# markweberdev/maskbit

Hardware: AMD Instinct MI355X
Metric: images/sec (256x256, 64-step MaskBit-12bit, CFG) (higher is better)
Workload: dtype f16

## Files before the change

include/maskbit_hip_diag.h:

```cpp
#ifndef MASKBIT_HIP_DIAG_H
#define MASKBIT_HIP_DIAG_H

#include "maskbit_hip.h"

#ifdef __cplusplus
extern "C" {
#endif

int mb_gemm(int epi, const void* A, const void* W, const float* bias, const float* residual, float* out_f32,
            void* out_h16, int M, int N, int K, int period, int variant, mb_stream stream);
int mb_gemm_ex(int epi, const void* A, const void* W, const float* bias, const float* residual, float* out_f32, void* out_h16,
               int M, int N, int K, const float* ln_stats, const float* ln_g, const float* ln_b, int period, int variant, mb_stream stream);
int mb_layernorm(const float* y, const float* gamma, const float* beta, float eps, float* x_f32, void* x_h16, void* x_lo, float* stats,
                 int M, int d, mb_stream stream);
int mb_gemm_act_split(int epi, const void* A_hi, const void* A_lo, const void* W, const float* bias, const float* residual,
                      float* out_f32, void* out_h16, int M, int N, int kw, int variant, mb_stream stream);
int mb_gemm_mini(int epi, const void* A, const void* W, const float* bias, const float* residual, float* out_f32, void* out_h16, void* out4,
                 void* out4_scale, int rows, int pair, int N, int K, int nlo, const void* const* lo, mb_stream stream);
int mb_gemm_mini_seq(int epi, const void* A, const void* W, const float* bias, const float* residual, float* out_f32, void* out_h16, void* out4,
                     void* out4_scale, void* out4l, void* out4l_scale, int rows, int pair, int seq_rows, int N, int K, int nlo, const void* const* lo, mb_stream stream);
int mb_w4_from_f32(const float* W, int N, int K, void* dst4, void* scale_out, mb_stream stream);
int mb_w4lo_from_f32(const float* W, int N, int K, void* dst4, void* scale_out, mb_stream stream);
int mb_gemm_head(int epi, const void* A_hi, const void* A_lo, const void* W_hi, const void* W_lo, const float* scale, const float* bias, int bias_per_pos,
                 float* out_f32, int M, int N, int kw, int period, mb_stream stream);
int mb_cast_f32_to_h16(const float* src, void* dst, int64_t n, mb_stream stream);
int mb_split_f32_planes(const float* src, void* hi, void* lo, int N, int K, float* scale_out, unsigned* tmp, mb_stream stream);
int mb_gemm_mini_split(int epi, const void* A_hi, const void* A_lo, const void* W, const float* bias, void* out_h16, void* out4, void* out4_scale,
                       int rows, int N, int kw, const void* const* lo, mb_stream stream);
int mb_layernorm_f4(const float* y, const float* gamma, const float* beta, float eps, float* x_f32, void* x_h16, void* x4, void* x4_scale, void* xl4,
                    void* xl4_scale, int M, int d, mb_stream stream);
int mb_layernorm_f4_seq(const float* y, const float* gamma, const float* beta, float eps, float* x_f32, void* x_h16, void* x4, void* x4_scale, void* xl4,
                        void* xl4_scale, int M, int d, int seq_rows, mb_stream stream);

int mb_layernorm_pair(const float* y, const float* gamma, const float* beta, float eps, void* x_h16, float* stats, void* x4, void* x4_scale, void* xl4,
                      void* xl4_scale, int P, int d, int seq_rows, mb_stream stream);
int mb_pairify(const float* x_f32, void* x_h16, void* x4, void* x4_scale, void* xl4, void* xl4_scale, int P, int d, int seq_rows, mb_stream stream);
int mb_embed_ln(const int64_t* tokens, const int64_t* labels, const uint8_t* drop, const float* w_in, const float* b_in, const float* class_emb,
                const float* pos, const float* gamma, const float* beta, const float* tables, float* x_f32, void* x_h16, void* x_lo, void* x4,
                void* x4_scale, void* xl4, void* xl4_scale, int nb, int seq, int m, int gbits, int d, int nclass, mb_stream stream);
int mb_embed_pair(const int64_t* tokens, const int64_t* labels, const float* w_in, const float* b_in, const float* class_emb, const float* pos,
                  const float* gamma, const float* beta, const float* tables, float* x_f32, void* x_h16, void* x4, void* x4_scale, void* xl4,
                  void* xl4_scale, int nb, int seq, int m, int gbits, int d, int nclass, mb_stream stream);
int mb_attention_pair(const void* qkv, void* out_h16, int pairs, int N, int d, int heads, mb_stream stream);
int mb_attention_pair_f4(const void* qkv, void* out_h16, void* out4, void* out4_scale, void* out4l, void* out4l_scale, int pairs, int N, int d, int heads, mb_stream stream);
int mb_attention(const void* qkv, void* out_h16, void* out4, void* out4_scale, int nb, int N, int d, int heads, mb_stream stream);
int mb_attention_probs(const void* qkv, float* out_f32, int nb, int N, int d, int heads, mb_stream stream);
int mb_gen_set_alo(mb_gen* g, int gemm_mask);
int mb_set_cu_count(int n);
int mb_gemm_ht_supported(int epi, int M, int N, int K);

int mb_seeded_noise(const int64_t* seeds, int step, float randomize_temperature, float conf_weight, float* exp_u, float* exp_noise, float* conf_u,
                    float* conf_noise, int B, int P, int C, mb_stream stream);

int mb_vq_argmin(const float* z, const float* codebook, int N, int C, int K, int l2, int splits, int64_t* idx, float* dist, mb_stream stream);

int mb_conv_layer(const void* in_h16, const float* w_oihw, const float* bias, const float* gn_gamma, const float* gn_beta, const void* residual_h16,
                  void* out_h16, float* img_nchw, uint8_t* img_nhwc_u8, const float* out_gamma, const float* out_beta, float* out_scale_shift,
                  float* out_gn_part, int* part_tiles, unsigned* saturated, int B, int H, int W, int Cin, int Cout, int ks, int up, int final_layer,
                  mb_stream stream);
int mb_groupnorm_stats(const void* x_h16, const float* gamma, const float* beta, float* scale_shift, int B, int HW, int C, mb_stream stream);
int mb_avgpool2(const void* x_h16, void* y_h16, int B, int H, int W, int C, mb_stream stream);
int mb_s2d(const void* x_h16, void* y_h16, int B, int H, int W, int C, mb_stream stream);

int mb_conv_relu_layer(const void* in_h16, const float* w_oihw, const float* bias, void* out_h16, unsigned* saturated, int B, int H, int W, int Cin,
                       int Cout, int ks, mb_stream stream);
int mb_maxpool2(const void* x_h16, void* y_h16, int B, int H, int W, int C, mb_stream stream);
int mb_lpips_input(const float* real, const float* fake, const float* shift_scale, void* out_h16, int B, int H, int W, int clamp01, mb_stream stream);
int mb_lpips_distance(const void* feat_a, const void* feat_b, const float* w, int B, int HW, int C, double* per_image, mb_stream stream);
int mb_lpips_features(mb_lpips* h, const float* real, const float* fake, int B, int H, int W, int clamp01, void* tap0, void* tap1, void* tap2, void* tap3,
                      void* tap4, mb_stream stream);

int mb_convbn_layer(const void* in_h16, const float* w_oihw, const float* scale, const float* shift, void* out_h16, unsigned* saturated, int B, int H,
                    int W, int Cin, int Cout, int kh, int kw, int stride, int ph, int pw, int in_off, int in_cs, int out_off, int out_cs, int variant,
                    mb_stream stream);
int mb_pool3(const void* x_h16, void* y_h16, int B, int H, int W, int C, int mode, int in_off, int in_cs, int out_off, int out_cs, mb_stream stream);
int mb_inception_input(const uint8_t* u8, void* out_h16, int B, int H, int W, mb_stream stream);
int mb_inception_taps(mb_inception* h, const uint8_t* u8, int B, int H, int W, void* map0, void* map1, void* map2, void* map3, float* tap64,
                      float* tap192, float* tap768, float* pool, float* logits_unbiased, float* logits, mb_stream stream);

int mb_spatial_attention(const void* q, const void* k, const void* v, void* out_h16, unsigned* sat, int B, int N, int ld, int ldo, mb_stream stream);
int mb_taming_set_tap(mb_taming* h, int block, void* out_h16);

#ifdef __cplusplus
}
#endif
#endif
```

maskbit_amd/_lib.py:

```python
from __future__ import annotations

import ctypes as C
import os
from typing import Optional

_HERE = os.path.dirname(os.path.abspath(__file__))
LIB_PATH = os.path.join(_HERE, "libmaskbit_hip.so")
ABI_VERSION = 8


class GenCfg(C.Structure):
    _fields_ = [(n, C.c_int) for n in ("bits", "splits", "hidden", "heads", "depth", "mlp", "seq", "nclass", "prenorm", "embed_tables", "precision")]


class DecCfg(C.Structure):
    _fields_ = [("token_size", C.c_int), ("hidden_channels", C.c_int), ("num_resolutions", C.c_int),
                ("num_res_blocks", C.c_int), ("num_channels", C.c_int), ("channel_mult", C.c_int * 8),
                ("latent_size", C.c_int), ("build_encoder", C.c_int), ("sample_with_conv", C.c_int),
                ("enc_res_blocks", C.c_int)]


class SamplePlan(C.Structure):
    _fields_ = [("num_steps", C.c_int), ("use_guidance", C.c_int), ("scale", C.POINTER(C.c_float)),
                ("temperature", C.POINTER(C.c_float)), ("mask_len", C.POINTER(C.c_int)), ("step_begin", C.c_int), ("step_end", C.c_int)]


class EditPlan(C.Structure):
    _fields_ = [("num_steps", C.c_int), ("use_guidance", C.c_int), ("scale", C.POINTER(C.c_float)),
                ("temperature", C.POINTER(C.c_float)), ("mask_ratio", C.POINTER(C.c_float)), ("step_begin", C.c_int), ("step_end", C.c_int)]


SIGNATURES = {
    "mb_gen_saturation_count": (C.c_int, [C.c_void_p, C.POINTER(C.c_uint), C.c_int, C.c_void_p]),
    "mb_abi_version": (C.c_int, []),
    "mb_last_error": (C.c_char_p, []),
    "mb_gen_create": (C.c_int, [C.POINTER(GenCfg), C.c_int, C.POINTER(C.c_void_p)]),
    "mb_gen_destroy": (None, [C.c_void_p]),
    "mb_gen_load": (C.c_int, [C.c_void_p, C.c_char_p, C.c_void_p, C.POINTER(C.c_int64), C.c_int, C.c_void_p]),
    "mb_gen_set_alo": (C.c_int, [C.c_void_p, C.c_int]),
    "mb_gen_forward": (C.c_int, [C.c_void_p, C.c_void_p, C.c_void_p, C.c_void_p, C.c_void_p, C.c_int, C.c_void_p]),
    "mb_gen_forward_cfg": (C.c_int, [C.c_void_p, C.c_void_p, C.c_void_p, C.c_void_p, C.c_int, C.c_void_p]),
    "mb_gen_forward_attn": (C.c_int, [C.c_void_p, C.c_void_p, C.c_void_p, C.c_void_p, C.c_void_p, C.c_void_p, C.c_int, C.c_void_p]),
    "mb_sample_step": (C.c_int, [C.c_void_p, C.c_void_p, C.c_float, C.c_float, C.c_void_p, C.c_void_p, C.c_int,
                                 C.c_void_p, C.c_void_p, C.c_void_p, C.c_int, C.c_int, C.c_int, C.c_int, C.c_void_p]),
    "mb_dec_create": (C.c_int, [C.POINTER(DecCfg), C.c_int, C.POINTER(C.c_void_p)]),
    "mb_dec_destroy": (None, [C.c_void_p]),
    "mb_dec_load": (C.c_int, [C.c_void_p, C.c_char_p, C.c_void_p, C.POINTER(C.c_int64), C.c_int, C.c_void_p]),
    "mb_dec_decode": (C.c_int, [C.c_void_p, C.c_void_p, C.c_void_p, C.c_void_p, C.c_int, C.c_void_p]),
    "mb_dec_saturation_count": (C.c_int, [C.c_void_p, C.POINTER(C.c_uint), C.c_int, C.c_void_p]),
    "mb_enc_encode": (C.c_int, [C.c_void_p, C.c_void_p, C.c_void_p, C.c_void_p, C.c_void_p, C.c_int, C.c_void_p]),
    "mb_dec_create_vq": (C.c_int, [C.POINTER(DecCfg), C.c_int, C.c_int, C.c_int, C.POINTER(C.c_void_p)]),
    "mb_dec_decode_latent": (C.c_int, [C.c_void_p, C.c_void_p, C.c_void_p, C.c_void_p, C.c_int, C.c_void_p]),
    "mb_enc_encode_vq": (C.c_int, [C.c_void_p, C.c_void_p, C.c_void_p, C.c_void_p, C.c_void_p, C.c_void_p, C.c_int, C.c_void_p]),
    "mb_vq_argmin": (C.c_int, [C.c_void_p, C.c_void_p, C.c_int, C.c_int, C.c_int, C.c_int, C.c_int, C.c_void_p, C.c_void_p, C.c_void_p]),
    "mb_sample": (C.c_int, [C.c_void_p, C.c_void_p, C.POINTER(SamplePlan), C.c_void_p, C.c_int, C.c_void_p, C.c_void_p,
                            C.c_void_p, C.c_void_p, C.c_void_p, C.c_void_p, C.c_void_p]),
    "mb_sample_step_edit": (C.c_int, [C.c_void_p, C.c_void_p, C.c_float, C.c_float, C.c_void_p, C.c_void_p, C.c_float, C.c_void_p,
                                      C.c_void_p, C.c_void_p, C.c_void_p, C.c_int, C.c_int, C.c_int, C.c_int, C.c_void_p]),
    "mb_sample_edit": (C.c_int, [C.c_void_p, C.c_void_p, C.POINTER(EditPlan), C.c_void_p, C.c_int, C.c_void_p, C.c_void_p, C.c_void_p,
                                 C.c_void_p, C.c_void_p, C.c_void_p, C.c_void_p, C.c_void_p]),
    "mb_sample_step_seeded": (C.c_int, [C.c_void_p, C.c_void_p, C.c_float, C.c_float, C.c_void_p, C.c_int, C.c_float, C.c_float, C.c_float, C.c_void_p,
                                        C.c_void_p, C.c_void_p, C.c_void_p, C.c_int, C.c_int, C.c_int, C.c_int, C.c_void_p]),
    "mb_sample_seeded": (C.c_int, [C.c_void_p, C.c_void_p, C.POINTER(EditPlan), C.c_void_p, C.c_int, C.c_void_p, C.c_void_p, C.c_float,
                                   C.POINTER(C.c_float), C.c_void_p, C.c_void_p, C.c_void_p, C.c_void_p, C.c_void_p]),
    "mb_seeded_noise": (C.c_int, [C.c_void_p, C.c_int, C.c_float, C.c_float, C.c_void_p, C.c_void_p, C.c_void_p, C.c_void_p, C.c_int, C.c_int, C.c_int,
                                  C.c_void_p]),
    "mb_edit_init": (C.c_int, [C.c_void_p, C.c_void_p, C.c_void_p, C.c_void_p, C.c_int, C.c_int, C.c_int, C.c_int, C.c_void_p]),
    "mb_edit_token_mask": (C.c_int, [C.c_void_p, C.c_void_p, C.c_int, C.c_int, C.c_int, C.c_int, C.c_void_p]),
    "mb_edit_composite": (C.c_int, [C.c_void_p, C.c_void_p, C.c_void_p, C.c_void_p, C.c_void_p, C.c_int, C.c_int, C.c_int, C.c_int, C.c_void_p]),
    "mb_gemm_ex": (C.c_int, [C.c_int, C.c_void_p, C.c_void_p, C.c_void_p, C.c_void_p, C.c_void_p, C.c_void_p, C.c_int, C.c_int, C.c_int,
                             C.c_void_p, C.c_void_p, C.c_void_p, C.c_int, C.c_int, C.c_void_p]),
    "mb_layernorm": (C.c_int, [C.c_void_p, C.c_void_p, C.c_void_p, C.c_float, C.c_void_p, C.c_void_p, C.c_void_p, C.c_void_p, C.c_int, C.c_int, C.c_void_p]),
    "mb_w4_from_f32": (C.c_int, [C.c_void_p, C.c_int, C.c_int, C.c_void_p, C.c_void_p, C.c_void_p]),
    "mb_w4lo_from_f32": (C.c_int, [C.c_void_p, C.c_int, C.c_int, C.c_void_p, C.c_void_p, C.c_void_p]),
    "mb_gemm_head": (C.c_int, [C.c_int, C.c_void_p, C.c_void_p, C.c_void_p, C.c_void_p, C.c_void_p, C.c_void_p, C.c_int, C.c_void_p, C.c_int, C.c_int,
                               C.c_int, C.c_int, C.c_void_p]),
    "mb_cast_f32_to_h16": (C.c_int, [C.c_void_p, C.c_void_p, C.c_int64, C.c_void_p]),
    "mb_split_f32_planes": (C.c_int, [C.c_void_p, C.c_void_p, C.c_void_p, C.c_int, C.c_int, C.c_void_p, C.c_void_p, C.c_void_p]),
    "mb_layernorm_f4": (C.c_int, [C.c_void_p, C.c_void_p, C.c_void_p, C.c_float, C.c_void_p, C.c_void_p, C.c_void_p, C.c_void_p, C.c_void_p, C.c_void_p,
                                  C.c_int, C.c_int, C.c_void_p]),
    "mb_layernorm_f4_seq": (C.c_int, [C.c_void_p, C.c_void_p, C.c_void_p, C.c_float] + [C.c_void_p] * 6 + [C.c_int] * 3 + [C.c_void_p]),
    "mb_layernorm_pair": (C.c_int, [C.c_void_p, C.c_void_p, C.c_void_p, C.c_float] + [C.c_void_p] * 6 + [C.c_int] * 3 + [C.c_void_p]),
    "mb_pairify": (C.c_int, [C.c_void_p] * 6 + [C.c_int] * 3 + [C.c_void_p]),
    "mb_embed_ln": (C.c_int, [C.c_void_p] * 17 + [C.c_int] * 6 + [C.c_void_p]),
    "mb_embed_pair": (C.c_int, [C.c_void_p] * 15 + [C.c_int] * 6 + [C.c_void_p]),
    "mb_attention": (C.c_int, [C.c_void_p, C.c_void_p, C.c_void_p, C.c_void_p, C.c_int, C.c_int, C.c_int, C.c_int, C.c_void_p]),
    "mb_attention_probs": (C.c_int, [C.c_void_p, C.c_void_p, C.c_int, C.c_int, C.c_int, C.c_int, C.c_void_p]),
    "mb_attention_pair": (C.c_int, [C.c_void_p, C.c_void_p, C.c_int, C.c_int, C.c_int, C.c_int, C.c_void_p]),
    "mb_attention_pair_f4": (C.c_int, [C.c_void_p, C.c_void_p, C.c_void_p, C.c_void_p, C.c_void_p, C.c_void_p, C.c_int, C.c_int, C.c_int, C.c_int, C.c_void_p]),
    "mb_gemm_mini": (C.c_int, [C.c_int, C.c_void_p, C.c_void_p, C.c_void_p, C.c_void_p, C.c_void_p, C.c_void_p, C.c_void_p, C.c_void_p, C.c_int, C.c_int,
                               C.c_int, C.c_int, C.c_int, C.POINTER(C.c_void_p), C.c_void_p]),
    "mb_gemm_mini_seq": (C.c_int, [C.c_int, C.c_void_p, C.c_void_p, C.c_void_p, C.c_void_p, C.c_void_p, C.c_void_p, C.c_void_p, C.c_void_p, C.c_void_p, C.c_void_p, C.c_int, C.c_int,
                                   C.c_int, C.c_int, C.c_int, C.c_int, C.POINTER(C.c_void_p), C.c_void_p]),
    "mb_gemm_mini_split": (C.c_int, [C.c_int, C.c_void_p, C.c_void_p, C.c_void_p, C.c_void_p, C.c_void_p, C.c_void_p, C.c_void_p, C.c_int, C.c_int, C.c_int,
                                     C.POINTER(C.c_void_p), C.c_void_p]),
    "mb_gemm_act_split": (C.c_int, [C.c_int, C.c_void_p, C.c_void_p, C.c_void_p, C.c_void_p, C.c_void_p, C.c_void_p, C.c_void_p, C.c_int, C.c_int, C.c_int,
                                    C.c_int, C.c_void_p]),
    "mb_gemm": (C.c_int, [C.c_int, C.c_void_p, C.c_void_p, C.c_void_p, C.c_void_p, C.c_void_p, C.c_void_p, C.c_int, C.c_int, C.c_int,
                          C.c_int, C.c_int, C.c_void_p]),
    "mb_conv_layer": (C.c_int, [C.c_void_p] * 13 + [C.POINTER(C.c_int), C.POINTER(C.c_uint)] + [C.c_int] * 8 + [C.c_void_p]),
    "mb_groupnorm_stats": (C.c_int, [C.c_void_p, C.c_void_p, C.c_void_p, C.c_void_p, C.c_int, C.c_int, C.c_int, C.c_void_p]),
    "mb_avgpool2": (C.c_int, [C.c_void_p, C.c_void_p, C.c_int, C.c_int, C.c_int, C.c_int, C.c_void_p]),
    "mb_s2d": (C.c_int, [C.c_void_p, C.c_void_p, C.c_int, C.c_int, C.c_int, C.c_int, C.c_void_p]),
    "mb_eval_workspace_bytes": (C.c_size_t, [C.c_int, C.c_int, C.c_int, C.c_int]),
    "mb_eval_images": (C.c_int, [C.c_void_p, C.c_void_p, C.c_int, C.c_int, C.c_int, C.c_int, C.c_uint, C.c_int, C.c_void_p, C.c_void_p, C.c_void_p, C.c_void_p]),
    "mb_eval_codebook": (C.c_int, [C.c_void_p, C.c_int64, C.c_int, C.c_void_p, C.c_void_p, C.c_void_p]),
    "mb_mlm_workspace_bytes": (C.c_size_t, [C.c_int, C.c_int, C.c_int, C.c_int]),
    "mb_mlm_state_bytes": (C.c_size_t, []),
    "mb_mlm_mask": (C.c_int, [C.c_void_p, C.c_void_p, C.c_void_p, C.c_int64, C.c_void_p, C.c_void_p, C.c_int, C.c_int, C.c_int, C.c_void_p]),
    "mb_mlm_loss": (C.c_int, [C.c_void_p, C.c_void_p, C.c_void_p, C.c_float, C.c_int, C.c_int, C.c_int, C.c_int, C.c_void_p, C.c_void_p, C.c_void_p,
                              C.c_void_p, C.c_void_p]),
    "mb_lpips_create": (C.c_int, [C.c_int, C.c_int, C.c_int, C.POINTER(C.c_void_p)]),
    "mb_lpips_destroy": (None, [C.c_void_p]),
    "mb_lpips_load": (C.c_int, [C.c_void_p, C.c_char_p, C.c_void_p, C.POINTER(C.c_int64), C.c_int, C.c_void_p]),
    "mb_lpips_forward": (C.c_int, [C.c_void_p, C.c_void_p, C.c_void_p, C.c_int, C.c_int, C.c_int, C.c_int, C.c_void_p, C.c_void_p, C.c_void_p]),
    "mb_lpips_saturation_count": (C.c_int, [C.c_void_p, C.POINTER(C.c_uint), C.c_int, C.c_void_p]),
    "mb_conv_relu_layer": (C.c_int, [C.c_void_p] * 4 + [C.POINTER(C.c_uint)] + [C.c_int] * 6 + [C.c_void_p]),
    "mb_maxpool2": (C.c_int, [C.c_void_p, C.c_void_p, C.c_int, C.c_int, C.c_int, C.c_int, C.c_void_p]),
    "mb_lpips_input": (C.c_int, [C.c_void_p, C.c_void_p, C.c_void_p, C.c_void_p, C.c_int, C.c_int, C.c_int, C.c_int, C.c_void_p]),
    "mb_lpips_distance": (C.c_int, [C.c_void_p, C.c_void_p, C.c_void_p, C.c_int, C.c_int, C.c_int, C.c_void_p, C.c_void_p]),
    "mb_lpips_features": (C.c_int, [C.c_void_p, C.c_void_p, C.c_void_p, C.c_int, C.c_int, C.c_int, C.c_int] + [C.c_void_p] * 6),
    "mb_fid_accumulate": (C.c_int, [C.c_void_p, C.c_int, C.c_int, C.c_int, C.c_int64, C.c_void_p, C.c_void_p, C.c_void_p]),
    "mb_is_workspace_bytes": (C.c_size_t, [C.c_int, C.c_int]),
    "mb_is_accumulate": (C.c_int, [C.c_void_p, C.c_int, C.c_int, C.c_int, C.c_int64, C.c_void_p, C.c_void_p, C.c_void_p, C.c_void_p]),
    "mb_inception_create": (C.c_int, [C.c_int, C.POINTER(C.c_void_p)]),
    "mb_inception_destroy": (None, [C.c_void_p]),
    "mb_inception_load": (C.c_int, [C.c_void_p, C.c_char_p, C.c_void_p, C.POINTER(C.c_int64), C.c_int, C.c_void_p]),
    "mb_inception_forward": (C.c_int, [C.c_void_p, C.c_void_p, C.c_int, C.c_int, C.c_int, C.c_void_p, C.c_void_p, C.c_void_p, C.c_void_p]),
    "mb_inception_saturation_count": (C.c_int, [C.c_void_p, C.POINTER(C.c_uint), C.c_int, C.c_void_p]),
    "mb_convbn_layer": (C.c_int, [C.c_void_p] * 5 + [C.POINTER(C.c_uint)] + [C.c_int] * 15 + [C.c_void_p]),
    "mb_pool3": (C.c_int, [C.c_void_p, C.c_void_p] + [C.c_int] * 9 + [C.c_void_p]),
    "mb_inception_input": (C.c_int, [C.c_void_p, C.c_void_p, C.c_int, C.c_int, C.c_int, C.c_void_p]),
    "mb_inception_taps": (C.c_int, [C.c_void_p, C.c_void_p, C.c_int, C.c_int, C.c_int] + [C.c_void_p] * 11),
    "mb_taming_create": (C.c_int, [C.c_int, C.c_int, C.POINTER(C.c_void_p)]),
    "mb_taming_destroy": (None, [C.c_void_p]),
    "mb_taming_load": (C.c_int, [C.c_void_p, C.c_char_p, C.c_void_p, C.POINTER(C.c_int64), C.c_int, C.c_void_p]),
    "mb_taming_encode": (C.c_int, [C.c_void_p, C.c_void_p, C.c_void_p, C.c_void_p, C.c_void_p, C.c_void_p, C.c_int, C.c_void_p]),
    "mb_taming_decode": (C.c_int, [C.c_void_p, C.c_void_p, C.c_void_p, C.c_void_p, C.c_int, C.c_void_p]),
    "mb_taming_decode_latent": (C.c_int, [C.c_void_p, C.c_void_p, C.c_void_p, C.c_void_p, C.c_int, C.c_void_p]),
    "mb_taming_saturation_count": (C.c_int, [C.c_void_p, C.POINTER(C.c_uint), C.c_int, C.c_void_p]),
    "mb_taming_set_tap": (C.c_int, [C.c_void_p, C.c_int, C.c_void_p]),
    "mb_spatial_attention": (C.c_int, [C.c_void_p] * 5 + [C.c_int] * 4 + [C.c_void_p]),
    "mb_set_cu_count":(C.c_int, [C.c_int]),
    "mb_gemm_ht_supported": (C.c_int, [C.c_int, C.c_int, C.c_int, C.c_int]),
    "mb_prof_enable": (C.c_int, [C.c_int]),
    "mb_prof_read": (C.c_int, [C.c_char_p, C.c_int]),
}

_lib: Optional[C.CDLL] = None


def load() -> C.CDLL:
    global _lib
    if _lib is not None:
        return _lib
    import torch
    if not os.path.exists(LIB_PATH):
        raise RuntimeError(
            f"{LIB_PATH} is missing: the MaskBit HIP kernels are not built. Run `python -c 'import __graft_entry__ as g; "
            f"g.build()'` (needs hipcc, gfx950). There is no CPU fallback in maskbit_amd.")
    lib = C.CDLL(LIB_PATH)
    for name, (res, args) in SIGNATURES.items():
        fn = getattr(lib, name)
        fn.restype = res
        fn.argtypes = args
    v = lib.mb_abi_version()
    if v != ABI_VERSION:
        raise RuntimeError(f"libmaskbit_hip.so ABI {v} != binding ABI {ABI_VERSION}; rebuild")
    _lib = lib
    return lib


def check(rc: int, what: str = "") -> None:
    if rc != 0:
        msg = load().mb_last_error()
        raise RuntimeError(f"{what or 'libmaskbit_hip'} failed (code {rc}): {msg.decode() if msg else '?'}")


def prof_enable(on, every: int = 1) -> None:
    load().mb_prof_enable(max(1, int(every)) if on else 0)


def prof_read() -> dict:
    buf = C.create_string_buffer(1 << 16)
    n = load().mb_prof_read(buf, len(buf))
    if n < 0:
        check(n, "mb_prof_read")
    out = {}
    for line in buf.value.decode().splitlines():
        name, calls, ms = line.split()
        out[name] = (int(calls), float(ms))
    return out
```

maskbit_amd/csrc/attention.hip:

```cpp
#include <type_traits>

#include "mb_kernels.h"

namespace mb {

constexpr int ATT_SDEPTH = 3;
constexpr int ATT_NKT = 18;
constexpr int ATT_NP = ATT_NKT * 16;
constexpr int ATT_NW = 4;
constexpr int ATT_MAXQT = (ATT_NKT + ATT_NW - 1) / ATT_NW;

typedef __attribute__((ext_vector_type(4))) unsigned u32x4;

__device__ __forceinline__ uint2 fp4_row8(const f32x4 (&o)[4], float inv, float mul) {
  uint32_t p[4];
#pragma unroll
  for (int nt = 0; nt < 4; ++nt) p[nt] = fp4_pack4(o[nt][0] * inv, o[nt][1] * inv, o[nt][2] * inv, o[nt][3] * inv, mul);
  const auto sw = __builtin_amdgcn_permlane16_swap((p[0] & 0xffffu) | (p[2] << 16), (p[1] & 0xffffu) | (p[3] << 16), false, false);
  const uint32_t q0 = __builtin_amdgcn_perm(sw[1], sw[0], 0x05040100u);
  const uint32_t q1 = __builtin_amdgcn_perm(sw[1], sw[0], 0x07060302u);
  const auto sx = __builtin_amdgcn_permlane32_swap(q0, q1, false, false);
  return make_uint2(sx[0], sx[1]);
}

__device__ __forceinline__ uint2 fp4_row8_vals(const f32x4 (&lo)[4], float mul) {
  uint32_t p[4];
#pragma unroll
  for (int nt = 0; nt < 4; ++nt) p[nt] = fp4_pack4(lo[nt][0], lo[nt][1], lo[nt][2], lo[nt][3], mul);
  const auto sw = __builtin_amdgcn_permlane16_swap((p[0] & 0xffffu) | (p[2] << 16), (p[1] & 0xffffu) | (p[3] << 16), false, false);
  const uint32_t q0 = __builtin_amdgcn_perm(sw[1], sw[0], 0x05040100u);
  const uint32_t q1 = __builtin_amdgcn_perm(sw[1], sw[0], 0x07060302u);
  const auto sx = __builtin_amdgcn_permlane32_swap(q0, q1, false, false);
  return make_uint2(sx[0], sx[1]);
}
__device__ __forceinline__ uint2 fp4_lo_block(const f32x4 (&o)[4], float inv, uint32_t& sbyte) {
  f32x4 lo[4];
  float am = 0.f;
#pragma unroll
  for (int nt = 0; nt < 4; ++nt)
#pragma unroll
    for (int r = 0; r < 4; ++r) { const float v = o[nt][r] * inv; lo[nt][r] = v - (float)to_h(v); am = fmaxf(am, fabsf(lo[nt][r])); }
  am = rows_max(am);
  sbyte = fp4_scale_byte_nosat(am);
  return fp4_row8_vals(lo, fp4_scale_mul_nosat(am));
}

template <int DH, int AUX = 0>
__global__ __launch_bounds__(64 * ATT_NW, 2) void attention_kernel(const h16* __restrict__ qkv, h16* __restrict__ out,
                                                          int N, int d, int heads, float scale_log2e, int sq_off = 0,
                                                          uint8_t* __restrict__ out4 = nullptr, uint8_t* __restrict__ out4s = nullptr, int out4_nseq = 0,
                                                          uint8_t* __restrict__ out4l = nullptr, uint8_t* __restrict__ out4ls = nullptr) {
  constexpr int ROW = DH * 2;
  constexpr int SL = DH / 8;
  constexpr int KS = DH / 32;
  constexpr int NT = DH / 16;
  constexpr int RPI = 64 / SL;
  constexpr int NINST = ATT_NP / RPI;
  __shared__ __attribute__((aligned(16))) char smem[2 * ATT_NP * ROW];

  const int tid = threadIdx.x, lane = tid & 63;
  const int wave = __builtin_amdgcn_readfirstlane(tid >> 6);
  char* Ks = smem;
  char* Vs = Ks + ATT_NP * ROW;
  const int sq0 = blockIdx.x / heads, h = blockIdx.x - sq0 * heads;
  const size_t rs = (size_t)3 * d;
  constexpr int NPASS = AUX == 4 ? 2 : 1;
  f32x4 oc[AUX == 4 ? ATT_MAXQT - 1 : 1][DH / 16];
  constexpr int LAST_WAVES = ATT_NKT - ATT_NW * (ATT_MAXQT - 1);
  __shared__ __attribute__((aligned(16))) float oc_last[AUX == 4 ? LAST_WAVES * 64 * DH / 4 : 4];
#pragma unroll 1
  for (int pass = 0; pass < NPASS; ++pass) {
  const int sq = sq0 + (AUX == 4 ? pass * sq_off : sq_off);
  const h16* base = qkv + (size_t)sq * N * rs + h * DH;
  if (AUX == 4 && pass > 0) __syncthreads();

  auto kswz = [](int row) { return SL == 8 ? ((row >> 1) & 7) : ((0 - (row >> 2)) & 3); };
  auto vswz = [](int row) { return SL == 8 ? (((row >> 1) & 3) << 1) : (((row >> 1) & 1) << 1); };

  for (int j = wave; j < NINST; j += ATT_NW) {
    const int row = j * RPI + lane / SL, p = lane % SL;
    const h16* src = base + (size_t)min(row, N - 1) * rs;
    MB_GLDS16(src + d + (p ^ kswz(row)) * 8, Ks + j * 1024);
    MB_GLDS16(src + 2 * d + (p ^ vswz(row)) * 8, Vs + j * 1024);
  }
  const int wlast = wave;
  auto qt_of = [&](int i) { return i < ATT_MAXQT - 1 ? wave + ATT_NW * i : ATT_NW * (ATT_MAXQT - 1) + wlast; };
  const int l15 = lane & 15, g = lane >> 4;
  const int nqt = (N + 15) / 16;
  h16x8 qf[ATT_MAXQT][KS];
  auto q_fetch = [&](int i) {
    const int qrow = min(qt_of(i) * 16 + l15, N - 1);
#pragma unroll
    for (int ks = 0; ks < KS; ++ks) qf[i][ks] = *(const h16x8*)(base + (size_t)qrow * rs + (ks * 4 + g) * 8);
  };
#pragma unroll
  for (int i = 0; i < (AUX == 4 ? 1 : ATT_MAXQT); ++i) q_fetch(i);
  asm volatile("s_waitcnt vmcnt(0)" ::: "memory");
  __syncthreads();

  const int koff = l15 * ROW;
  const int vrow = g * 4 + (l15 >> 2), vchunk = (l15 & 3) * 8;
  unsigned vb_nt[NT];
#pragma unroll
  for (int nt = 0; nt < NT; ++nt)
    vb_nt[nt] = (unsigned)(uintptr_t)Vs + vrow * ROW + ((((nt * 32 + vchunk) >> 4) ^ vswz(vrow)) << 4) + (vchunk & 8);

#pragma unroll
  for (int i = 0; i < ATT_MAXQT; ++i) {
    const int qt = qt_of(i);
    if (qt >= nqt) break;
    f32x4 s[ATT_NKT];
    constexpr int GK = ATT_SDEPTH, NG = ATT_NKT / GK;
    static_assert(ATT_NKT % GK == 0, "whole groups");
    h16x8 kfr[2][GK][KS];
    auto k_fetch = [&](h16x8 (&dst)[GK][KS], int grp) {
#pragma unroll
      for (int j = 0; j < GK; ++j) {
        const int kt = grp * GK + j, row = kt * 16 + l15;
#pragma unroll
        for (int ks = 0; ks < KS; ++ks) dst[j][ks] = *(const h16x8*)(Ks + kt * 16 * ROW + koff + (((ks * 4 + g) ^ kswz(row)) * 16));
      }
    };
    k_fetch(kfr[0], 0);
#pragma unroll
    for (int grp = 0; grp < NG; ++grp) {
      if (grp + 1 < NG) k_fetch(kfr[(grp + 1) & 1], grp + 1);
#pragma unroll
      for (int ks = 0; ks < KS; ++ks)
#pragma unroll
        for (int j = 0; j < GK; ++j) {
          const int kt = grp * GK + j;
          if (ks == 0) s[kt] = f32x4{0.f, 0.f, 0.f, 0.f};
          if (kt == ATT_NKT - 1 && kt * 16 >= N) continue;
          s[kt] = MB_MFMA_16x16x32(kfr[grp & 1][j][ks], qf[i][ks], s[kt]);
        }
      __builtin_amdgcn_sched_barrier(0);
    }
    if (AUX == 4 && i + 1 < ATT_MAXQT) q_fetch(i + 1);
    float mx = -INFINITY;
#pragma unroll
    for (int kt = 0; kt < ATT_NKT; ++kt)
#pragma unroll
      for (int r = 0; r < 4; ++r) {
        if (kt >= ATT_NKT - 2) s[kt][r] = (kt * 16 + g * 4 + r < N) ? s[kt][r] : -INFINITY;
        mx = fmaxf(mx, s[kt][r]);
      }
    mx = rows_max(mx);
// ... 33 lines not shown
        else
          asm volatile("s_waitcnt lgkmcnt(0)" : "+v"(cur[0][0]), "+v"(cur[0][1]), "+v"(cur[1][0]), "+v"(cur[1][1]),
                       "+v"(cur[2][0]), "+v"(cur[2][1]), "+v"(cur[3][0]), "+v"(cur[3][1])::"memory");
      } else {
        if (more_in_flight)
          asm volatile("s_waitcnt lgkmcnt(4)" : "+v"(cur[0][0]), "+v"(cur[0][1]), "+v"(cur[1][0]), "+v"(cur[1][1])::"memory");
        else
          asm volatile("s_waitcnt lgkmcnt(0)" : "+v"(cur[0][0]), "+v"(cur[0][1]), "+v"(cur[1][0]), "+v"(cur[1][1])::"memory");
      }
      __builtin_amdgcn_sched_barrier(0);
      const f32x4 p0 = s[2 * kb], p1 = s[2 * kb + 1];
      const h16x8 pf = {(h16)p0[0], (h16)p0[1], (h16)p0[2], (h16)p0[3],
                         (h16)p1[0], (h16)p1[1], (h16)p1[2], (h16)p1[3]};
#pragma unroll
      for (int nt = 0; nt < NT; ++nt) {
        const u32x4 raw = {cur[nt][0].x, cur[nt][0].y, cur[nt][1].x, cur[nt][1].y};
        o[nt] = MB_MFMA_16x16x32(__builtin_bit_cast(h16x8, raw), pf, o[nt]);
      }
      __builtin_amdgcn_sched_barrier(0);
    };
    constexpr int NKB = ATT_NKT / 2;
    issue(va, std::integral_constant<int, 0>{});
    auto step = [&](auto kbc) {
      constexpr int kb = decltype(kbc)::value;
      if constexpr (kb < NKB) {
        if constexpr (kb + 1 < NKB) issue(vb, std::integral_constant<int, kb + 1>{});
        consume(va, kb, kb + 1 < NKB);
        if constexpr (kb + 1 < NKB) {
          if constexpr (kb + 2 < NKB) issue(va, std::integral_constant<int, kb + 2>{});
          consume(vb, kb + 1, kb + 2 < NKB);
        }
      }
    };
    step(std::integral_constant<int, 0>{}); step(std::integral_constant<int, 2>{}); step(std::integral_constant<int, 4>{});
    step(std::integral_constant<int, 6>{}); step(std::integral_constant<int, 8>{});
    static_assert(NKB <= 10, "add steps");
    const int q = qt * 16 + l15;
    if constexpr ((AUX == 4 || AUX == 5) && DH == 64) {
      if (out4 && (AUX != 4 || pass == 0)) {
        float am = 0.f;
#pragma unroll
        for (int nt = 0; nt < NT; ++nt)
#pragma unroll
          for (int r = 0; r < 4; ++r) am = fmaxf(am, fabsf(o[nt][r]));
        am = rows_max(am) * inv;
        const float mul = fp4_scale_mul_nosat(am);
        const uint2 pk8 = fp4_row8(o, inv, mul);
        uint32_t lob = 0;
        uint2 lo8 = make_uint2(0u, 0u);
        if (out4l) lo8 = fp4_lo_block(o, inv, lob);
        if (q < 256) {
          const size_t row = (size_t)sq * N + q;
          if (g == 0) out4s[fp4_scale_index(h, out4_nseq, sq, q)] = (uint8_t)fp4_scale_byte_nosat(am);
          *(uint2*)(out4 + row * 2 * d + (h * DH) / 2 + (g >> 1) * 16 + (g & 1) * 8) = pk8;
          if (out4l) {
            if (g == 0) out4ls[fp4_scale_index(h, out4_nseq, sq, q)] = (uint8_t)lob;
            *(uint2*)(out4l + row * 2 * d + (h * DH) / 2 + (g >> 1) * 16 + (g & 1) * 8) = lo8;
          }
        }
      }
    }
    if (q < N) {
      const size_t ooff = ((size_t)sq * N + q) * d + h * DH;
#pragma unroll
      for (int nt = 0; nt < NT; ++nt) {
        f32x4 v = {o[nt][0] * inv, o[nt][1] * inv, o[nt][2] * inv, o[nt][3] * inv};
        if constexpr (AUX == 4) {
          if (i < ATT_MAXQT - 1) { f32x4& r = oc[i < ATT_MAXQT - 1 ? i : 0][nt]; if (pass == 0) r = v; else v = v - r; }
          else { f32x4* slot = (f32x4*)oc_last + ((qt - ATT_NW * (ATT_MAXQT - 1)) * NT + nt) * 64 + lane; if (pass == 0) *slot = v; else v = v - *slot; }
        }
        const h16x4 hi = {to_h(v[0]), to_h(v[1]), to_h(v[2]), to_h(v[3])};
        *(h16x4*)(out + ooff + nt * 16 + g * 4) = hi;
      }
    }
  }
  }
}

constexpr int ATTL_KB = 128;
template <int DH, bool PAIRM = false>
__global__ __launch_bounds__(256, 2) void attention_long_kernel(const h16* __restrict__ qkv, h16* __restrict__ out,
                                                               int N, int d, int heads, int nchunk, float scale_log2e, int sq_off = 0,
                                                               uint8_t* __restrict__ out4 = nullptr, uint8_t* __restrict__ out4s = nullptr, int out4_nseq = 0,
                                                               uint8_t* __restrict__ out4l = nullptr, uint8_t* __restrict__ out4ls = nullptr) {
  constexpr int ROW = DH * 2, SL = DH / 8, KS = DH / 32, NT = DH / 16, RPI = 64 / SL;
  constexpr int BLK_BYTES = ATTL_KB * ROW;
  constexpr int NINST = ATTL_KB / RPI;
  constexpr int NKT = ATTL_KB / 16;
  __shared__ __attribute__((aligned(16))) char smem[2 * 2 * BLK_BYTES];
  const int tid = threadIdx.x, lane = tid & 63;
  const int wave = __builtin_amdgcn_readfirstlane(tid >> 6);
  int bid = blockIdx.x;
  const int chunk = bid % nchunk; bid /= nchunk;
  const int sq0 = bid / heads, h = bid - sq0 * heads;
  const size_t rs = (size_t)3 * d;
  auto kswz = [](int row) { return SL == 8 ? ((row >> 1) & 7) : ((0 - (row >> 2)) & 3); };
  auto vswz = [](int row) { return SL == 8 ? (((row >> 1) & 3) << 1) : (((row >> 1) & 1) << 1); };
  const int nblk = (N + ATTL_KB - 1) / ATTL_KB;
  f32x4 oc[NT];
#pragma unroll 1
  for (int pass = 0; pass < (PAIRM ? 2 : 1); ++pass) {
  const int sq = sq0 + pass * sq_off;
  const h16* base = qkv + (size_t)sq * N * rs + h * DH;
  if (PAIRM && pass > 0) __syncthreads();
  auto stage = [&](int b, int buf) {
    char* Kb = smem + buf * 2 * BLK_BYTES;
    char* Vb = Kb + BLK_BYTES;
    for (int j = wave; j < NINST; j += 4) {
      const int r = j * RPI + lane / SL, p = lane % SL;
      const h16* src = base + (size_t)min(b * ATTL_KB + r, N - 1) * rs;
      MB_GLDS16(src + d + (p ^ kswz(r)) * 8, Kb + j * 1024);
      MB_GLDS16(src + 2 * d + (p ^ vswz(r)) * 8, Vb + j * 1024);
    }
  };
  const int l15 = lane & 15, g = lane >> 4;
  const int qt = chunk * 4 + wave;
  h16x8 qf[KS];
  {
    const int qrow = min(qt * 16 + l15, N - 1);
#pragma unroll
    for (int ks = 0; ks < KS; ++ks) qf[ks] = *(const h16x8*)(base + (size_t)qrow * rs + (ks * 4 + g) * 8);
  }
  const int koff = l15 * ROW;
  const int vrow = g * 4 + (l15 >> 2), vchunk = (l15 & 3) * 8;
  unsigned vb_nt[NT];
#pragma unroll
  for (int nt = 0; nt < NT; ++nt) vb_nt[nt] = vrow * ROW + ((((nt * 32 + vchunk) >> 4) ^ vswz(vrow)) << 4) + (vchunk & 8);

  float m_run = -INFINITY, l_run = 0.f;
  f32x4 o[NT];
#pragma unroll
  for (int nt = 0; nt < NT; ++nt) o[nt] = f32x4{0.f, 0.f, 0.f, 0.f};

  stage(0, 0);
  for (int b = 0; b < nblk; ++b) {
    if (b + 1 < nblk) stage(b + 1, (b + 1) & 1);
    if (b + 1 < nblk) {
      if constexpr (NINST == 16) asm volatile("s_waitcnt vmcnt(8)" ::: "memory");
      else asm volatile("s_waitcnt vmcnt(4)" ::: "memory");
    } else asm volatile("s_waitcnt vmcnt(0)" ::: "memory");
    __syncthreads();
    const char* Kb = smem + (b & 1) * 2 * BLK_BYTES;
    const unsigned Vb = (unsigned)(uintptr_t)(Kb + BLK_BYTES);
    f32x4 sblk[NKT];
#pragma unroll
    for (int kt = 0; kt < NKT; ++kt) {
      sblk[kt] = f32x4{0.f, 0.f, 0.f, 0.f};
      const int row = kt * 16 + l15;
#pragma unroll
      for (int ks = 0; ks < KS; ++ks) {
        const h16x8 kf = *(const h16x8*)(Kb + kt * 16 * ROW + koff + (((ks * 4 + g) ^ kswz(row)) * 16));
        sblk[kt] = MB_MFMA_16x16x32(kf, qf[ks], sblk[kt]);
      }
    }
    const int key0 = b * ATTL_KB;
    float mx = -INFINITY;
#pragma unroll
    for (int kt = 0; kt < NKT; ++kt)
#pragma unroll
      for (int r = 0; r < 4; ++r) {
        if (key0 + kt * 16 + g * 4 + r >= N) sblk[kt][r] = -INFINITY;
        mx = fmaxf(mx, sblk[kt][r]);
      }
    mx = rows_max(mx);
    const float m_new = fmaxf(m_run, mx);
    const float alpha = __builtin_amdgcn_exp2f((m_run - m_new) * scale_log2e);
    const float mxs = m_new * scale_log2e;
    float sum = 0.f;
    h16x4 pk[NKT];
#pragma unroll
    for (int kt = 0; kt < NKT; ++kt) {
      float p[4];
#pragma unroll
      for (int r = 0; r < 4; ++r) { p[r] = __builtin_amdgcn_exp2f(fmaf(sblk[kt][r], scale_log2e, -mxs)); sum += p[r]; }
      pk[kt] = h16x4{(h16)p[0], (h16)p[1], (h16)p[2], (h16)p[3]};
    }
    sum = rows_sum(sum);
// ... 47 lines not shown
        if (out4l) {
          if (g == 0) out4ls[fp4_scale_index(h, out4_nseq, sq, q, (N - 1) >> 6)] = (uint8_t)lob;
          *(uint2*)(out4l + row * 2 * d + (h * DH) / 2 + (g >> 1) * 16 + (g & 1) * 8) = lo8;
        }
      }
    }
  }
  if (q < N || PAIRM) {
    const size_t ooff = ((size_t)sq * N + min(q, N - 1)) * d + h * DH;
#pragma unroll
    for (int nt = 0; nt < NT; ++nt) {
      f32x4 v = {o[nt][0] * inv, o[nt][1] * inv, o[nt][2] * inv, o[nt][3] * inv};
      if constexpr (PAIRM) { if (pass == 0) oc[nt] = v; else v = v - oc[nt]; }
      if (q >= N) continue;
      const h16x4 hi = {to_h(v[0]), to_h(v[1]), to_h(v[2]), to_h(v[3])};
      *(h16x4*)(out + ooff + nt * 16 + g * 4) = hi;
    }
  }
  }
}

template <int DH>
__global__ __launch_bounds__(256) void attention_probs_kernel(const h16* __restrict__ qkv, float* __restrict__ out, int N, int d, int heads) {
  extern __shared__ __attribute__((aligned(16))) char smem[];
  const int wave = threadIdx.x >> 6, lane = threadIdx.x & 63;
  const int rows_per_seq = (N + 3) / 4;
  const int seq = blockIdx.x / rows_per_seq, r = (blockIdx.x % rows_per_seq) * 4 + wave;
  if (r >= N) return;
  float* sc = (float*)smem + (size_t)wave * 2 * N;
  float* av = sc + N;
  for (int j = lane; j < N; j += 64) av[j] = 0.f;
  const float scale = 1.0f / sqrtf((float)DH), invh = 1.0f / (float)heads;
  const h16* base = qkv + (size_t)seq * N * 3 * d;
  for (int h = 0; h < heads; ++h) {
    float q[DH];
    const h16* qp = base + (size_t)r * 3 * d + h * DH;
#pragma unroll
    for (int i = 0; i < DH / 8; ++i) {
      const h16x8 v = *(const h16x8*)(qp + i * 8);
#pragma unroll
      for (int e = 0; e < 8; ++e) q[i * 8 + e] = (float)v[e] * scale;
    }
    float mx = -3.0e38f;
    for (int j = lane; j < N; j += 64) {
      const h16* kp = base + (size_t)j * 3 * d + d + h * DH;
      float a = 0.f;
#pragma unroll
      for (int i = 0; i < DH / 8; ++i) {
        const h16x8 v = *(const h16x8*)(kp + i * 8);
#pragma unroll
        for (int e = 0; e < 8; ++e) a = fmaf(q[i * 8 + e], (float)v[e], a);
      }
      sc[j] = a;
      mx = fmaxf(mx, a);
    }
    mx = wave_max(mx);
    float sum = 0.f;
    for (int j = lane; j < N; j += 64) { const float e = expf(sc[j] - mx); sc[j] = e; sum += e; }
    sum = wave_sum(sum);
    const float w = invh / sum;
    for (int j = lane; j < N; j += 64) av[j] = fmaf(sc[j], w, av[j]);
  }
  float* orow = out + ((size_t)seq * N + r) * N;
  for (int j = lane; j < N; j += 64) orow[j] = av[j];
}

int attention_probs(hipStream_t s, const h16* qkv, float* out, int nb, int N, int d, int heads) {
  const int dh = d / heads;
  const size_t lds = (size_t)4 * 2 * N * sizeof(float);
  if ((dh != 32 && dh != 64) || lds > 160 * 1024) return -1;
  dim3 grid(nb * ((N + 3) / 4)), block(256);
  if (dh == 64) {
    (void)hipFuncSetAttribute((const void*)attention_probs_kernel<64>, hipFuncAttributeMaxDynamicSharedMemorySize, (int)lds);
    hipLaunchKernelGGL(attention_probs_kernel<64>, grid, block, lds, s, qkv, out, N, d, heads);
  } else {
    (void)hipFuncSetAttribute((const void*)attention_probs_kernel<32>, hipFuncAttributeMaxDynamicSharedMemorySize, (int)lds);
    hipLaunchKernelGGL(attention_probs_kernel<32>, grid, block, lds, s, qkv, out, N, d, heads);
  }
  return 0;
}

static bool att_streams(int N) { return N > ATT_NP || N < ATT_NP - 32; }

void attention(hipStream_t s, const h16* qkv, h16* out, int nb, int N, int d, int heads, uint8_t* out4, uint8_t* out4s) {
  const int dh = d / heads;
  const float scale_log2e = 1.4426950408889634f / sqrtf((float)dh);
  if (att_streams(N)) {
    const int nchunk = (N + 63) / 64;
    const bool f4 = N > ATT_NP && (N - 1) % 64 == 0;
    dim3 grid(nb * heads * nchunk), block(256);
    if (dh == 64) hipLaunchKernelGGL(attention_long_kernel<64>, grid, block, 0, s, qkv, out, N, d, heads, nchunk, scale_log2e, 0, f4 ? out4 : nullptr, f4 ? out4s : nullptr, nb);
    else hipLaunchKernelGGL(attention_long_kernel<32>, grid, block, 0, s, qkv, out, N, d, heads, nchunk, scale_log2e);
    return;
  }
  dim3 grid(nb * heads), block(64 * ATT_NW);
  if (out4 && dh == 64 && N == 257)
    hipLaunchKernelGGL((attention_kernel<64, 5>), grid, block, 0, s, qkv, out, N, d, heads, scale_log2e, 0, out4, out4s, nb);
  else if (dh == 64) hipLaunchKernelGGL(attention_kernel<64>, grid, block, 0, s, qkv, out, N, d, heads, scale_log2e);
  else hipLaunchKernelGGL(attention_kernel<32>, grid, block, 0, s, qkv, out, N, d, heads, scale_log2e);
}

int attention_pair(hipStream_t s, const h16* qkv, h16* out, int P, int N, int d, int heads, uint8_t* out4, uint8_t* out4s, uint8_t* out4l, uint8_t* out4ls) {
  const int dh = d / heads;
  if (dh != 64 && dh != 32) return -1;
  if ((out4l || out4ls) && (!out4 || !out4s || !out4l || !out4ls)) return -1;
  const float scale_log2e = 1.4426950408889634f / sqrtf((float)dh);
  if (att_streams(N)) {
    if ((out4 || out4s) && (dh != 64 || (N - 1) % 64 || N < ATT_NP)) return -1;
    const int nchunk = ((N + 15) / 16 + 3) / 4;
    dim3 grid(P * heads * nchunk), block(256);
    if (dh == 64) hipLaunchKernelGGL((attention_long_kernel<64, true>), grid, block, 0, s, qkv, out, N, d, heads, nchunk, scale_log2e, P, out4, out4s, P, out4l, out4ls);
    else hipLaunchKernelGGL((attention_long_kernel<32, true>), grid, block, 0, s, qkv, out, N, d, heads, nchunk, scale_log2e, P);
    return 0;
  }
  dim3 grid(P * heads), block(64 * ATT_NW);
  if ((out4 || out4s) && (dh != 64 || N != 257)) return -1;
  if (dh == 64) hipLaunchKernelGGL((attention_kernel<64, 4>), grid, block, 0, s, qkv, out, N, d, heads, scale_log2e, P, out4, out4s, P, out4l, out4ls);
  else hipLaunchKernelGGL((attention_kernel<32, 4>), grid, block, 0, s, qkv, out, N, d, heads, scale_log2e, P);
  return 0;
}

}
```

maskbit_amd/csrc/diag.hip:

```cpp
#include <hip/hip_runtime.h>

#include "../../include/maskbit_hip_diag.h"
#include "mb_abi.h"
#include "mb_conv.h"
#include "mb_kernels.h"
#include "mb_spattn.h"
#include "mb_vq.h"

using mb::fail;
using mb::launched;
using mb::ProfScope;

namespace {

int run_gemm(mb_stream stream, int epi, const mb::GemmArgs& a, int variant, const char* mini = nullptr) {
  ProfScope p("gemm_diag", (hipStream_t)stream);
  if (mb::gemm_tn((hipStream_t)stream, (mb::GemmEpi)epi, a, variant))
    return mini ? fail(-3, "%s: shape refused", mini) : fail(-3, "GEMM shape M=%d N=%d K=%d is outside the kernels' shapes", a.M, a.N, a.K);
  return launched();
}

int w4_entry(const char* what, decltype(mb::w4_from_f32)* pack, const float* W, int N, int K, void* dst4, void* scale_out, mb_stream stream) {
  if (!W || !dst4 || !scale_out || N <= 0 || K <= 0 || N % 64 || K % 128) return fail(-1, "%s: bad arguments", what);
  pack((hipStream_t)stream, W, (uint8_t*)dst4, N, K, (uint8_t*)scale_out);
  return launched();
}

int pool_entry(const char* what, decltype(mb::launch_s2d)* launch, const void* x, void* y, int B, int H, int W, int C, mb_stream stream) {
  if (!x || !y) return fail(-1, "%s: null argument", what);
  if (B <= 0 || H <= 0 || W <= 0 || H % 2 || W % 2 || C <= 0 || C % 8) return fail(-1, "%s: H and W must be even, C a multiple of 8", what);
  launch((hipStream_t)stream, (const h16*)x, (h16*)y, B, H, W, C);
  return launched();
}

int f4_rows(const char* who, mb::Fp4Rows& f4, void* x4, void* x4_scale, void* xl4, void* xl4_scale, int rows, int d, int seq_rows) {
  f4 = mb::Fp4Rows{};
  if ((x4 != nullptr) != (x4_scale != nullptr) || (xl4 != nullptr) != (xl4_scale != nullptr)) return fail(-1, "%s: an e2m1 copy and its scale array go together", who);
  if (!x4 && !xl4) return 0;
  if (d != 768 && d != 1024) return fail(-1, "%s: e2m1 copies are written at d = 768 / 1024 only, not %d", who, d);
  if (seq_rows < 65 || (seq_rows - 1) % 64 || rows % seq_rows)
    return fail(-1, "%s: e2m1 copies: sequences of 64 k tokens + the class token, whole sequences (%d rows of %d)", who, rows, seq_rows);
  f4 = mb::Fp4Rows{(uint8_t*)x4, (uint8_t*)x4_scale, (uint8_t*)xl4, (uint8_t*)xl4_scale, rows / seq_rows, seq_rows};
  return 0;
}

int embed_args(const char* who, mb::EmbedArgs& e, const int64_t* tokens, const int64_t* labels, const float* w_in, const float* b_in, const float* class_emb,
               const float* pos, const float* gamma, const float* beta, const float* tables, float* x_f32, void* x_h16, void* x4, void* x4_scale, void* xl4,
               void* xl4_scale, int nb, int seq, int m, int gbits, int d, int nclass) {
  if (!tokens || !labels || !class_emb || !pos || !gamma || !beta || !x_f32 || !x_h16 || (!tables && (!w_in || !b_in))) return fail(-1, "%s: null argument", who);
  if (nb <= 0 || seq <= 0 || m <= 0 || gbits <= 0 || d <= 0 || nclass < 0) return fail(-1, "%s: bad sizes", who);
  if (d > 2048) return fail(-1, "%s: d = %d is beyond the row kernels (2048)", who, d);
  if ((int64_t)m * gbits > 24) return fail(-1, "%s: %d groups of %d bits are beyond the embed kernels (24 bits)", who, m, gbits);
  if (tables && m > 8) return fail(-1, "%s: %d embedding tables are beyond the embed kernel (8)", who, m);
  mb::Fp4Rows f4;
  if (int rc = f4_rows(who, f4, x4, x4_scale, xl4, xl4_scale, nb * (seq + 1), d, seq + 1)) return rc;
  e = mb::EmbedArgs{tokens, labels, nullptr, nullptr, b_in, class_emb, pos, gamma, beta, x_f32, (h16*)x_h16, nb, seq, m, gbits, d, nclass, tables};
  e.f4 = f4;
  return 0;
}
int embed_weight(const char* who, mb::DevArena& arena, mb::EmbedArgs& e, const float* w_in, hipStream_t s) {
  if (e.tables) return 0;
  const int K = e.m * e.gbits;
  float* wt = nullptr;
  arena.get(&wt, (size_t)K * e.d);
  if (int rc = arena.failed(who)) return rc;
  mb::transpose_f32(s, w_in, wt, e.d, K);
  e.w_in = wt;
  return 0;
}

}

extern "C" {

int mb_set_cu_count(int n) { mb::set_cu_count(n); return 0; }
int mb_gemm_ht_supported(int epi, int M, int N, int K) {
  mb::GemmArgs a{nullptr, nullptr, nullptr, nullptr, nullptr, nullptr, M, N, K, 0};
  return mb::gemm_ht_supported((mb::GemmEpi)epi, a) ? 1 : 0;
}

int mb_gemm(int epi, const void* A, const void* W, const float* bias, const float* residual, float* out_f32, void* out_h16,
            int M, int N, int K, int period, int variant, mb_stream stream) {
  if (!A || !W || !bias || epi < 0 || epi > 4) return fail(-1, "mb_gemm: bad arguments");
  if (K % 64) return fail(-1, "mb_gemm: K must be a multiple of 64");
  mb::GemmArgs a{(const h16*)A, (const h16*)W, bias, residual, out_f32, (h16*)out_h16, M, N, K, period};
  return run_gemm(stream, epi, a, variant);
}
int mb_gemm_ex(int epi, const void* A, const void* W, const float* bias, const float* residual, float* out_f32, void* out_h16,
               int M, int N, int K, const float* ln_stats, const float* ln_g, const float* ln_b, int period, int variant, mb_stream stream) {
  if (!A || !W || !bias || epi < 0 || epi > 4) return fail(-1, "mb_gemm_ex: bad arguments");
  if (K % 64) return fail(-1, "mb_gemm_ex: K must be a multiple of 64");
  if (ln_stats && (!ln_g || !ln_b || epi != mb::EPI_RES_F32)) return fail(-1, "mb_gemm_ex: LayerNorm residual needs gamma, beta and the fp32+residual epilogue");
  mb::GemmArgs a{(const h16*)A, (const h16*)W, bias, residual, out_f32, (h16*)out_h16, M, N, K, period, nullptr, ln_stats, ln_g, ln_b};
  return run_gemm(stream, epi, a, variant);
}
int mb_gemm_act_split(int epi, const void* A_hi, const void* A_lo, const void* W, const float* bias, const float* residual, float* out_f32,
                      void* out_h16, int M, int N, int kw, int variant, mb_stream stream) {
  if (!A_hi || !A_lo || !W || !bias || epi < 0 || epi > 3 || kw <= 0 || kw % 64) return fail(-1, "mb_gemm_act_split: bad arguments");
  mb::GemmArgs a{(const h16*)A_hi, (const h16*)W, bias, residual, out_f32, (h16*)out_h16, M, N, 2 * kw, 0};
  a.A2 = (const h16*)A_lo; a.kw = kw;
  return run_gemm(stream, epi, a, variant);
}
int mb_gemm_mini(int epi, const void* A, const void* W, const float* bias, const float* residual, float* out_f32, void* out_h16, void* out4,
                 void* out4_scale, int rows, int pair, int N, int K, int nlo, const void* const* lo , mb_stream stream) {
  return mb_gemm_mini_seq(epi, A, W, bias, residual, out_f32, out_h16, out4, out4_scale, nullptr, nullptr, rows, pair, 0, N, K, nlo, lo, stream);
}
int mb_gemm_mini_seq(int epi, const void* A, const void* W, const float* bias, const float* residual, float* out_f32, void* out_h16, void* out4,
                     void* out4_scale, void* out4l, void* out4l_scale, int rows, int pair, int seq_rows, int N, int K, int nlo, const void* const* lo, mb_stream stream) {
  if ((out4l || out4l_scale) && (!out4l || !out4l_scale || !out4 || !out4_scale)) return fail(-1, "mb_gemm_mini_seq: the lo copy (out4l / out4l_scale) rides with the value copy (out4 / out4_scale)");
  if (!A || !W || !bias || epi < 0 || epi > 2 || rows <= 0 || K <= 0 || K % 64 || nlo < 0 || nlo > 2 || (nlo && !lo)) return fail(-1, "mb_gemm_mini: bad arguments");
  mb::GemmArgs a{(const h16*)A, (const h16*)W, bias, residual, out_f32, (h16*)out_h16, pair ? 2 * rows : rows, N, K, 0};
  if (pair) a.pair_rows = rows;
  a.seq_rows = seq_rows;
  a.nlo = nlo;
  for (int i = 0; i < nlo; ++i) a.lo[i] = {(const uint8_t*)lo[4 * i], (const uint8_t*)lo[4 * i + 1], (const uint8_t*)lo[4 * i + 2], (const uint8_t*)lo[4 * i + 3]};
  a.out4 = (uint8_t*)out4; a.out4_scale = (uint8_t*)out4_scale;
  a.out4l = (uint8_t*)out4l; a.out4l_scale = (uint8_t*)out4l_scale;
  if ((!seq_rows && a.M % 257) || !mb::gemm_ht_supported((mb::GemmEpi)epi, a)) return fail(-3, "mb_gemm_mini: shape not supported by the sequence-aligned tiles");
  return run_gemm(stream, epi, a, 257, "mb_gemm_mini");
}
int mb_gemm_mini_split(int epi, const void* A_hi, const void* A_lo, const void* W, const float* bias, void* out_h16, void* out4, void* out4_scale,
                       int rows, int N, int kw, const void* const* lo , mb_stream stream) {
  if (!A_hi || !A_lo || !W || !bias || !out_h16 || !lo || epi < 0 || epi > 1 || rows <= 0 || rows % 257 || kw <= 0 || kw % 128)
    return fail(-1, "mb_gemm_mini_split: bad arguments");
  mb::GemmArgs a{(const h16*)A_hi, (const h16*)W, bias, nullptr, nullptr, (h16*)out_h16, rows, N, 2 * kw, 0};
  a.A2 = (const h16*)A_lo; a.kw = kw;
  a.nlo = 1;
  a.lo[0] = {(const uint8_t*)lo[0], (const uint8_t*)lo[1], (const uint8_t*)lo[2], (const uint8_t*)lo[3]};
  a.out4 = (uint8_t*)out4; a.out4_scale = (uint8_t*)out4_scale;
  if (!mb::gemm_ht_supported((mb::GemmEpi)epi, a)) return fail(-3, "mb_gemm_mini_split: shape not supported by the sequence-aligned tiles");
  return run_gemm(stream, epi, a, 257, "mb_gemm_mini_split");
}

int mb_gemm_head(int epi, const void* A_hi, const void* A_lo, const void* W_hi, const void* W_lo, const float* scale, const float* bias, int bias_per_pos,
                 float* out_f32, int M, int N, int kw, int period, mb_stream stream) {
  if (!A_hi || !A_lo || !W_hi || !bias || !out_f32) return fail(-1, "mb_gemm_head: null argument");
  if ((W_lo != nullptr) != (scale != nullptr)) return fail(-1, "mb_gemm_head: the weights' lo plane and the scale go together");
  if (epi != mb::EPI_GELU_F32 && epi != mb::EPI_LOGITS_F32) return fail(-1, "mb_gemm_head: epilogue 3 or 4");
  if (M <= 0 || N <= 0 || N % 4 || kw <= 0 || kw % 64) return fail(-1, "mb_gemm_head: M > 0, N a multiple of 4, kw a multiple of 64");
  if (epi == mb::EPI_LOGITS_F32 && (period < 2 || M % period)) return fail(-1, "mb_gemm_head: epilogue 4: whole sequences of period >= 2 rows");
  if (bias_per_pos && epi != mb::EPI_LOGITS_F32) return fail(-1, "mb_gemm_head: a per-position bias goes with epilogue 4");
  mb::GemmArgs a{(const h16*)A_hi, (const h16*)W_hi, bias, nullptr, out_f32, nullptr, M, N, (W_lo ? 3 : 2) * kw, period, scale};
  a.A2 = (const h16*)A_lo; a.kw = kw; a.W2 = (const h16*)W_lo;
  a.bias_per_pos = bias_per_pos;
  return run_gemm(stream, epi, a, 0, "mb_gemm_head");
}
int mb_cast_f32_to_h16(const float* src, void* dst, int64_t n, mb_stream stream) {
  if (!src || !dst || n < 0) return fail(-1, "mb_cast_f32_to_h16: bad arguments");
  mb::cast_f32_to_h16((hipStream_t)stream, src, (h16*)dst, (size_t)n);
  return launched();
}
int mb_split_f32_planes(const float* src, void* hi, void* lo, int N, int K, float* scale_out, unsigned* tmp, mb_stream stream) {
  if (!src || !hi || !lo || !scale_out || !tmp || N <= 0 || K <= 0) return fail(-1, "mb_split_f32_planes: bad arguments");
  mb::split_f32_to_h16_planes((hipStream_t)stream, src, (h16*)hi, (h16*)lo, N, K, scale_out, tmp);
  return launched();
}

int mb_w4_from_f32(const float* W, int N, int K, void* dst4, void* scale_out, mb_stream stream) {
  return w4_entry("mb_w4_from_f32", mb::w4_from_f32, W, N, K, dst4, scale_out, stream);
}
int mb_w4lo_from_f32(const float* W, int N, int K, void* dst4, void* scale_out, mb_stream stream) {
  return w4_entry("mb_w4lo_from_f32", mb::w4lo_from_f32, W, N, K, dst4, scale_out, stream);
}

int mb_layernorm(const float* y, const float* gamma, const float* beta, float eps, float* x_f32, void* x_h16, void* x_lo, float* stats, int M,
                 int d, mb_stream stream) {
  if (!y || !gamma || !beta || M <= 0 || d <= 0 || d > 2048) return fail(-1, "mb_layernorm: bad arguments");
  mb::layernorm_rows((hipStream_t)stream, y, gamma, beta, eps, x_f32, (h16*)x_h16, stats, M, d, (h16*)x_lo);
  return launched();
}
int mb_layernorm_f4_seq(const float* y, const float* gamma, const float* beta, float eps, float* x_f32, void* x_h16, void* x4, void* x4_scale, void* xl4,
                        void* xl4_scale, int M, int d, int seq_rows, mb_stream stream) {
  if (!y || !gamma || !beta || (!x4 && !xl4) || M <= 0) return fail(-1, "mb_layernorm_f4: bad arguments (an e2m1 output is required)");
  mb::Fp4Rows f4;
  if (int rc = f4_rows("mb_layernorm_f4", f4, x4, x4_scale, xl4, xl4_scale, M, d, seq_rows)) return rc;
  mb::layernorm_rows((hipStream_t)stream, y, gamma, beta, eps, x_f32, (h16*)x_h16, nullptr, M, d, nullptr, f4);
  return launched();
}
int mb_layernorm_f4(const float* y, const float* gamma, const float* beta, float eps, float* x_f32, void* x_h16, void* x4, void* x4_scale, void* xl4,
                    void* xl4_scale, int M, int d, mb_stream stream) {
  return mb_layernorm_f4_seq(y, gamma, beta, eps, x_f32, x_h16, x4, x4_scale, xl4, xl4_scale, M, d, 257, stream);
}

int mb_layernorm_pair(const float* y, const float* gamma, const float* beta, float eps, void* x_h16, float* stats, void* x4, void* x4_scale, void* xl4,
                      void* xl4_scale, int P, int d, int seq_rows, mb_stream stream) {
  if (!y || !gamma || !beta || !x_h16 || P <= 0 || d <= 0 || d > 2048) return fail(-1, "mb_layernorm_pair: bad arguments");
  mb::Fp4Rows f4;
  if (int rc = f4_rows("mb_layernorm_pair", f4, x4, x4_scale, xl4, xl4_scale, P, d, seq_rows)) return rc;
  if (mb::layernorm_pair((hipStream_t)stream, y, gamma, beta, eps, (h16*)x_h16, stats, P, d, f4))
    return fail(-3, "mb_layernorm_pair: width %d is outside the pair kernels (768 or 1024)", d);
  return launched();
}
int mb_pairify(const float* x_f32, void* x_h16, void* x4, void* x4_scale, void* xl4, void* xl4_scale, int P, int d, int seq_rows, mb_stream stream) {
  if (!x_f32 || !x_h16 || P <= 0 || d <= 0 || d > 2048) return fail(-1, "mb_pairify: bad arguments");
  mb::Fp4Rows f4;
  if (int rc = f4_rows("mb_pairify", f4, x4, x4_scale, xl4, xl4_scale, P, d, seq_rows)) return rc;
  if (mb::pairify_rows((hipStream_t)stream, x_f32, (h16*)x_h16, P, d, f4))
    return fail(-3, "mb_pairify: width %d is outside the pair kernels (768 or 1024)", d);
  return launched();
}
int mb_embed_ln(const int64_t* tokens, const int64_t* labels, const uint8_t* drop, const float* w_in, const float* b_in, const float* class_emb,
                const float* pos, const float* gamma, const float* beta, const float* tables, float* x_f32, void* x_h16, void* x_lo, void* x4,
                void* x4_scale, void* xl4, void* xl4_scale, int nb, int seq, int m, int gbits, int d, int nclass, mb_stream stream) {
  mb::EmbedArgs e;
  if (int rc = embed_args("mb_embed_ln", e, tokens, labels, w_in, b_in, class_emb, pos, gamma, beta, tables, x_f32, x_h16, x4, x4_scale, xl4, xl4_scale,
                          nb, seq, m, gbits, d, nclass)) return rc;
  e.drop = drop; e.x_lo = (h16*)x_lo;
  mb::DevArena arena;
  if (int rc = embed_weight("mb_embed_ln", arena, e, w_in, (hipStream_t)stream)) return rc;
  mb::embed_ln((hipStream_t)stream, e);
  if (hipStreamSynchronize((hipStream_t)stream) != hipSuccess) return fail(-10, "mb_embed_ln: the launch failed");
  return launched();
}
int mb_embed_pair(const int64_t* tokens, const int64_t* labels, const float* w_in, const float* b_in, const float* class_emb, const float* pos,
                  const float* gamma, const float* beta, const float* tables, float* x_f32, void* x_h16, void* x4, void* x4_scale, void* xl4,
                  void* xl4_scale, int nb, int seq, int m, int gbits, int d, int nclass, mb_stream stream) {
  const bool f4 = x4 || x4_scale || xl4 || xl4_scale;
  if (tables || (m > 0 && gbits > 0 && (int64_t)m * gbits > 24) || (!f4 && d > 0 && d <= 2048 && d != 768 && d != 1024))
    return fail(-3, "mb_embed_pair: not served by the fused kernel (embedding tables, more than 24 bits, widths other than 768 / 1024): embed_ln + pairify");
  mb::EmbedArgs e;
  if (int rc = embed_args("mb_embed_pair", e, tokens, labels, w_in, b_in, class_emb, pos, gamma, beta, tables, x_f32, x_h16, x4, x4_scale, xl4, xl4_scale,
                          nb, seq, m, gbits, d, nclass)) return rc;
  mb::DevArena arena;
  if (int rc = embed_weight("mb_embed_pair", arena, e, w_in, (hipStream_t)stream)) return rc;
  const int refused = mb::embed_pair((hipStream_t)stream, e);
  if (hipStreamSynchronize((hipStream_t)stream) != hipSuccess) return fail(-10, "mb_embed_pair: the launch failed");
  if (refused) return fail(-3, "mb_embed_pair: not served by the fused kernel");
  return launched();
}

int mb_attention(const void* qkv, void* out_h16, void* out4, void* out4_scale, int nb, int N, int d, int heads, mb_stream stream) {
  if (!qkv || !out_h16 || (!out4) != (!out4_scale) || nb <= 0 || N <= 0 || d <= 0 || heads <= 0 || d % heads) return fail(-1, "mb_attention: bad arguments");
  if (d / heads != 32 && d / heads != 64) return fail(-3, "mb_attention: head width %d is outside the attention kernels (32 or 64)", d / heads);
  ProfScope p("attention", (hipStream_t)stream);
  mb::attention((hipStream_t)stream, (const h16*)qkv, (h16*)out_h16, nb, N, d, heads, (uint8_t*)out4, (uint8_t*)out4_scale);
  return launched();
}
int mb_attention_probs(const void* qkv, float* out_f32, int nb, int N, int d, int heads, mb_stream stream) {
  if (!qkv || !out_f32 || nb <= 0 || N <= 0 || d <= 0 || heads <= 0 || d % heads) return fail(-1, "mb_attention_probs: bad arguments");
  if (mb::attention_probs((hipStream_t)stream, (const h16*)qkv, out_f32, nb, N, d, heads))
    return fail(-3, "mb_attention_probs: head width %d / N = %d tokens is outside the probabilities kernel (32 or 64; N <= 5120)", d / heads, N);
  return launched();
}
int mb_attention_pair(const void* qkv, void* out_h16, int pairs, int N, int d, int heads, mb_stream stream) {
  if (!qkv || !out_h16 || pairs <= 0 || N <= 0 || heads <= 0 || d % heads) return fail(-1, "mb_attention_pair: bad arguments");
  ProfScope p("attention", (hipStream_t)stream);
  if (mb::attention_pair((hipStream_t)stream, (const h16*)qkv, (h16*)out_h16, pairs, N, d, heads, nullptr, nullptr))
    return fail(-3, "mb_attention_pair: head width %d (N = %d tokens) is outside the attention kernels", d / heads, N);
  return launched();
}
int mb_attention_pair_f4(const void* qkv, void* out_h16, void* out4, void* out4_scale, void* out4l, void* out4l_scale, int pairs, int N, int d, int heads, mb_stream stream) {
  if (!qkv || !out_h16 || !out4 || !out4_scale || (!out4l) != (!out4l_scale) || pairs <= 0 || N <= 0 || heads <= 0 || d % heads) return fail(-1, "mb_attention_pair_f4: bad arguments");
  ProfScope p("attention", (hipStream_t)stream);
  if (mb::attention_pair((hipStream_t)stream, (const h16*)qkv, (h16*)out_h16, pairs, N, d, heads, (uint8_t*)out4, (uint8_t*)out4_scale, (uint8_t*)out4l, (uint8_t*)out4l_scale))
    return fail(-3, "mb_attention_pair_f4: head width %d / N = %d tokens: no e2m1 copy for this shape", d / heads, N);
  return launched();
}

int mb_seeded_noise(const int64_t* seeds, int step, float randomize_temperature, float conf_weight, float* exp_u, float* exp_noise, float* conf_u,
                    float* conf_noise, int B, int P, int C, mb_stream stream) {
  if (!seeds || !exp_noise || !conf_noise) return fail(-1, "mb_seeded_noise: null argument");
  if (B <= 0 || P <= 0 || C <= 0 || step < 0) return fail(-1, "mb_seeded_noise: bad sizes");
  if (exp_u == exp_noise || conf_u == conf_noise) return fail(-1, "mb_seeded_noise: the uniforms and the noise must not alias");
  if (mb::seeded_noise_dump((hipStream_t)stream, seeds, step, randomize_temperature, conf_weight, exp_u, exp_noise, conf_u, conf_noise, B, P, C))
    return fail(-1, "mb_seeded_noise: C=%d or P=%d too large", C, P);
  return launched();
}

int mb_vq_argmin(const float* z, const float* codebook, int N, int C, int K, int l2, int splits, int64_t* idx, float* dist, mb_stream stream) {
  if (!z || !codebook || !idx) return fail(-1, "mb_vq_argmin: null argument");
  if (int rc = mb::vq_argmin(z, codebook, N, C, K, l2, splits, idx, dist, (hipStream_t)stream)) return rc;
  return launched();
}

int mb_conv_layer(const void* in_h16, const float* w_oihw, const float* bias, const float* gn_gamma, const float* gn_beta, const void* residual_h16,
                  void* out_h16, float* img_nchw, uint8_t* img_nhwc_u8, const float* out_gamma, const float* out_beta, float* out_scale_shift,
                  float* out_gn_part, int* part_tiles, unsigned* saturated, int B, int H, int W, int Cin, int Cout, int ks, int up_, int final_layer,
                  mb_stream stream) {
  using namespace mb;
  hipStream_t s = (hipStream_t)stream;
  const bool fin = final_layer != 0, up = up_ != 0;
  if (!in_h16 || !w_oihw || B <= 0 || Cin <= 0 || Cout <= 0) return fail(-1, "mb_conv_layer: null or empty argument");
  if (ks < 1 || ks > 3) return fail(-1, "mb_conv_layer: ks must be 1, 2 or 3");
  if (H <= 0 || W <= 0 || H % TH8 || W % TW) return fail(-1, "mb_conv_layer: the output must be whole 8 x 16 pixel tiles");
  if (fin && (ks != 3 || up || Cout > 4 || residual_h16 || !(img_nchw || img_nhwc_u8))) return fail(-1, "mb_conv_layer: final layer: ks 3, at most 4 channels, no residual, an image output");
  if (!fin && (!out_h16 || Cout % 4)) return fail(-1, "mb_conv_layer: fp16 output: Cout must be a multiple of 4");
  if (up && ks != 3) return fail(-1, "mb_conv_layer: upsampling goes with ks 3");
  if (ks == 2 && (Cin % 16 || gn_gamma)) return fail(-1, "mb_conv_layer: ks 2 (stride-2 conv): Cin must be a multiple of 16, no prologue");
  if ((gn_gamma != nullptr) != (gn_beta != nullptr) || (gn_gamma && (Cin % CK || Cin > 2048))) return fail(-1, "mb_conv_layer: prologue: gamma and beta, Cin a multiple of 64 up to 2048");
  if (out_scale_shift && (fin || !out_gamma || !out_beta || Cout % 32 || Cout > 2048)) return fail(-1, "mb_conv_layer: output statistics: gamma and beta, Cout a multiple of 32 up to 2048");
  Conv c;
  if (ks == 2) shape_down_conv(c, Cin); else shape_conv(c, Cin, Cout, ks, bias != nullptr, up, fin);
  if (ks == 2) { c.cout = Cout; c.cout_w = Cout; c.cout_pad = (Cout + 127) / 128 * 128; c.has_bias = bias != nullptr; }
  DevArena m;
  GnCtx gc;
  const int Hin = ks == 2 ? 2 * H : (up ? H / 2 : H), Win = ks == 2 ? 2 * W : (up ? W / 2 : W);
  if (up && (H % 2 || W % 2)) return fail(-1, "mb_conv_layer: upsampling needs even H and W");
  const size_t npix_in = (size_t)B * Hin * Win;
  h16* staged = nullptr;
  m.get(&c.w, conv_weight_elems(c)); m.get(&c.b, (size_t)c.cout_pad); m.get(&c.sat, 1);
  m.get(&gc.part, gn_part_elems(B, std::max(H, Hin), std::max(W, Win))); m.get(&gc.ss, (size_t)B * std::max(c.cin_pad, std::max(Cout, 1)));
  if (int rc = m.failed("mb_conv_layer")) return rc;
  bool ok = hipMemsetAsync(c.b, 0, c.cout_pad * sizeof(float), s) == hipSuccess && hipMemsetAsync(c.sat, 0, sizeof(unsigned), s) == hipSuccess;
  if (ok && bias) ok = hipMemcpyAsync(c.b, bias, (size_t)Cout * sizeof(float), hipMemcpyDeviceToDevice, s) == hipSuccess;
  launch_repack_conv(s, c, w_oihw);
  const h16* in = (const h16*)in_h16;
  if (ks == 2) {
    if (!m.get(&staged, npix_in * Cin)) return m.failed("mb_conv_layer");
    launch_s2d(s, in, staged, B, Hin, Win, Cin);
    in = staged;
  } else if (c.cin_pad != Cin) {
    if (!m.get(&staged, npix_in * c.cin_pad)) return m.failed("mb_conv_layer");
    ok = ok && hipMemsetAsync(staged, 0, npix_in * c.cin_pad * sizeof(h16), s) == hipSuccess &&
         hipMemcpy2DAsync(staged, c.cin_pad * sizeof(h16), in, Cin * sizeof(h16), Cin * sizeof(h16), npix_in, hipMemcpyDeviceToDevice, s) == hipSuccess;
    in = staged;
  }
  if (!ok) return fail(-10, "mb_conv_layer: copy failed");
  const float2* gn = nullptr;
  if (gn_gamma) {
    Norm n; n.c = Cin; n.g = const_cast<float*>(gn_gamma); n.b = const_cast<float*>(gn_beta);
    launch_gn(s, &gc, n, in, B, Hin * Win);
    gn = gc.ss;
  }
  launch_conv(s, &gc, c, in, gn, (const h16*)residual_h16, (h16*)out_h16, img_nchw, img_nhwc_u8, B, H, W, fin);
  const int tiles = gc.of == (const void*)out_h16 && !fin ? gc.ntile : 0;
  if (part_tiles) *part_tiles = tiles;
  if (out_gn_part && tiles) ok = hipMemcpyAsync(out_gn_part, gc.part, (size_t)B * tiles * 64 * sizeof(float), hipMemcpyDeviceToDevice, s) == hipSuccess;
  if (ok && out_scale_shift) {
    Norm n; n.c = Cout; n.g = const_cast<float*>(out_gamma); n.b = const_cast<float*>(out_beta);
    launch_gn(s, &gc, n, (const h16*)out_h16, B, H * W);
    ok = hipMemcpyAsync(out_scale_shift, gc.ss, (size_t)B * Cout * sizeof(float2), hipMemcpyDeviceToDevice, s) == hipSuccess;
  }
  unsigned nsat = 0;
  ok = ok && hipMemcpyAsync(&nsat, c.sat, sizeof(unsigned), hipMemcpyDeviceToHost, s) == hipSuccess;
  if (hipStreamSynchronize(s) != hipSuccess || !ok) return fail(-10, "mb_conv_layer: copy failed");
  if (saturated) *saturated = nsat;
  return launched();
// ... 63 lines not shown
```

maskbit_amd/csrc/engine.hip:

```cpp
#include <hip/hip_runtime.h>

#include <algorithm>
#include <cstdio>
#include <cstring>
#include <string>
#include <vector>

#include "../../include/maskbit_hip_diag.h"
#include "mb_abi.h"
#include "mb_kernels.h"

using mb::fail;
using mb::g_prof;
using mb::launched;
using mb::ProfScope;

struct F4Buf { uint8_t *v = nullptr, *s = nullptr; };

struct mb_gen {
  mb_gen_cfg c{};
  int max_seqs = 0, chunk_seqs = 0, N = 0, C = 0, gbits = 0, device = 0;
  struct Layer {
    h16 *wqkv = nullptr, *wo = nullptr, *w1 = nullptr, *w2 = nullptr;
    float *bqkv = nullptr, *bo = nullptr, *b1 = nullptr, *b2 = nullptr;
    float *ln1g = nullptr, *ln1b = nullptr, *ln2g = nullptr, *ln2b = nullptr;
  };
  std::vector<Layer> layers;
  float *w_in = nullptr, *b_in = nullptr, *class_emb = nullptr, *pos = nullptr, *ln0g = nullptr, *ln0b = nullptr;
  h16 *wl = nullptr, *wp = nullptr;
  float *bl = nullptr, *lnhg = nullptr, *lnhb = nullptr, *bp = nullptr;
  float *lnag = nullptr, *lnab = nullptr;
  float *tables = nullptr, *bias_pos = nullptr;
  unsigned* split_tmp = nullptr;
  float *y_f32 = nullptr, *ln_stats = nullptr;
  h16 *x_h16 = nullptr, *x_lo = nullptr, *qkv = nullptr, *att = nullptr, *h = nullptr;
  bool pair_ok = false, mini_ok = false;
  F4Buf x4, xl4;
  std::vector<uint8_t*> w4, w4s;
  float* logits_tmp = nullptr;
  h16 *wl_lo = nullptr, *wp_lo = nullptr;
  float* head_scale = nullptr;
  unsigned* sat = nullptr;
  std::vector<uint8_t*> w4lo, w4los;
  F4Buf att4, h4;
  F4Buf attl4, hl4;
  struct Run {
    struct Id {
      int B = 0, steps = 0, guided = 0, kind = 0;
      bool operator==(const Id& o) const { return B == o.B && steps == o.steps && guided == o.guided && kind == o.kind; }
    } id;
    int next = -1;
    const int64_t* cfg_labels = nullptr;
    int cfg_B = 0;
  } run;
  int* num_regen = nullptr;
  int alo_mask = 0, alo_mask_built = 0;
  int64_t *tok_a = nullptr, *tok_b = nullptr, *tok_cfg = nullptr, *lab_cfg = nullptr, *pred = nullptr, *codes = nullptr;
  uint8_t* drop_cfg = nullptr;
  float* logits = nullptr;
  mb::DevArena mem;
  int loaded = 0;
};

namespace {

void alloc_f4(mb::DevArena& m, F4Buf* b, size_t rows, size_t width, size_t ntok) {
  m.zeroed(&b->v, rows * 2 * width);
  m.zeroed(&b->s, (width / 64) * ntok + 256);
}

int head_gemms(mb_gen* g, float* logits, int M, hipStream_t s) {
  using namespace mb;
  const mb_gen_cfg& c = g->c;
  const int d = c.hidden;
  int rc = 0;
  { ProfScope p("gemm_head", s, true);
    GemmArgs ga{g->x_h16, g->wl, g->bl, nullptr, g->y_f32, nullptr, M, d, 3 * d, 0, g->head_scale};
    ga.A2 = g->x_lo; ga.kw = d; ga.W2 = g->wl_lo;
    rc |= gemm_tn(s, EPI_GELU_F32, ga); }
  { ProfScope p("layernorm", s, true);
    layernorm_rows(s, g->y_f32, g->lnhg, g->lnhb, 1e-12f, nullptr, g->x_h16, nullptr, M, d, g->x_lo); }
  { ProfScope p("gemm_head", s, true);
    GemmArgs ga{g->x_h16, g->wp, c.embed_tables ? g->bias_pos : g->bp, nullptr, logits, nullptr, M, c.splits * g->C, (g->wp_lo ? 3 : 2) * d, g->N,
                g->wp_lo ? g->head_scale + 1 : nullptr};
    ga.A2 = g->x_lo; ga.kw = d; ga.W2 = g->wp_lo;
    ga.bias_per_pos = c.embed_tables;
    rc |= gemm_tn(s, EPI_LOGITS_F32, ga); }
  return rc;
}

int gen_forward_impl(mb_gen* g, const int64_t* tokens, const int64_t* labels, const uint8_t* drop, float* logits,
                     int nb, hipStream_t s, float* attn = nullptr) {
  using namespace mb;
  const mb_gen_cfg& c = g->c;
  const int d = c.hidden, f = c.mlp, N = g->N, M = nb * N;
  auto attn_maps = [&](int l) {
    return attn ? attention_probs(s, g->qkv, attn + (size_t)l * nb * N * N, nb, N, d, c.heads) : 0;
  };
  int attn_rc = 0, gemm_rc = 0;
  const bool xlo = c.precision >= 1;
  const bool wm = g->mini_ok && c.precision >= 2;
  const bool xlo_all = xlo && !wm;
  auto xlo_layer = [&](int l) { return xlo && (xlo_all || 2 * l + 1 >= c.depth); };
  h16* const xlo_ffn = xlo ? g->x_lo : nullptr;
  h16* const xlo_qkv = xlo_all ? g->x_lo : nullptr;
  Fp4Rows f4x;
  if (wm) { f4x.x4 = g->x4.v; f4x.x4s = g->x4.s; f4x.nseq = nb; f4x.seq_rows = N; }
  auto lo_set = [&](GemmArgs& ga, const uint8_t* a4, const uint8_t* a4s, int widx) {
    if (!wm) return;
    ga.nlo = 1; ga.lo[0] = {a4, a4s, g->w4lo[widx], g->w4los[widx]};
  };
  auto xgemm = [&](GemmEpi epi, const h16* W, const float* bias, h16* out, int Nout, int widx) {
    GemmArgs ga{g->x_h16, W, bias, nullptr, nullptr, out, M, Nout, d, 0};
    if (wm) ga.seq_rows = N;
    lo_set(ga, g->x4.v, g->x4.s, widx);
    if (wm && epi == EPI_GELU_H16) { ga.out4 = g->h4.v; ga.out4_scale = g->h4.s; }
    if (((widx & 3) == 2 || xlo_all) && xlo_layer(widx >> 2)) { ga.K = 2 * d; ga.A2 = g->x_lo; ga.kw = d; }
    ga.sat = g->sat;
    gemm_rc |= gemm_tn(s, epi, ga, wm ? 257 : 0);
  };
  auto rgemm = [&](const h16* A, const h16* W, const float* bias, int K, int widx, const uint8_t* a4, const uint8_t* a4s, const float* ln_g, const float* ln_b) {
    GemmArgs ga{A, W, bias, g->y_f32, g->y_f32, nullptr, M, d, K, 0};
    if (ln_g) { ga.ln_stats = g->ln_stats; ga.ln_g = ln_g; ga.ln_b = ln_b; }
    if (wm) ga.seq_rows = N;
    lo_set(ga, a4, a4s, widx);
    gemm_rc |= gemm_tn(s, EPI_RES_F32, ga, wm ? 257 : 0);
  };
  {
    ProfScope p("embed_ln", s, true);
    EmbedArgs e{tokens, labels, drop, g->w_in, g->b_in, g->class_emb, g->pos, g->ln0g, g->ln0b,
                g->y_f32, g->x_h16, nb, c.seq, c.splits, g->gbits, d, c.nclass, g->tables};
    e.x_lo = c.depth ? (c.prenorm ? nullptr : xlo_qkv) : g->x_lo;
    e.f4 = f4x;
    embed_ln(s, e);
  }
  for (int l = 0; l < c.depth; ++l) {
    const mb_gen::Layer& L = g->layers[l];
    if (c.prenorm) { ProfScope p("layernorm", s, true); layernorm_rows(s, g->y_f32, L.ln1g, L.ln1b, 1e-12f, nullptr, g->x_h16, nullptr, M, d, xlo_qkv, f4x); }
    { ProfScope p("gemm_qkv", s, true); xgemm(EPI_H16, L.wqkv, L.bqkv, g->qkv, 3 * d, 4 * l); }
    { ProfScope p("attention", s, true); attention(s, g->qkv, g->att, nb, N, d, c.heads, wm ? g->att4.v : nullptr, wm ? g->att4.s : nullptr); }
    attn_rc |= attn_maps(l);
    { ProfScope p("gemm_attn_out", s, true);
      const bool re = !c.prenorm && l > 0;
      rgemm(g->att, L.wo, L.bo, d, 4 * l + 1, g->att4.v, g->att4.s, re ? g->layers[l - 1].ln2g : nullptr, re ? g->layers[l - 1].ln2b : nullptr); }
    { ProfScope p("layernorm", s, true);
      layernorm_rows(s, g->y_f32, c.prenorm ? L.ln2g : L.ln1g, c.prenorm ? L.ln2b : L.ln1b, 1e-12f, nullptr, g->x_h16, c.prenorm ? nullptr : g->ln_stats, M, d, xlo_layer(l) ? xlo_ffn : nullptr, f4x); }
    { ProfScope p("gemm_ffn_up", s, true); xgemm(EPI_GELU_H16, L.w1, L.b1, g->h, f, 4 * l + 2); }
    { ProfScope p("gemm_ffn_down", s, true);
      rgemm(g->h, L.w2, L.b2, f, 4 * l + 3, g->h4.v, g->h4.s, c.prenorm ? nullptr : L.ln1g, c.prenorm ? nullptr : L.ln1b); }
    if (!c.prenorm) { ProfScope p("layernorm", s, true);
      const bool last = l + 1 == c.depth;
      layernorm_rows(s, g->y_f32, L.ln2g, L.ln2b, 1e-12f, nullptr, g->x_h16, g->ln_stats, M, d, last ? g->x_lo : xlo_qkv, last ? Fp4Rows{} : f4x); }
  }
  if (c.prenorm) { ProfScope p("layernorm", s, true); layernorm_rows(s, g->y_f32, g->lnag, g->lnab, 1e-12f, nullptr, g->x_h16, nullptr, M, d, g->x_lo); }
  gemm_rc |= head_gemms(g, logits, M, s);
  if (int rc = launched()) return rc;
  if (attn_rc) return fail(-3, "attention maps: head dim %d / %d tokens not supported", d / c.heads, N);
  if (gemm_rc) return fail(-3, "a trunk GEMM of this forward (%d sequences x %d tokens, hidden %d, mlp %d; precision %d%s) is outside the half-tile "
                               "kernel's shapes: its correction mini-tiles cannot run", nb, N, d, f, c.precision, wm ? ", weight-correction mini-tiles" : "");
  return 0;
}

int gen_forward_pair_impl(mb_gen* g, const int64_t* tokens, const int64_t* labels, const uint8_t* drop, float* logits, int B, bool wmode, hipStream_t s) {
  using namespace mb;
  const mb_gen_cfg& c = g->c;
  const int d = c.hidden, f = c.mlp, N = g->N, nb = 2 * B, M = nb * N, P = B * N;
  int rc = 0;
  auto alo_on = [&](int gemm) { return wmode && c.precision >= 3 && ((g->alo_mask >> gemm) & 1); };
  auto f4_for = [&](bool feeds_ffn = false) {
    Fp4Rows f;
    if (wmode) {
      f.x4 = g->x4.v; f.x4s = g->x4.s; f.nseq = B; f.seq_rows = N;
      if (alo_on(feeds_ffn ? 2 : 0)) { f.xl4 = g->xl4.v; f.xl4s = g->xl4.s; }
    }
    return f;
  };
  auto pgemm = [&](GemmEpi epi, const h16* A, const h16* W, const float* bias, h16* out16, float* res, int Nout, int K, int widx, int lo,
                   const uint8_t* a4 = nullptr, const uint8_t* a4s = nullptr, const uint8_t* al4 = nullptr, const uint8_t* al4s = nullptr) {
    GemmArgs ga{A, W, bias, res, res, out16, M, Nout, K, 0};
    ga.pair_rows = P;
    ga.seq_rows = N;
    if (epi != EPI_RES_F32) ga.sat = g->sat;
    if (lo) {
      ga.nlo = lo; ga.lo[0] = {a4, a4s, g->w4lo[widx], g->w4los[widx]};
      if (lo == 2) ga.lo[1] = {al4, al4s, g->w4[widx], g->w4s[widx]};
    }
    return ga;
  };
  {
    ProfScope p("embed_ln", s, true);
    EmbedArgs e{tokens, labels, nullptr, g->w_in, g->b_in, g->class_emb, g->pos, g->ln0g, g->ln0b,
                g->y_f32, g->x_h16, B, c.seq, c.splits, g->gbits, d, c.nclass, g->tables};
    e.f4 = f4_for();
    if (embed_pair(s, e)) {
      e.drop = drop; e.nb = nb; e.f4 = Fp4Rows{};
      embed_ln(s, e);
      rc |= pairify_rows(s, g->y_f32, g->x_h16, P, d, f4_for());
    }
  }
  if (c.prenorm && c.depth > 0) {
    ProfScope p("layernorm", s, true);
    rc |= layernorm_pair(s, g->y_f32, g->layers[0].ln1g, g->layers[0].ln1b, 1e-12f, g->x_h16, nullptr, P, d, f4_for());
  }
  for (int l = 0; l < c.depth; ++l) {
    const mb_gen::Layer& L = g->layers[l];
    const int xlo_mode = wmode ? (alo_on(2) ? 2 : 1) : 0;
    { ProfScope p("gemm_qkv", s, true);
      GemmArgs ga = pgemm(EPI_H16, g->x_h16, L.wqkv, L.bqkv, g->qkv, nullptr, 3 * d, d, 4 * l, wmode ? (alo_on(0) ? 2 : 1) : 0, g->x4.v, g->x4.s, g->xl4.v, g->xl4.s);
      rc |= gemm_tn(s, EPI_H16, ga, 257); }
    const bool lo_o = alo_on(1), lo_h = alo_on(3);
    { ProfScope p("attention", s, true); rc |= attention_pair(s, g->qkv, g->att, B, N, d, c.heads, wmode ? g->att4.v : nullptr, wmode ? g->att4.s : nullptr,
                                                              lo_o ? g->attl4.v : nullptr, lo_o ? g->attl4.s : nullptr); }
    { ProfScope p("gemm_attn_out", s, true);
      GemmArgs ga = pgemm(EPI_RES_F32, g->att, L.wo, L.bo, nullptr, g->y_f32, d, d, 4 * l + 1, wmode ? (alo_on(1) ? 2 : 1) : 0, g->att4.v, g->att4.s, g->attl4.v, g->attl4.s);
      if (l > 0 && !c.prenorm) { ga.ln_stats = g->ln_stats; ga.ln_g = g->layers[l - 1].ln2g; ga.ln_b = g->layers[l - 1].ln2b; }
      rc |= gemm_tn(s, EPI_RES_F32, ga, 257); }
    { ProfScope p("layernorm", s, true);
      rc |= layernorm_pair(s, g->y_f32, c.prenorm ? L.ln2g : L.ln1g, c.prenorm ? L.ln2b : L.ln1b, 1e-12f, g->x_h16, c.prenorm ? nullptr : g->ln_stats, P, d, f4_for(true)); }
    { ProfScope p("gemm_ffn_up", s, true);
      GemmArgs ga = pgemm(EPI_GELU_H16, g->x_h16, L.w1, L.b1, g->h, nullptr, f, d, 4 * l + 2, xlo_mode, g->x4.v, g->x4.s, g->xl4.v, g->xl4.s);
      if (wmode) { ga.out4 = g->h4.v; ga.out4_scale = g->h4.s; }
      if (lo_h) { ga.out4l = g->hl4.v; ga.out4l_scale = g->hl4.s; }
      rc |= gemm_tn(s, EPI_GELU_H16, ga, 257); }
    { ProfScope p("gemm_ffn_down", s, true);
      GemmArgs ga = pgemm(EPI_RES_F32, g->h, L.w2, L.b2, nullptr, g->y_f32, d, f, 4 * l + 3, wmode ? (alo_on(3) ? 2 : 1) : 0, g->h4.v, g->h4.s, g->hl4.v, g->hl4.s);
      if (!c.prenorm) { ga.ln_stats = g->ln_stats; ga.ln_g = L.ln1g; ga.ln_b = L.ln1b; }
      rc |= gemm_tn(s, EPI_RES_F32, ga, 257); }
    { ProfScope p("layernorm", s, true);
      if (c.prenorm) {
        if (l + 1 == c.depth) layernorm_rows(s, g->y_f32, g->lnag, g->lnab, 1e-12f, nullptr, g->x_h16, nullptr, M, d, g->x_lo);
        else rc |= layernorm_pair(s, g->y_f32, g->layers[l + 1].ln1g, g->layers[l + 1].ln1b, 1e-12f, g->x_h16, nullptr, P, d, f4_for());
      }
      else if (l + 1 == c.depth) layernorm_rows(s, g->y_f32, L.ln2g, L.ln2b, 1e-12f, nullptr, g->x_h16, g->ln_stats, M, d, g->x_lo);
      else rc |= layernorm_pair(s, g->y_f32, L.ln2g, L.ln2b, 1e-12f, g->x_h16, g->ln_stats, P, d, f4_for()); }
  }
  rc |= head_gemms(g, logits, M, s);
  if (int lrc = launched()) return lrc;
  if (rc) return fail(-3, "differential CFG forward: a kernel refused the shape (%d pairs x %d tokens, hidden %d, mlp %d)", B, N, d, f);
  return 0;
}

int gen_forward(mb_gen* g, const int64_t* tokens, const int64_t* labels, const uint8_t* drop, float* logits, int nb, hipStream_t s,
                float* attn = nullptr) {
  const int chunk = g->chunk_seqs;
  g_prof.begin_forward(true);
  if (nb <= chunk) return gen_forward_impl(g, tokens, labels, drop, logits, nb, s, attn);
  if (attn) return fail(-3, "attention maps are limited to %d sequences per call", chunk);
  const size_t P = (size_t)g->c.seq * g->c.splits;
  for (int b0 = 0; b0 < nb; b0 += chunk) {
    const int nc = nb - b0 < chunk ? nb - b0 : chunk;
    int rc = gen_forward_impl(g, tokens + (size_t)b0 * P, labels + b0, drop ? drop + b0 : nullptr, logits + (size_t)b0 * P * g->C, nc, s);
    if (rc) return rc;
  }
  return 0;
}

int gen_forward_cfg(mb_gen* g, const int64_t* tokens, const int64_t* labels, float* logits, int B, hipStream_t s) {
  const size_t P = (size_t)g->c.seq * g->c.splits;
  const bool pair = g->pair_ok && g->c.precision >= 1;
  const bool wmode = pair && g->c.precision >= 2;
  const int chunk = g->chunk_seqs / 2;
  if (chunk < 1) return fail(-1, "engine holds %d sequences: too few for a guided forward", g->chunk_seqs);
  for (int b0 = 0; b0 < B; b0 += chunk) {
    const int nc = B - b0 < chunk ? B - b0 : chunk;
    HIP_TRY(hipMemcpyAsync(g->tok_cfg, tokens + (size_t)b0 * P, nc * P * sizeof(int64_t), hipMemcpyDeviceToDevice, s));
    if (!(pair && !g->c.embed_tables && g->c.bits <= 24))
      HIP_TRY(hipMemcpyAsync(g->tok_cfg + nc * P, tokens + (size_t)b0 * P, nc * P * sizeof(int64_t), hipMemcpyDeviceToDevice, s));
    if (!(nc == B && g->run.cfg_labels == labels && g->run.cfg_B == B)) {
      HIP_TRY(hipMemcpyAsync(g->lab_cfg, labels + b0, nc * sizeof(int64_t), hipMemcpyDeviceToDevice, s));
      HIP_TRY(hipMemcpyAsync(g->lab_cfg + nc, labels + b0, nc * sizeof(int64_t), hipMemcpyDeviceToDevice, s));
      HIP_TRY(hipMemsetAsync(g->drop_cfg, 0, nc, s));
      HIP_TRY(hipMemsetAsync(g->drop_cfg + nc, 1, nc, s));
    }
    float* out = (nc == B) ? logits : g->logits_tmp;
    if (b0 == 0) g_prof.begin_forward(false);
    int rc = pair ? gen_forward_pair_impl(g, g->tok_cfg, g->lab_cfg, g->drop_cfg, out, nc, wmode, s)
                  : gen_forward_impl(g, g->tok_cfg, g->lab_cfg, g->drop_cfg, out, 2 * nc, s);
    if (rc) return rc;
    if (nc != B) {
      HIP_TRY(hipMemcpyAsync(logits + (size_t)b0 * P * g->C, out, nc * P * g->C * sizeof(float), hipMemcpyDeviceToDevice, s));
      HIP_TRY(hipMemcpyAsync(logits + (size_t)(B + b0) * P * g->C, out + (size_t)nc * P * g->C, nc * P * g->C * sizeof(float), hipMemcpyDeviceToDevice, s));
    }
  }
  return 0;
}

}

extern "C" {

int mb_abi_version(void) { return MB_ABI_VERSION; }
const char* mb_last_error(void) { return mb::g_err.c_str(); }

int mb_prof_enable(int on) {
  if (!on) g_prof.drain();
  g_prof.on = on != 0;
  if (on) { g_prof.acc.clear(); g_prof.stride = on; g_prof.tick[0] = g_prof.tick[1] = 0; }
  return 0;
}
int mb_prof_read(char* buf, int buflen) {
  g_prof.drain();
  std::string out;
  char line[256];
  for (auto& kv : g_prof.acc) {
    snprintf(line, sizeof line, "%s %ld %.6f\n", g_prof.names[kv.first].c_str(), kv.second.first, kv.second.second);
    out += line;
  }
  if ((int)out.size() + 1 > buflen) return fail(-3, "mb_prof_read: buffer too small (%zu needed)", out.size() + 1);
  memcpy(buf, out.c_str(), out.size() + 1);
  return (int)out.size();
}

int mb_gen_create(const mb_gen_cfg* cfg, int max_seqs, mb_gen** out) {
  if (!cfg || !out || max_seqs <= 0) return fail(-1, "mb_gen_create: bad arguments");
  const mb_gen_cfg& c = *cfg;
  if (c.splits <= 0 || c.bits % c.splits) return fail(-1, "bits (%d) must be divisible by splits (%d)", c.bits, c.splits);
  if (c.bits > 24) return fail(-1, "bits > 24 is not supported");
// ... 84 lines not shown
  int l = -1, sub = -1; char rest[96] = {0};
  std::string n(name);
  if (c.embed_tables && (n.rfind("prediction_layer.", 0) == 0 || n.rfind("input_proj.", 0) == 0))
    return fail(-2, "mb_gen_load: unknown checkpoint entry '%s' (embed_tables engine: tok_emb_list.* / bias.* instead)", name);
  if (sscanf(name, "transformer.layers.%d.%d.%95s", &l, &sub, rest) == 3) {
    if (l < 0 || l >= c.depth) return fail(-2, "layer index out of range in '%s'", name);
    mb_gen::Layer& L = g->layers[l];
    std::string r(rest);
    if (sub == 0) {
      if (r == "mha.in_proj_weight") { dst_h = L.wqkv; want = 3 * d * d; wrows = 3 * d; wcols = d; sidx = 4 * l; }
      else if (r == "mha.in_proj_bias") { dst_f = L.bqkv; want = 3 * d; }
      else if (r == "mha.out_proj.weight") { dst_h = L.wo; want = d * d; wrows = d; wcols = d; sidx = 4 * l + 1; }
      else if (r == "mha.out_proj.bias") { dst_f = L.bo; want = d; }
      else if (r == "norm.weight") { dst_f = L.ln1g; want = d; }
      else if (r == "norm.bias") { dst_f = L.ln1b; want = d; }
    } else if (sub == 1) {
      if (r == "net.0.weight") { dst_h = L.w1; want = f * d; wrows = f; wcols = d; sidx = 4 * l + 2; }
      else if (r == "net.0.bias") { dst_f = L.b1; want = f; }
      else if (r == "net.2.weight") { dst_h = L.w2; want = d * f; wrows = d; wcols = f; sidx = 4 * l + 3; }
      else if (r == "net.2.bias") { dst_f = L.b2; want = d; }
      else if (r == "norm.weight") { dst_f = L.ln2g; want = d; }
      else if (r == "norm.bias") { dst_f = L.ln2b; want = d; }
    }
  } else if (n == "pos_emb") { dst_f = g->pos; want = (size_t)g->N * d; }
  else if (n == "class_emb.weight") { dst_f = g->class_emb; want = (size_t)(c.nclass + 1) * d; }
  else if (n == "input_proj.weight") { dst_f = g->w_in; want = d * c.bits; }
  else if (n == "input_proj.bias") { dst_f = g->b_in; want = d; }
  else if (n == "first_layer.0.weight") { dst_f = g->ln0g; want = d; }
  else if (n == "first_layer.0.bias") { dst_f = g->ln0b; want = d; }
  else if (n == "last_layer.0.weight") { dst_h = g->wl; want = d * d; wrows = d; wcols = d; sidx = 4 * c.depth; }
  else if (n == "last_layer.0.bias") { dst_f = g->bl; want = d; }
  else if (n == "last_layer.2.weight") { dst_f = g->lnhg; want = d; }
  else if (n == "last_layer.2.bias") { dst_f = g->lnhb; want = d; }
  else if (n == "prediction_layer.weight") { dst_h = g->wp; want = (size_t)c.splits * g->C * d; wrows = c.splits * g->C; wcols = d; sidx = 4 * c.depth + 1; }
  else if (n == "prediction_layer.bias") { dst_f = g->bp; want = (size_t)c.splits * g->C; }
  else if (n == "bits_to_indices") return 0;
  else if (c.prenorm && n == "norm_after_transformer.weight") { dst_f = g->lnag; want = d; }
  else if (c.prenorm && n == "norm_after_transformer.bias") { dst_f = g->lnab; want = d; }
  else if (c.embed_tables) {
    int q = -1;
    if (sscanf(name, "tok_emb_list.%d.weight", &q) == 1 && n == "tok_emb_list." + std::to_string(q) + ".weight") {
      if (q < 0 || q >= c.splits) return fail(-2, "group index out of range in '%s'", name);
      const size_t rows = (size_t)g->C + 1;
      if (numel != rows * d) return fail(-4, "mb_gen_load: '%s' has %zu elements, expected %zu", name, numel, rows * d);
      HIP_TRY(hipMemcpyAsync(g->tables + (size_t)q * rows * d, data, numel * sizeof(float), hipMemcpyDeviceToDevice, s));
      mb::cast_f32_to_h16(s, data, g->wp + (size_t)q * g->C * d, (size_t)g->C * d);
      g->loaded++;
      return 0;
    }
    if (sscanf(name, "bias.%d", &q) == 1 && n == "bias." + std::to_string(q)) {
      if (q < 0 || q >= c.splits) return fail(-2, "group index out of range in '%s'", name);
      if (numel != (size_t)c.seq * g->C) return fail(-4, "mb_gen_load: '%s' has %zu elements, expected %zu", name, numel, (size_t)c.seq * g->C);
      HIP_TRY(hipMemcpy2DAsync(g->bias_pos + (size_t)q * g->C, (size_t)c.splits * g->C * sizeof(float), data, (size_t)g->C * sizeof(float),
                               (size_t)g->C * sizeof(float), (size_t)c.seq, hipMemcpyDeviceToDevice, s));
      g->loaded++;
      return 0;
    }
  }
  if (!dst_f && !dst_h) return fail(-2, "mb_gen_load: unknown checkpoint entry '%s'", name);
  if (numel != want) return fail(-4, "mb_gen_load: '%s' has %zu elements, expected %zu", name, numel, want);
  if (dst_f == g->w_in) mb::transpose_f32(s, data, g->w_in, (int)d, c.bits);
  else if (dst_h == g->wl) mb::split_f32_to_h16_planes(s, data, g->wl, g->wl_lo, wrows, wcols, g->head_scale, g->split_tmp);
  else if (dst_h == g->wp) mb::split_f32_to_h16_planes(s, data, g->wp, g->wp_lo, wrows, wcols, g->head_scale + 1, g->split_tmp);
  else if (dst_h) {
    mb::cast_f32_to_h16(s, data, dst_h, numel);
    if (g->mini_ok && sidx >= 0 && sidx < 4 * c.depth) {
      mb::w4lo_from_f32(s, data, g->w4lo[sidx], wrows, wcols, g->w4los[sidx]);
      if (g->w4[sidx]) mb::w4_from_f32(s, data, g->w4[sidx], wrows, wcols, g->w4s[sidx]);
    }
  }
  else HIP_TRY(hipMemcpyAsync(dst_f, data, numel * sizeof(float), hipMemcpyDeviceToDevice, s));
  g->loaded++;
  return 0;
}

int mb_gen_set_alo(mb_gen* g, int gemm_mask) {
  if (!g || gemm_mask < 0 || gemm_mask > 15) return fail(-1, "mb_gen_set_alo: mask outside [0, 15]");
  if (gemm_mask & ~g->alo_mask_built)
    return fail(-1, "mb_gen_set_alo: the handle was created (precision %d) with the activation-lo operands of GEMM mask %d only", g->c.precision, g->alo_mask_built);
  g->alo_mask = gemm_mask;
  return 0;
}

int mb_gen_saturation_count(mb_gen* g, unsigned* count, int reset, mb_stream stream) {
  if (!g || !count) return fail(-1, "mb_gen_saturation_count: null argument");
  HIP_TRY(hipMemcpyAsync(count, g->sat, sizeof(unsigned), hipMemcpyDeviceToHost, (hipStream_t)stream));
  if (reset) HIP_TRY(hipMemsetAsync(g->sat, 0, sizeof(unsigned), (hipStream_t)stream));
  HIP_TRY(hipStreamSynchronize((hipStream_t)stream));
  return 0;
}

int mb_gen_forward(mb_gen* g, const int64_t* tokens, const int64_t* labels, const uint8_t* drop, float* logits,
                   int nb, mb_stream stream) {
  if (!g || !tokens || !labels || !logits) return fail(-1, "mb_gen_forward: null argument");
  if (nb <= 0 || nb > g->max_seqs) return fail(-1, "mb_gen_forward: nb=%d outside [1, %d]", nb, g->max_seqs);
  return gen_forward(g, tokens, labels, drop, logits, nb, (hipStream_t)stream);
}

int mb_gen_forward_cfg(mb_gen* g, const int64_t* tokens, const int64_t* labels, float* logits, int B, mb_stream stream) {
  if (!g || !tokens || !labels || !logits) return fail(-1, "mb_gen_forward_cfg: null argument");
  if (B <= 0 || 2 * B > g->max_seqs) return fail(-1, "mb_gen_forward_cfg: B=%d needs %d sequences, engine holds %d", B, 2 * B, g->max_seqs);
  return gen_forward_cfg(g, tokens, labels, logits, B, (hipStream_t)stream);
}

int mb_gen_forward_attn(mb_gen* g, const int64_t* tokens, const int64_t* labels, const uint8_t* drop, float* logits, float* attn,
                        int nb, mb_stream stream) {
  if (!g || !tokens || !labels || !logits || !attn) return fail(-1, "mb_gen_forward_attn: null argument");
  if (nb <= 0 || nb > g->max_seqs) return fail(-1, "mb_gen_forward_attn: nb=%d outside [1, %d]", nb, g->max_seqs);
  return gen_forward(g, tokens, labels, drop, logits, nb, (hipStream_t)stream, attn);
}

static int sample_step_checked(const char* who, const mb::StepArgs& a, const int64_t* tokens_in, const int32_t* num_regen, float mask_ratio, hipStream_t s) {
  if (!a.logits_c || (!a.seeds && (!a.exp_noise || !a.conf_noise)) || !tokens_in || !a.tokens) return fail(-1, "%s: null argument", who);
  if (tokens_in == a.tokens) return fail(-1, "%s: tokens_in and tokens_out must not alias", who);
  if (a.B <= 0 || a.P <= 0 || a.C <= 0) return fail(-1, "%s: bad sizes", who);
  ProfScope p(a.seeds ? "sample_step_seeded" : num_regen ? "sample_step_edit" : "sample_step", s);
  if (mb::sample_step(s, a, tokens_in, num_regen, mask_ratio)) return fail(-1, "%s: C=%d or n*m=%d too large", who, a.C, a.P);
  return launched();
}

static int step_slots(int n, int m) { return n > 0 && m > 0 ? n * m : 0; }

int mb_sample_step(const float* logits_c, const float* logits_u, float scale, float temperature,
                   const float* exp_noise, const float* conf_noise, int k_mask_len, const int64_t* tokens_in,
                   int64_t* tokens_out, int64_t* pred_out, int B, int n, int m, int C, mb_stream stream) {
  mb::StepArgs a{};
  a.logits_c = logits_c; a.logits_u = logits_u; a.scale = scale; a.temperature = temperature;
  a.exp_noise = exp_noise; a.conf_noise = conf_noise; a.k_mask_len = k_mask_len;
  a.tokens = tokens_out; a.pred = pred_out; a.B = B; a.P = step_slots(n, m); a.C = C;
  return sample_step_checked("mb_sample_step", a, tokens_in, nullptr, 0.f, (hipStream_t)stream);
}

int mb_sample_step_edit(const float* logits_c, const float* logits_u, float scale, float temperature, const float* exp_noise, const float* conf_noise,
                        float mask_ratio, const int32_t* num_regen, const int64_t* tokens_in, int64_t* tokens_out, int64_t* pred_out, int B, int n, int m,
                        int C, mb_stream stream) {
  if (!num_regen) return fail(-1, "mb_sample_step_edit: null argument");
  mb::StepArgs a{};
  a.logits_c = logits_c; a.logits_u = logits_u; a.scale = scale; a.temperature = temperature;
  a.exp_noise = exp_noise; a.conf_noise = conf_noise;
  a.tokens = tokens_out; a.pred = pred_out; a.B = B; a.P = step_slots(n, m); a.C = C;
  return sample_step_checked("mb_sample_step_edit", a, tokens_in, num_regen, mask_ratio, (hipStream_t)stream);
}

int mb_sample_step_seeded(const float* logits_c, const float* logits_u, float scale, float temperature, const int64_t* seeds, int step,
                          float randomize_temperature, float conf_weight, float mask_ratio, const int32_t* num_regen, const int64_t* tokens_in,
                          int64_t* tokens_out, int64_t* pred_out, int B, int n, int m, int C, mb_stream stream) {
  if (!seeds || !num_regen) return fail(-1, "mb_sample_step_seeded: null argument");
  if (step < 0) return fail(-1, "mb_sample_step_seeded: step = %d is negative", step);
  if (pred_out && (pred_out == tokens_out || pred_out == tokens_in)) return fail(-1, "mb_sample_step_seeded: pred_out must not alias tokens_in or tokens_out");
  mb::StepArgs a{};
  a.logits_c = logits_c; a.logits_u = logits_u; a.scale = scale; a.temperature = temperature;
  a.seeds = seeds; a.step = step; a.rand_temp = randomize_temperature; a.conf_w = conf_weight;
  a.tokens = tokens_out; a.pred = pred_out; a.B = B; a.P = step_slots(n, m); a.C = C;
  return sample_step_checked("mb_sample_step_seeded", a, tokens_in, num_regen, mask_ratio, (hipStream_t)stream);
}

}

namespace {

struct RunNoise {
  const float* exp_noise = nullptr; const float* conf_noise = nullptr;
  const int64_t* seeds = nullptr; float rand_temp = 0.f; const float* conf_weight = nullptr;
};
struct RunSpec {
  const char* who = nullptr;
// ... 130 lines not shown
```

maskbit_amd/csrc/gemm.hip:

```cpp
#include <cstdio>
#include <cstdlib>

#include "mb_kernels.h"

namespace mb {

constexpr int BM = 128, BN = 128, BK = 64;
constexpr int TILE_BYTES = BM * BK * 2;

template <int EPI>
__global__ __launch_bounds__(256, 2) void gemm_tn_kernel(GemmArgs a) {
  __shared__ __attribute__((aligned(16))) char smem[4 * TILE_BYTES];
  const int tid = threadIdx.x, lane = tid & 63, wave = tid >> 6;
  const int wm = wave >> 1, wn = wave & 1;
  const int tiles_n = (a.N + BN - 1) / BN;
  const int tiles_m = (a.M + BM - 1) / BM;
  const int L = xcd_remap(blockIdx.x, tiles_m * tiles_n);
  const int m0 = (L / tiles_n) * BM, n0 = (L % tiles_n) * BN;
  const int K = a.K, KA = a.kw ? a.kw : a.K, nka = KA / BK;
  const int KW = a.kw ? a.kw : a.K, nkw = KW / BK;

  const h16* xsrc[4];
  const h16* wsrc[4];
  const ptrdiff_t a2 = a.A2 ? a.A2 - a.A : 0;
  const ptrdiff_t w2 = a.W2 ? a.W2 - a.W : 0;
#pragma unroll
  for (int j = 0; j < 4; ++j) {
    const int row = wave * 32 + j * 8 + (lane >> 3);
    const int slot = (lane & 7) ^ ((row >> 1) & 7);
    const int mr = min(m0 + row, a.M - 1), nr = min(n0 + row, a.N - 1);
    xsrc[j] = a.A + (size_t)mr * KA + slot * 8;
    wsrc[j] = a.W + (size_t)nr * KW + slot * 8;
  }
  auto stage = [&](int t, int buf) {
    const int ta = t < nka ? t : t - nka;
    char* xb = smem + buf * 2 * TILE_BYTES + wave * 32 * 128;
    char* wb = xb + TILE_BYTES;
    if (a.W2) {
      const int seg = t / nkw, tt = t - seg * nkw;
#pragma unroll
      for (int j = 0; j < 4; ++j) {
        MB_GLDS16(xsrc[j] + (seg == 1 ? a2 : 0) + tt * BK, xb + j * 8 * 128);
        MB_GLDS16(wsrc[j] + (seg == 2 ? w2 : 0) + tt * BK, wb + j * 8 * 128);
      }
      return;
    }
#pragma unroll
    for (int j = 0; j < 4; ++j) {
      MB_GLDS16(xsrc[j] + (t < nka ? 0 : a2) + ta * BK, xb + j * 8 * 128);
      MB_GLDS16(wsrc[j] + (t < nkw ? t : t - nkw) * BK, wb + j * 8 * 128);
    }
  };

  int foff[2];
#pragma unroll
  for (int kk = 0; kk < 2; ++kk)
    foff[kk] = (lane & 15) * 128 + (((kk * 4 + (lane >> 4)) ^ ((lane & 15) >> 1)) * 16);

  f32x4 acc[4][4];
#pragma unroll
  for (int i = 0; i < 4; ++i)
#pragma unroll
    for (int j = 0; j < 4; ++j) acc[i][j] = f32x4{0.f, 0.f, 0.f, 0.f};

  const int nk = K / BK;
  stage(0, 0);
  for (int t = 0; t < nk; ++t) {
    asm volatile("s_waitcnt vmcnt(0)" ::: "memory");
    __syncthreads();
    if (t + 1 < nk) stage(t + 1, (t + 1) & 1);
    const char* xb = smem + (t & 1) * 2 * TILE_BYTES + wm * 64 * 128;
    const char* wb = smem + (t & 1) * 2 * TILE_BYTES + TILE_BYTES + wn * 64 * 128;
#pragma unroll
    for (int kk = 0; kk < 2; ++kk) {
      h16x8 wf[4], xf[4];
#pragma unroll
      for (int i = 0; i < 4; ++i) wf[i] = *(const h16x8*)(wb + i * 16 * 128 + foff[kk]);
#pragma unroll
      for (int j = 0; j < 4; ++j) xf[j] = *(const h16x8*)(xb + j * 16 * 128 + foff[kk]);
#pragma unroll
      for (int i = 0; i < 4; ++i)
#pragma unroll
        for (int j = 0; j < 4; ++j)
          acc[i][j] = MB_MFMA_16x16x32(wf[i], xf[j], acc[i][j]);
    }
  }

  const float sc = a.scale ? *a.scale : 1.0f;
  bool satb = false;
#pragma unroll
  for (int j = 0; j < 4; ++j) {
    const int m = m0 + wm * 64 + j * 16 + (lane & 15);
    if (m >= a.M) continue;
    size_t orow = (size_t)m;
    const float* brow = a.bias;
    if (EPI == EPI_LOGITS_F32) {
      const int sq = m / a.period, pos = m - sq * a.period;
      if (pos == a.period - 1) continue;
      orow = (size_t)sq * (a.period - 1) + pos;
      if (a.bias_per_pos) brow = a.bias + (size_t)pos * a.N;
// ... 158 lines not shown
```

maskbit_amd/csrc/gemm_ht.hip:

```cpp
#include <algorithm>

#include "mb_kernels.h"

namespace mb {

#define MB_SWZ(r) (((r) >> 1) & 7)

typedef int i32x4 __attribute__((ext_vector_type(4)));
typedef int i32x8 __attribute__((ext_vector_type(8)));
typedef h16 h16x16 __attribute__((ext_vector_type(16)));


template <int MT, int EPI, int XP = 0, bool SEQ = false, bool PAIR = false, int NS = 1>
__global__ __launch_bounds__(512, 2) void gemm_ht_kernel(GemmArgs a, int tiles_m, int tiles_n) {
  constexpr bool HN = NS > 1, QN = NS == 4;
  constexpr int NTW = 4 / NS;
  static_assert(NS == 1 || NS == 2 || NS == 4, "column split");
  static_assert(!HN || (SEQ && !PAIR && XP == 6 && EPI == EPI_RES_F32), "half-column tiles: plain sequence tiles with mini-tiles, residual epilogue");
  static_assert(!SEQ || MT == 8, "sequence-aligned tiles use the 256-row machinery");
  static_assert(XP == 0 || XP == 6, "fp16 K-tiles, optionally with mini-tiles");
  static_assert(!PAIR || SEQ, "pair tiles are sequence-aligned");
  constexpr bool MINI = XP == 6;
  static_assert(!MINI || SEQ, "mini-tile passes are written for sequence-aligned tiles");
  constexpr int MINI_A = 128 * 64, MINI_B = 256 * 64;
  constexpr bool PERSIST = true;
  constexpr int BM = 32 * MT, MH = MT / 2;
  constexpr int AH_ROWS = BM / 2;
  constexpr int AH_BYTES = AH_ROWS * 128, BH_BYTES = 128 * 128;
  constexpr int X_BYTES = SEQ ? 1024 : 0;
  constexpr int PAR_BYTES = 2 * AH_BYTES + 2 * BH_BYTES + X_BYTES;
  constexpr int MINI_OFF = 2 * PAR_BYTES;
  constexpr int A_INSTR = AH_ROWS / 8;
  extern __shared__ __attribute__((aligned(16))) char smem[];

  const int tid = threadIdx.x, lane = tid & 63;
  const int wave = __builtin_amdgcn_readfirstlane(tid >> 6);
  const int grp = wave >> 2;
  const int wm = wave >> 2, wn = wave & 3;
  const int l15 = lane & 15, g = lane >> 4;
  const int K = a.K, nk = K / 64;
  constexpr bool SPLIT = !PAIR;
  const int KA = SPLIT && a.kw ? a.kw : K, nka = KA / 64;
  const int KW = SPLIT && a.kw ? a.kw : K, nkw = KW / 64;
  const h16* const Alo = SPLIT && a.A2 ? a.A2 : a.A;
  const h16* const Wlo = a.W;
  const int SQ = a.seq_rows ? a.seq_rows : 257;
  const int tps_sh = 31 - __builtin_clz((unsigned)((SQ - 1) >> (PAIR ? 7 : 8)));
  const int TPS = 1 << tps_sh;
  const int ntiles = tiles_m * tiles_n;

  struct Plan {
    uint32_t offA[2][2], offB[2][2], offX;
    int m0, n0;
    int cls;
    int q;
    int seq;
    int hb;
  };
  int dstA[2], dstB[2];
#pragma unroll
  for (int j = 0; j < 2; ++j) { dstA[j] = min(wave + 8 * j, A_INSTR - 1) * 1024; dstB[j] = (QN ? (wave >> 1) * 4 + (wave & 1) : wave + 8 * j) * 1024; }
  auto make_plan = [&](int vb, Plan& p) {
    int lane_o = lane;
    asm volatile("" : "+v"(lane_o));
    const int L = xcd_remap(vb, ntiles);
    const int sr = L / (8 * tiles_n);
    const int rows_sr = min(8, tiles_m - sr * 8);
    const int rem = L - sr * 8 * tiles_n;
    const int tn = rem / rows_sr, tm = sr * 8 + (rem - tn * rows_sr);
    p.m0 = SEQ ? (tm >> tps_sh) * SQ + (tm & (TPS - 1)) * (PAIR ? 128 : 256) : tm * BM; p.n0 = (tn / NS) * 256;
    p.hb = tn % NS;
    p.cls = SEQ ? (tm >> tps_sh) * SQ + SQ - 1 : 0; p.q = SEQ ? tm & (TPS - 1) : 0;
    p.seq = SEQ ? tm >> tps_sh : tm;
#pragma unroll
    for (int j = 0; j < 2; ++j) {
      const int ja = min(wave + 8 * j, A_INSTR - 1);
      const int hra = ja * 8 + (lane_o >> 3);
      const int wms = hra / (8 * MT), r = hra - wms * (8 * MT);
      const int slot_a = (lane_o & 7) ^ MB_SWZ(hra);
      const int hrb = (QN ? (wave >> 1) * 4 + (wave & 1) : wave + 8 * j) * 8 + (lane_o >> 3);
      const int wns = hrb >> 5, c = hrb & 31;
      const int slot_b = (lane_o & 7) ^ MB_SWZ(hrb);
#pragma unroll
      for (int h = 0; h < 2; ++h) {
        const int gm = PAIR ? p.m0 + h * a.pair_rows + hra : min(p.m0 + wms * (16 * MT) + h * (8 * MT) + r, a.M - 1);
        p.offA[h][j] = (uint32_t)gm * (uint32_t)(2 * KA) + slot_a * 16;
        const int gn = min(p.n0 + wns * 64 + (HN ? p.hb * (64 / NS) : h * 32) + c, a.N - 1);
        p.offB[h][j] = (uint32_t)gn * (uint32_t)(2 * KW) + slot_b * 16;
      }
    }
    p.offX = (uint32_t)(PAIR ? p.cls + ((lane_o >> 3) == 1 ? a.pair_rows : 0) : min(p.cls, a.M - 1)) * (uint32_t)(2 * KA) + ((lane_o & 7) ^ MB_SWZ(lane_o >> 3)) * 16;
  };
  auto ktile_a = [&](int u) -> const char* { if constexpr (!SPLIT) return (const char*)a.A + u * 128; return (const char*)(u < nka ? a.A : Alo) + (u < nka ? u : u - nka) * 128; };
  auto ktile_w = [&](int u) -> const char* { if constexpr (!SPLIT) return (const char*)a.W + u * 128; return (const char*)(u < nkw ? a.W : Wlo) + (u < nkw ? u : u - nkw) * 128; };
  auto dma_x = [&](const Plan& p, const char* kp, int parb) {
    if (SEQ && wave == 7) MB_GLDS16_SB(kp, p.offX, smem + parb + 2 * AH_BYTES + 2 * BH_BYTES);
  };
  auto dma_a = [&](const Plan& p, const char* kp, int parb, int h) {
    char* buf = smem + parb + h * AH_BYTES;
#pragma unroll
    for (int j = 0; j < 2; ++j) {
      MB_GLDS16_SB2(kp, p.offA[h][j], buf, dstA[j]);
    }
  };
  auto dma_b = [&](const Plan& p, const char* kp, int parb, int h) {
    if (HN && h == 1) return;
    char* buf = smem + parb + 2 * AH_BYTES + h * BH_BYTES;
#pragma unroll
    for (int j = 0; j < (QN ? 1 : 2); ++j) {
      MB_GLDS16_SB2(kp, p.offB[h][j], buf, dstB[j]);
    }
  };
  const int KM = SPLIT && a.kw ? a.kw : K;
  const int nmk = KM / 128;
  const int nseq = PAIR ? a.pair_rows / SQ : a.M / SQ;
  const int grp_bytes = PAIR ? TPS * 128 : TPS * 256;
  const bool mini_every = MINI && (PAIR ? a.nlo == 2 : !a.kw);
  struct MiniPos { const uint8_t *a4, *w4, *xs, *ws; };
  const uint32_t ml_a = (uint32_t)((lane >> 2) * 2 * KM + (((lane & 3) ^ ((lane >> 3) & 3)) * 16));
  auto ml_w = [&]() -> uint32_t { int lo_ = lane; asm volatile("" : "+v"(lo_)); return (uint32_t)lo_ * 16; };
  const uint32_t ml_xs = (uint32_t)(lane >> 5) * (uint32_t)nseq * (uint32_t)grp_bytes + (lane & 15) * 4;
  auto ml_ws = [&]() -> uint32_t { int lo_ = lane; asm volatile("" : "+v"(lo_)); return (uint32_t)(lo_ & 15) * 4; };
  auto mini_pos = [&](const Plan& p) -> MiniPos {
    constexpr int si = 0, ps = 0;
    const int m0 = p.m0, n0 = p.n0, hb = p.hb, tq = p.q, sq = p.seq;
    const uint32_t row0 = PAIR ? m0 + wave * 16 : m0 + (wave >> 2) * 128 + ps * 64 + (wave & 3) * 16;
    const uint32_t wrow = QN ? wave * 4 + hb : HN ? (wave >> 1) * 4 + hb * 2 + (wave & 1) : wave;
    const uint32_t gq = PAIR ? tq * 2 + wm : tq * 4 + wm * 2 + ps;
    MiniPos m;
    m.a4 = a.lo[si].A4 + (size_t)row0 * 2 * KM;
    m.w4 = a.lo[si].W4 + (size_t)((n0 >> 4) + wrow) * nmk * 1024;
    m.xs = a.lo[si].a_scale + ((uint32_t)sq * (uint32_t)grp_bytes + gq * 64);
    m.ws = a.lo[si].w_scale + (uint32_t)(((n0 >> 6) + wn) * nmk) * 64;
    auto uni = [](const uint8_t* q) -> const uint8_t* {
      const uint64_t v = (uint64_t)q;
      return (const uint8_t*)(((uint64_t)(uint32_t)__builtin_amdgcn_readfirstlane((int)(v >> 32)) << 32) | (uint32_t)__builtin_amdgcn_readfirstlane((int)v));
    };
    m.a4 = uni(m.a4); m.w4 = uni(m.w4); m.xs = uni(m.xs); m.ws = uni(m.ws);
    return m;
  };
  const uint32_t xs_step = 2u * (uint32_t)nseq * (uint32_t)grp_bytes;
  auto mini_step = [&](MiniPos& m) { m.a4 += 64; m.w4 += 1024; m.xs += xs_step; m.ws += 64; };
  auto mini_switch = [&](MiniPos& m) {
    const size_t back = (size_t)nmk;
    if constexpr (PAIR) {
      auto ka = (const char __attribute__((address_space(4)))*)__builtin_amdgcn_kernarg_segment_ptr();
      asm volatile("" : "+s"(ka));
      auto l = (const GemmArgs::LoSet __attribute__((address_space(4)))*)(ka + offsetof(GemmArgs, lo));
// ... 604 lines not shown
```

maskbit_amd/csrc/mb_common.h:

```cpp
#pragma once
#include <hip/hip_runtime.h>
#include <stdint.h>

typedef _Float16 h16;
#define MB_MFMA_16x16x32(a, b, c) __builtin_amdgcn_mfma_f32_16x16x32_f16(a, b, c, 0, 0, 0)
#define MB_H16_MAX 65504.0f
typedef __attribute__((ext_vector_type(2))) h16 h16x2;
typedef __attribute__((ext_vector_type(4))) h16 h16x4;
typedef __attribute__((ext_vector_type(8))) h16 h16x8;

__device__ __forceinline__ h16 to_h(float x) { return (h16)__builtin_amdgcn_fmed3f(x, -MB_H16_MAX, MB_H16_MAX); }
typedef __attribute__((ext_vector_type(4))) float f32x4;
typedef __attribute__((ext_vector_type(16))) float f32x16;

#define MB_WAVE 64

#define MB_GLDS16_AUX(gptr, ldsptr, aux)                                                        \
  __builtin_amdgcn_global_load_lds((const void __attribute__((address_space(1)))*)(gptr),       \
                                   (void __attribute__((address_space(3)))*)(ldsptr), 16, 0, aux)
#define MB_GLDS16(gptr, ldsptr) MB_GLDS16_AUX(gptr, ldsptr, 0)
#define MB_GLDS16_SB(sbase, voff, ldsptr)                                                                      \
  _Pragma("clang diagnostic push") _Pragma("clang diagnostic ignored \"-Winline-asm\"")                        \
  asm volatile("s_mov_b32 m0, %2\n\ts_nop 0\n\tglobal_load_lds_dwordx4 %0, %1"                                 \
               :: "v"((uint32_t)(voff)), "s"((const void*)(sbase)),                                             \
// ... 7 lines not shown
  _Pragma("clang diagnostic pop")

__device__ __forceinline__ float wave_sum(float v) {
#pragma unroll
  for (int o = 32; o > 0; o >>= 1) v += __shfl_xor(v, o);
  return v;
}
__device__ __forceinline__ float wave_max(float v) {
#pragma unroll
  for (int o = 32; o > 0; o >>= 1) v = fmaxf(v, __shfl_xor(v, o));
  return v;
}

typedef float f32x2 __attribute__((ext_vector_type(2)));
__device__ __forceinline__ float rows_max(float v) {
  auto a = __builtin_amdgcn_permlane16_swap(__float_as_uint(v), __float_as_uint(v), false, false);
  v = fmaxf(__uint_as_float(a[0]), __uint_as_float(a[1]));
  auto b = __builtin_amdgcn_permlane32_swap(__float_as_uint(v), __float_as_uint(v), false, false);
  return fmaxf(__uint_as_float(b[0]), __uint_as_float(b[1]));
}
__device__ __forceinline__ float row16_max(float v) {
  v = fmaxf(v, __uint_as_float(__builtin_amdgcn_update_dpp(0u, __float_as_uint(v), 0xB1, 0xF, 0xF, false)));
  v = fmaxf(v, __uint_as_float(__builtin_amdgcn_update_dpp(0u, __float_as_uint(v), 0x4E, 0xF, 0xF, false)));
  v = fmaxf(v, __uint_as_float(__builtin_amdgcn_update_dpp(0u, __float_as_uint(v), 0x141, 0xF, 0xF, false)));
  return fmaxf(v, __uint_as_float(__builtin_amdgcn_update_dpp(0u, __float_as_uint(v), 0x140, 0xF, 0xF, false)));
}
__device__ __forceinline__ float rows_sum(float v) {
  auto a = __builtin_amdgcn_permlane16_swap(__float_as_uint(v), __float_as_uint(v), false, false);
  v = __uint_as_float(a[0]) + __uint_as_float(a[1]);
  auto b = __builtin_amdgcn_permlane32_swap(__float_as_uint(v), __float_as_uint(v), false, false);
  return __uint_as_float(b[0]) + __uint_as_float(b[1]);
}
__device__ __forceinline__ f32x2 gelu_erf2(f32x2 x) {
  const float a0 = fabsf(x.x), a1 = fabsf(x.y);
  const f32x2 t = {__builtin_amdgcn_rcpf(fmaf(0.3275911f * 0.70710678118654752f, a0, 1.0f)),
                   __builtin_amdgcn_rcpf(fmaf(0.3275911f * 0.70710678118654752f, a1, 1.0f))};
  f32x2 p = __builtin_elementwise_fma(t, (f32x2)(0.5f * 1.061405429f), (f32x2)(-0.5f * 1.453152027f));
  p = __builtin_elementwise_fma(p, t, (f32x2)(0.5f * 1.421413741f));
  p = __builtin_elementwise_fma(p, t, (f32x2)(-0.5f * 0.284496736f));
  p = __builtin_elementwise_fma(p, t, (f32x2)(0.5f * 0.254829592f));
  p = p * t;
  const f32x2 w = (x * x) * (f32x2)(-0.5f * 1.4426950408889634f);
  const f32x2 e = {__builtin_amdgcn_exp2f(w.x), __builtin_amdgcn_exp2f(w.y)};
  const f32x2 h = p * e;
  return (f32x2){fmaf(-a0, h.x, fmaxf(x.x, 0.0f)), fmaf(-a1, h.y, fmaxf(x.y, 0.0f))};
}
__device__ __forceinline__ float gelu_erf(float x) { return gelu_erf2((f32x2){x, x}).x; }

__device__ __forceinline__ uint32_t fp4_scale_byte(float maxlo) {
  const int e = (__float_as_int(maxlo) >> 23) & 0xff;
  return (uint32_t)(e >= 2 ? e - 2 : 0);
}
__device__ __forceinline__ float fp4_scale_mul(float maxlo) {
  const int e = (__float_as_int(maxlo) >> 23) & 0xff;
  return e >= 2 ? __int_as_float((256 - e) << 23) : 0.0f;
}
__device__ __forceinline__ int fp4_nosat_exp(float amax) {
  const int b = __float_as_int(amax);
  return ((b >> 23) & 0xff) + (((b & 0x7fffff) > 0x400000) ? 1 : 0);
}
__device__ __forceinline__ uint32_t fp4_scale_byte_nosat(float amax) { const int e = fp4_nosat_exp(amax); return (uint32_t)(e >= 2 ? e - 2 : 0); }
__device__ __forceinline__ float fp4_scale_mul_nosat(float amax) {
  const int e = fp4_nosat_exp(amax);
  return (e >= 2 && e <= 254) ? __int_as_float((256 - e) << 23) : 0.0f;
}
__device__ __forceinline__ uint32_t fp4_code(float v) {
  const float a = fminf(fabsf(v), 6.0f);
  int k = ((__float_as_int(a) >> 23) & 0xff) - 127;
  k = max(0, min(k, 2));
  const float r = rintf(a * __int_as_float((128 - k) << 23));
  return (uint32_t)((int)r + 2 * k) | (v < 0.0f ? 8u : 0u);
}
__device__ __forceinline__ uint32_t fp4_pack4(float v0, float v1, float v2, float v3, float mul) {
  const float inv = mul > 0.f ? __builtin_amdgcn_rcpf(mul) : 1.0f;
  const float z = mul > 0.f ? 1.0f : 0.0f;
  uint32_t w = __builtin_amdgcn_cvt_scalef32_pk_fp4_f32(0u, v0 * z, v1 * z, inv, 0);
  return __builtin_amdgcn_cvt_scalef32_pk_fp4_f32(w, v2 * z, v3 * z, inv, 1) & 0xffffu;
}

__device__ __forceinline__ float ln_affine(float v, float mean, float rstd, float g, float b) {
  return __fmaf_rn(__fmul_rn(__fsub_rn(v, mean), rstd), g, b);
}

__device__ __forceinline__ int xcd_remap(int b, int nblk) {
  const int q = nblk >> 3, r = nblk & 7, x = b & 7, i = b >> 3;
  return (x < r ? x * (q + 1) : r * (q + 1) + (x - r) * q) + i;
}
```

maskbit_amd/csrc/mb_kernels.h:

```cpp
#pragma once
#include "mb_common.h"

namespace mb {

enum GemmEpi {
  EPI_H16 = 0,
  EPI_GELU_H16 = 1,
  EPI_RES_F32 = 2,
  EPI_GELU_F32 = 3,
  EPI_LOGITS_F32 = 4,
};
struct GemmArgs {
  const h16* A;
  const h16* W;
  const float* bias;
  const float* residual;
  float* out_f32;
  h16* out_h16;
  int M, N, K;
  int period;
  const float* scale = nullptr;
  const float* ln_stats = nullptr;
  const float* ln_g = nullptr;
  const float* ln_b = nullptr;
  int bias_per_pos = 0;
  const h16* A2 = nullptr;
  int kw = 0;
  const h16* W2 = nullptr;
  int pair_rows = 0;
  int seq_rows = 0;
  uint8_t* out4 = nullptr;
  uint8_t* out4_scale = nullptr;
  uint8_t* out4l = nullptr;
  uint8_t* out4l_scale = nullptr;
  struct LoSet { const uint8_t* A4; const uint8_t* a_scale; const uint8_t* W4; const uint8_t* w_scale; };
  LoSet lo[2] = {};
  int nlo = 0;
  unsigned* sat = nullptr;
};
__host__ __device__ inline size_t w4_packed_offset(int n, int k, int K) {
  const int r = n & 15, c = (k & 127) >> 5;
  return ((size_t)(n >> 4) * (K >> 7) + (k >> 7)) * 1024 + r * 64 + ((c ^ ((r >> 1) & 3)) << 4) + ((k & 31) >> 1);
}
__host__ __device__ inline size_t w4_scale_index(int n, int j, int K) {
  return (((size_t)(n >> 6) * (K >> 7) + j) * 16 + (n & 15)) * 4 + ((n >> 4) & 3);
}
__host__ __device__ inline size_t fp4_scale_index(int blk, int nseq, int seq, int r, int groups = 4) {
  return (((size_t)blk * nseq + seq) * groups + (r >> 6)) * 64 + (r & 15) * 4 + ((r >> 4) & 3);
}
int gemm_tn(hipStream_t s, GemmEpi epi, const GemmArgs& a, int variant = 0);
bool gemm_ht_supported(GemmEpi epi, const GemmArgs& a);
void gemm_ht(hipStream_t s, GemmEpi epi, const GemmArgs& a, int mt);
void set_cu_count(int n);

void w4_from_f32(hipStream_t s, const float* src, uint8_t* dst4, int N, int K, uint8_t* scale_out);
void w4lo_from_f32(hipStream_t s, const float* src, uint8_t* dst4, int N, int K, uint8_t* scale_out);

struct Fp4Rows { uint8_t* x4 = nullptr; uint8_t* x4s = nullptr; uint8_t* xl4 = nullptr; uint8_t* xl4s = nullptr; int nseq = 0; int seq_rows = 257; };

void layernorm_rows(hipStream_t s, const float* y, const float* gamma, const float* beta, float eps,
                    float* x_f32, h16* x_h16, float* stats, int M, int d, h16* x_lo = nullptr,
                    const Fp4Rows& f4 = Fp4Rows{});

int layernorm_pair(hipStream_t s, const float* y, const float* gamma, const float* beta, float eps, h16* x_h16, float* stats, int P, int d,
                   const Fp4Rows& f4 = Fp4Rows{});
int pairify_rows(hipStream_t s, const float* x32, h16* x_h16, int P, int d, const Fp4Rows& f4 = Fp4Rows{});

struct EmbedArgs {
  const int64_t* tokens;
  const int64_t* labels;
  const uint8_t* drop;
  const float* w_in;
  const float* b_in;
  const float* class_emb;
  const float* pos;
  const float* gamma; const float* beta;
  float* x_f32; h16* x_h16;
  int nb, seq, m, gbits, d, nclass;
  const float* tables = nullptr;
  h16* x_lo = nullptr;
  Fp4Rows f4;
};
void embed_ln(hipStream_t s, const EmbedArgs& a);
int embed_pair(hipStream_t s, const EmbedArgs& a);
void transpose_f32(hipStream_t s, const float* src , float* dst , int rows, int cols);

void attention(hipStream_t s, const h16* qkv, h16* out, int nb, int N, int d, int heads,
               uint8_t* out4 = nullptr, uint8_t* out4s = nullptr);
int attention_pair(hipStream_t s, const h16* qkv, h16* out, int P, int N, int d, int heads, uint8_t* out4 = nullptr, uint8_t* out4s = nullptr,
                   uint8_t* out4l = nullptr, uint8_t* out4ls = nullptr);
int attention_probs(hipStream_t s, const h16* qkv, float* out, int nb, int N, int d, int heads);

struct StepArgs {
  const float* logits_c; const float* logits_u;
  float scale, temperature;
  const float* exp_noise;
  const float* conf_noise;
  int k_mask_len;
  int64_t* tokens;
  int64_t* pred;
  int B, P , C;
  const int64_t* seeds = nullptr;
  int step = 0;
  float rand_temp = 0.f, conf_w = 0.f;
};
int sample_step(hipStream_t s, const StepArgs& a, const int64_t* tokens_in, const int* num_regen = nullptr, float mask_ratio = 0.f);
int seeded_noise_dump(hipStream_t s, const int64_t* seeds, int step, float rand_temp, float conf_w, float* exp_u, float* exp_noise, float* conf_u,
                      float* conf_noise, int B, int P, int C);

void fill_i64(hipStream_t s, int64_t* dst, int64_t value, size_t n);

void edit_load_tokens(hipStream_t s, const int64_t* src, int64_t* dst, int* num_regen, int B, int P, int C);
void edit_init(hipStream_t s, const int64_t* codes, const uint8_t* regen, int64_t* tokens, int* num_regen, int B, int n, int m, int gbits);
void edit_token_mask(hipStream_t s, const uint8_t* pixel_mask, uint8_t* token_mask, int B, int H, int W, int st);
int edit_composite(hipStream_t s, const float* gen, const float* orig, const uint8_t* pixel_mask, float* out_nchw, uint8_t* out_u8, int B, int C, int H, int W);
void combine_groups(hipStream_t s, const int64_t* tokens , int64_t* codes , size_t rows, int m, int gbits);

void cast_f32_to_h16(hipStream_t s, const float* src, h16* dst, size_t n);
void split_f32_to_h16_planes(hipStream_t s, const float* src, h16* hi, h16* lo, int N, int K, float* scale_out, unsigned* tmp);

}
```

maskbit_amd/csrc/norm_embed.hip:

```cpp
#include "mb_kernels.h"

namespace mb {

constexpr int MAXS = 32;

template <int NV>
__device__ __forceinline__ void fp4_row_store(const float4* v, int lane, uint8_t* x4row, uint8_t* scales, int nseq, int seq, int tok, int groups) {
#pragma unroll
  for (int q = 0; q < NV; ++q) {
    float am = fmaxf(fmaxf(fabsf(v[q].x), fabsf(v[q].y)), fmaxf(fabsf(v[q].z), fabsf(v[q].w)));
    am = row16_max(am);
    if ((lane & 15) == 0) scales[fp4_scale_index(q * 4 + (lane >> 4), nseq, seq, tok, groups)] = (uint8_t)fp4_scale_byte_nosat(am);
    *(uint16_t*)(x4row + q * 128 + lane * 2) = (uint16_t)fp4_pack4(v[q].x, v[q].y, v[q].z, v[q].w, fp4_scale_mul_nosat(am));
  }
}
template <int NV>
__device__ __forceinline__ void fp4_rows_out(const Fp4Rows& f4, float4* v, int lane, int row, int d) {
  const int seq = row / f4.seq_rows, tok = row - seq * f4.seq_rows, groups = (f4.seq_rows - 1) >> 6;
  if (tok == f4.seq_rows - 1) return;
  if (f4.x4) fp4_row_store<NV>(v, lane, f4.x4 + (size_t)row * 2 * d, f4.x4s, f4.nseq, seq, tok, groups);
  if (f4.xl4) {
#pragma unroll
    for (int q = 0; q < NV; ++q)
      v[q] = make_float4(v[q].x - (float)to_h(v[q].x), v[q].y - (float)to_h(v[q].y), v[q].z - (float)to_h(v[q].z), v[q].w - (float)to_h(v[q].w));
    fp4_row_store<NV>(v, lane, f4.xl4 + (size_t)row * 2 * d, f4.xl4s, f4.nseq, seq, tok, groups);
  }
}

template <int NV>
__device__ __forceinline__ void ln_finish(float4* v, const float* sc, int ns, int d, int lane,
                                          const float* __restrict__ gamma, const float* __restrict__ beta,
                                          float eps, float* xo, h16* xb, float* st = nullptr, h16* xl = nullptr,
                                          const Fp4Rows* f4 = nullptr, int row = 0) {
  constexpr bool VEC = NV > 0;
  constexpr int nv = NV;
  float s = 0.f;
  if (VEC) {
#pragma unroll
    for (int q = 0; q < nv; ++q) s += (v[q].x + v[q].y) + (v[q].z + v[q].w);
  }
  else     { for (int q = 0; q < ns; ++q) s += sc[q]; }
  const float mean = wave_sum(s) / (float)d;
  float ss = 0.f;
  if (VEC) {
#pragma unroll
    for (int q = 0; q < nv; ++q) {
      const float a = v[q].x - mean, b = v[q].y - mean, c = v[q].z - mean, e = v[q].w - mean;
      ss += (a * a + b * b) + (c * c + e * e);
    }
  } else {
    for (int q = 0; q < ns; ++q) { const int c = lane + q * 64; if (c < d) { const float a = sc[q] - mean; ss += a * a; } }
  }
  const float rstd = rsqrtf(wave_sum(ss) / (float)d + eps);
  if (st && lane == 0) *(float2*)st = make_float2(mean, rstd);
  if (VEC) {
#pragma unroll
    for (int q = 0; q < nv; ++q) {
      const int c = q * 256 + lane * 4;
      const float4 g = *(const float4*)(gamma + c), b = *(const float4*)(beta + c);
      float4 o;
      o.x = ln_affine(v[q].x, mean, rstd, g.x, b.x); o.y = ln_affine(v[q].y, mean, rstd, g.y, b.y);
      o.z = ln_affine(v[q].z, mean, rstd, g.z, b.z); o.w = ln_affine(v[q].w, mean, rstd, g.w, b.w);
      if (xo) *(float4*)(xo + c) = o;
      const h16x4 hi = {to_h(o.x), to_h(o.y), to_h(o.z), to_h(o.w)};
      if (xb) *(h16x4*)(xb + c) = hi;
      if (xl) *(h16x4*)(xl + c) = h16x4{to_h(o.x - (float)hi[0]), to_h(o.y - (float)hi[1]), to_h(o.z - (float)hi[2]), to_h(o.w - (float)hi[3])};
      if (f4) v[q] = o;
    }
    if constexpr (VEC) { if (f4) fp4_rows_out<NV>(*f4, v, lane, row, d); }
  } else {
    for (int q = 0; q < ns; ++q) {
      const int c = lane + q * 64;
      if (c < d) {
        const float o = ln_affine(sc[q], mean, rstd, gamma[c], beta[c]);
        if (xo) xo[c] = o;
        if (xb) xb[c] = to_h(o);
        if (xl) xl[c] = to_h(o - (float)to_h(o));
      }
    }
  }
}

template <int NV>
__global__ __launch_bounds__(256) void ln_rows_kernel(const float* __restrict__ y, const float* __restrict__ gamma,
                                                      const float* __restrict__ beta, float eps, float* x_f32,
                                                      h16* x_h16, float* stats, int M, int d, h16* x_lo, Fp4Rows f4) {
  const int lane = threadIdx.x & 63;
  const int row = blockIdx.x * 4 + (threadIdx.x >> 6);
  if (row >= M) return;
  const float* yr = y + (size_t)row * d;
  constexpr bool VEC = NV > 0;
  float4 v[VEC ? NV : 1]; float sc[VEC ? 1 : MAXS];
  const int ns = (d + 63) / 64;
  if (VEC) {
#pragma unroll
    for (int q = 0; q < NV; ++q) v[q] = *(const float4*)(yr + q * 256 + lane * 4);
  }
  else     { for (int q = 0; q < ns; ++q) { const int c = lane + q * 64; sc[q] = c < d ? yr[c] : 0.f; } }
  ln_finish<NV>(v, sc, ns, d, lane, gamma, beta, eps, x_f32 ? x_f32 + (size_t)row * d : nullptr,
                 x_h16 ? x_h16 + (size_t)row * d : nullptr, stats ? stats + (size_t)row * 2 : nullptr,
                 x_lo ? x_lo + (size_t)row * d : nullptr,
                 (f4.x4 || f4.xl4) ? &f4 : nullptr, row);
}

template <int NV>
__device__ __forceinline__ float2 ln_normalize(float4* v, int d, const float* __restrict__ gamma, const float* __restrict__ beta, float eps, int lane) {
  float s = 0.f;
#pragma unroll
  for (int q = 0; q < NV; ++q) s += (v[q].x + v[q].y) + (v[q].z + v[q].w);
  const float mean = wave_sum(s) / (float)d;
  float ss = 0.f;
#pragma unroll
  for (int q = 0; q < NV; ++q) {
    const float a = v[q].x - mean, b = v[q].y - mean, c = v[q].z - mean, e = v[q].w - mean;
    ss += (a * a + b * b) + (c * c + e * e);
  }
  const float rstd = rsqrtf(wave_sum(ss) / (float)d + eps);
#pragma unroll
  for (int q = 0; q < NV; ++q) {
    const int c = q * 256 + lane * 4;
    const float4 g = *(const float4*)(gamma + c), b = *(const float4*)(beta + c);
    v[q] = make_float4(ln_affine(v[q].x, mean, rstd, g.x, b.x), ln_affine(v[q].y, mean, rstd, g.y, b.y),
                       ln_affine(v[q].z, mean, rstd, g.z, b.z), ln_affine(v[q].w, mean, rstd, g.w, b.w));
  }
  return make_float2(mean, rstd);
}

template <int NV>
__device__ __forceinline__ void pair_store(float4* xc, const float4* xu, int lane, h16* oc, h16* ou, const Fp4Rows& f4, int row, int d) {
#pragma unroll
  for (int q = 0; q < NV; ++q) {
    const int c = q * 256 + lane * 4;
    *(h16x4*)(oc + c) = h16x4{to_h(xc[q].x), to_h(xc[q].y), to_h(xc[q].z), to_h(xc[q].w)};
    *(h16x4*)(ou + c) = h16x4{to_h(xu[q].x - xc[q].x), to_h(xu[q].y - xc[q].y), to_h(xu[q].z - xc[q].z), to_h(xu[q].w - xc[q].w)};
  }
  if (f4.x4 || f4.xl4) fp4_rows_out<NV>(f4, xc, lane, row, d);
}

template <int NV>
__global__ __launch_bounds__(256) void ln_pair_kernel(const float* __restrict__ y, const float* __restrict__ gamma, const float* __restrict__ beta, float eps,
                                                      h16* __restrict__ x_h16, float* __restrict__ stats, int P, int d, Fp4Rows f4) {
  const int lane = threadIdx.x & 63;
  const int row = blockIdx.x * 4 + (threadIdx.x >> 6);
  if (row >= P) return;
  float4 vc[NV], vu[NV];
#pragma unroll
  for (int q = 0; q < NV; ++q) { vc[q] = *(const float4*)(y + (size_t)row * d + q * 256 + lane * 4); vu[q] = *(const float4*)(y + (size_t)(row + P) * d + q * 256 + lane * 4); }
  const float2 sc = ln_normalize<NV>(vc, d, gamma, beta, eps, lane), su = ln_normalize<NV>(vu, d, gamma, beta, eps, lane);
  if (stats && lane == 0) { *(float2*)(stats + 2 * (size_t)row) = sc; *(float2*)(stats + 2 * (size_t)(row + P)) = su; }
  pair_store<NV>(vc, vu, lane, x_h16 + (size_t)row * d, x_h16 + (size_t)(row + P) * d, f4, row, d);
}

template <int NV>
__global__ __launch_bounds__(256) void pairify_kernel(const float* __restrict__ x32, h16* __restrict__ x_h16, int P, int d, Fp4Rows f4) {
  const int lane = threadIdx.x & 63;
  const int row = blockIdx.x * 4 + (threadIdx.x >> 6);
  if (row >= P) return;
  float4 vc[NV], vu[NV];
#pragma unroll
  for (int q = 0; q < NV; ++q) { vc[q] = *(const float4*)(x32 + (size_t)row * d + q * 256 + lane * 4); vu[q] = *(const float4*)(x32 + (size_t)(row + P) * d + q * 256 + lane * 4); }
  pair_store<NV>(vc, vu, lane, x_h16 + (size_t)row * d, x_h16 + (size_t)(row + P) * d, f4, row, d);
}

int layernorm_pair(hipStream_t s, const float* y, const float* gamma, const float* beta, float eps, h16* x_h16, float* stats, int P, int d,
                   const Fp4Rows& f4) {
  dim3 grid((P + 3) / 4), block(256);
  if (d == 1024) hipLaunchKernelGGL(ln_pair_kernel<4>, grid, block, 0, s, y, gamma, beta, eps, x_h16, stats, P, d, f4);
  else if (d == 768) hipLaunchKernelGGL(ln_pair_kernel<3>, grid, block, 0, s, y, gamma, beta, eps, x_h16, stats, P, d, f4);
  else return -1;
  return 0;
}
int pairify_rows(hipStream_t s, const float* x32, h16* x_h16, int P, int d, const Fp4Rows& f4) {
  dim3 grid((P + 3) / 4), block(256);
  if (d == 1024) hipLaunchKernelGGL(pairify_kernel<4>, grid, block, 0, s, x32, x_h16, P, d, f4);
  else if (d == 768) hipLaunchKernelGGL(pairify_kernel<3>, grid, block, 0, s, x32, x_h16, P, d, f4);
  else return -1;
  return 0;
}

void layernorm_rows(hipStream_t s, const float* y, const float* gamma, const float* beta, float eps,
                    float* x_f32, h16* x_h16, float* stats, int M, int d, h16* x_lo, const Fp4Rows& f4) {
  dim3 grid((M + 3) / 4), block(256);
  if (d == 1024) hipLaunchKernelGGL(ln_rows_kernel<4>, grid, block, 0, s, y, gamma, beta, eps, x_f32, x_h16, stats, M, d, x_lo, f4);
  else if (d == 768) hipLaunchKernelGGL(ln_rows_kernel<3>, grid, block, 0, s, y, gamma, beta, eps, x_f32, x_h16, stats, M, d, x_lo, f4);
  else hipLaunchKernelGGL(ln_rows_kernel<0>, grid, block, 0, s, y, gamma, beta, eps, x_f32, x_h16, stats, M, d, x_lo, Fp4Rows{});
}

constexpr int MAXBITS = 24;

template <int NV>
__global__ __launch_bounds__(256) void embed_ln_kernel(EmbedArgs a) {
  const int lane = threadIdx.x & 63;
  const int row = blockIdx.x * 4 + (threadIdx.x >> 6);
  const int N = a.seq + 1;
  if (row >= a.nb * N) return;
  const int sq = row / N, t = row - sq * N;
  const int d = a.d, K = a.m * a.gbits;
  uint32_t plus = 0, live = 0;
  const float* cls = nullptr;
  const float* trow[8] = {};
  if (t < a.seq) {
    for (int g = 0; g < a.m; ++g) {
      const int64_t idx = a.tokens[((size_t)sq * a.seq + t) * a.m + g];
      if (a.tables && g < 8) {
        const int64_t nrow = ((int64_t)1 << a.gbits) + 1;
        const int64_t ix = idx < 0 ? 0 : (idx >= nrow ? nrow - 1 : idx);
        trow[g] = a.tables + ((size_t)g * nrow + (size_t)ix) * d;
      }
      const uint32_t gm = (1u << a.gbits) - 1u;
      if (idx != ((int64_t)1 << a.gbits)) { live |= gm << (g * a.gbits); plus |= ((uint32_t)idx & gm) << (g * a.gbits); }
    }
  } else {
    int64_t lab = a.labels[sq];
    if (a.drop && a.drop[sq]) lab = a.nclass;
    lab = lab < 0 ? 0 : (lab > a.nclass ? a.nclass : lab);
    cls = a.class_emb + (size_t)lab * d;
  }
  const float* pos = a.pos + (size_t)t * d;
  constexpr bool VEC = NV > 0;
  float4 v[VEC ? NV : 1]; float sc[VEC ? 1 : MAXS];
  const int ns = (d + 63) / 64;
  if (VEC) {
#pragma unroll
    for (int q = 0; q < NV; ++q) {
      const int c = q * 256 + lane * 4;
      float4 e = cls ? *(const float4*)(cls + c) : (a.tables ? make_float4(0.f, 0.f, 0.f, 0.f) : *(const float4*)(a.b_in + c));
      if (!cls && a.tables) {
#pragma unroll
        for (int g = 0; g < 8; ++g)
          if (g < a.m) { const float4 w = *(const float4*)(trow[g] + c); e.x += w.x; e.y += w.y; e.z += w.z; e.w += w.w; }
      } else if (!cls) {
#pragma unroll
        for (int j = 0; j < MAXBITS; ++j) {
          if (j < K) {
            const float4 w = *(const float4*)(a.w_in + (size_t)j * d + c);
            const float sj = ((live >> j) & 1u) ? (((plus >> j) & 1u) ? 1.f : -1.f) : 0.f;
            e.x = fmaf(sj, w.x, e.x); e.y = fmaf(sj, w.y, e.y); e.z = fmaf(sj, w.z, e.z); e.w = fmaf(sj, w.w, e.w);
          }
        }
      }
      const float4 p = *(const float4*)(pos + c);
      v[q] = make_float4(e.x + p.x, e.y + p.y, e.z + p.z, e.w + p.w);
    }
  } else {
    for (int q = 0; q < ns; ++q) {
      const int c = lane + q * 64;
      float e = 0.f;
      if (c < d) {
        if (cls) e = cls[c];
        else if (a.tables) {
          for (int g = 0; g < a.m && g < 8; ++g) e += trow[g][c];
        } else {
          e = a.b_in[c];
          for (int j = 0; j < K; ++j) {
            const float sj = ((live >> j) & 1u) ? (((plus >> j) & 1u) ? 1.f : -1.f) : 0.f;
            e = fmaf(sj, a.w_in[(size_t)j * d + c], e);
          }
        }
        e += pos[c];
      }
      sc[q] = e;
    }
  }
  ln_finish<NV>(v, sc, ns, d, lane, a.gamma, a.beta, 1e-12f, a.x_f32 + (size_t)row * d, a.x_h16 + (size_t)row * d, nullptr,
                 a.x_lo ? a.x_lo + (size_t)row * d : nullptr,
                 (a.f4.x4 || a.f4.xl4) ? &a.f4 : nullptr, row);
}

// ... 87 lines not shown
```

Before: 34.39.

## Add alternating block-walk order across transformer kernels for cache reuse

Introduces walk_tile/walk_seq/walk_row helpers that remap block indices into grouped and optionally reversed orders. They are threaded through attention, layernorm, pairify and GEMM launches so consecutive kernels can visit sequences in an order that reuses data the previous kernel left in the last-level cache. A fused GEMM+layernorm diagnostic entry point is also added. The remapping adds some index arithmetic per block, and changing the traversal order could hurt locality if the grouping does not fit the cache.

Result: faster. 34.75, median of 6 (+1.0%).

```diff
diff --git a/include/maskbit_hip_diag.h b/include/maskbit_hip_diag.h
--- a/include/maskbit_hip_diag.h
+++ b/include/maskbit_hip_diag.h
@@ -27,6 +27,8 @@
 int mb_split_f32_planes(const float* src, void* hi, void* lo, int N, int K, float* scale_out, unsigned* tmp, mb_stream stream);
 int mb_gemm_mini_split(int epi, const void* A_hi, const void* A_lo, const void* W, const float* bias, void* out_h16, void* out4, void* out4_scale,
                        int rows, int N, int kw, const void* const* lo, mb_stream stream);
+int mb_gemm_mini_ln(const void* A, const void* W, const float* bias, float* y, const float* ln_stats, const float* ln_g, const float* ln_b, int rows, int pair,
+                    int seq_rows, int N, int K, int nlo, const void* const* lo, mb_stream stream);
 int mb_layernorm_f4(const float* y, const float* gamma, const float* beta, float eps, float* x_f32, void* x_h16, void* x4, void* x4_scale, void* xl4,
                     void* xl4_scale, int M, int d, mb_stream stream);
 int mb_layernorm_f4_seq(const float* y, const float* gamma, const float* beta, float eps, float* x_f32, void* x_h16, void* x4, void* x4_scale, void* xl4,
@@ -47,6 +49,12 @@
 int mb_attention_probs(const void* qkv, float* out_f32, int nb, int N, int d, int heads, mb_stream stream);
 int mb_gen_set_alo(mb_gen* g, int gemm_mask);
 int mb_set_cu_count(int n);
+int mb_gen_set_walk(mb_gen* g, int mode);
+int mb_diag_set_walk(int reverse);
+int mb_walk_tile(int vb, int ntiles, int reverse);
+int mb_walk_seq(int slot, int n, int grp, int reverse);
+int mb_walk_row(int slot, int rows, int seq_rows, int pair, int reverse);
+int mb_walk_group(int seq_rows, int pair);
 int mb_gemm_ht_supported(int epi, int M, int N, int K);
 
 int mb_seeded_noise(const int64_t* seeds, int step, float randomize_temperature, float conf_weight, float* exp_u, float* exp_noise, float* conf_u,
diff --git a/maskbit_amd/_lib.py b/maskbit_amd/_lib.py
--- a/maskbit_amd/_lib.py
+++ b/maskbit_amd/_lib.py
@@ -94,6 +94,7 @@
                                    C.c_int, C.c_int, C.c_int, C.c_int, C.POINTER(C.c_void_p), C.c_void_p]),
     "mb_gemm_mini_split": (C.c_int, [C.c_int, C.c_void_p, C.c_void_p, C.c_void_p, C.c_void_p, C.c_void_p, C.c_void_p, C.c_void_p, C.c_int, C.c_int, C.c_int,
                                      C.POINTER(C.c_void_p), C.c_void_p]),
+    "mb_gemm_mini_ln": (C.c_int, [C.c_void_p] * 7 + [C.c_int] * 6 + [C.POINTER(C.c_void_p), C.c_void_p]),
     "mb_gemm_act_split": (C.c_int, [C.c_int, C.c_void_p, C.c_void_p, C.c_void_p, C.c_void_p, C.c_void_p, C.c_void_p, C.c_void_p, C.c_int, C.c_int, C.c_int,
                                     C.c_int, C.c_void_p]),
     "mb_gemm": (C.c_int, [C.c_int, C.c_void_p, C.c_void_p, C.c_void_p, C.c_void_p, C.c_void_p, C.c_void_p, C.c_int, C.c_int, C.c_int,
@@ -142,6 +143,12 @@
     "mb_taming_set_tap": (C.c_int, [C.c_void_p, C.c_int, C.c_void_p]),
     "mb_spatial_attention": (C.c_int, [C.c_void_p] * 5 + [C.c_int] * 4 + [C.c_void_p]),
     "mb_set_cu_count":(C.c_int, [C.c_int]),
+    "mb_gen_set_walk": (C.c_int, [C.c_void_p, C.c_int]),
+    "mb_diag_set_walk": (C.c_int, [C.c_int]),
+    "mb_walk_tile": (C.c_int, [C.c_int] * 3),
+    "mb_walk_seq": (C.c_int, [C.c_int] * 4),
+    "mb_walk_row": (C.c_int, [C.c_int] * 5),
+    "mb_walk_group": (C.c_int, [C.c_int] * 2),
     "mb_gemm_ht_supported": (C.c_int, [C.c_int, C.c_int, C.c_int, C.c_int]),
     "mb_prof_enable": (C.c_int, [C.c_int]),
     "mb_prof_read": (C.c_int, [C.c_char_p, C.c_int]),
diff --git a/maskbit_amd/csrc/attention.hip b/maskbit_amd/csrc/attention.hip
--- a/maskbit_amd/csrc/attention.hip
+++ b/maskbit_amd/csrc/attention.hip
@@ -49,7 +49,8 @@
 __global__ __launch_bounds__(64 * ATT_NW, 2) void attention_kernel(const h16* __restrict__ qkv, h16* __restrict__ out,
                                                           int N, int d, int heads, float scale_log2e, int sq_off = 0,
                                                           uint8_t* __restrict__ out4 = nullptr, uint8_t* __restrict__ out4s = nullptr, int out4_nseq = 0,
-                                                          uint8_t* __restrict__ out4l = nullptr, uint8_t* __restrict__ out4ls = nullptr) {
+                                                          uint8_t* __restrict__ out4l = nullptr, uint8_t* __restrict__ out4ls = nullptr,
+                                                          int reverse = 0, int wgrp = 8) {
   constexpr int ROW = DH * 2;
   constexpr int SL = DH / 8;
   constexpr int KS = DH / 32;
@@ -62,7 +63,9 @@
   const int wave = __builtin_amdgcn_readfirstlane(tid >> 6);
   char* Ks = smem;
   char* Vs = Ks + ATT_NP * ROW;
-  const int sq0 = blockIdx.x / heads, h = blockIdx.x - sq0 * heads;
+  const int wslot = reverse ? (int)(gridDim.x - 1 - blockIdx.x) : (int)blockIdx.x;
+  const int sslot = wslot / heads, h = wslot - sslot * heads;
+  const int sq0 = walk_seq(sslot, (int)gridDim.x / heads, wgrp, 0);
   const size_t rs = (size_t)3 * d;
   constexpr int NPASS = AUX == 4 ? 2 : 1;
   f32x4 oc[AUX == 4 ? ATT_MAXQT - 1 : 1][DH / 16];
@@ -262,7 +265,8 @@
 __global__ __launch_bounds__(256, 2) void attention_long_kernel(const h16* __restrict__ qkv, h16* __restrict__ out,
                                                                int N, int d, int heads, int nchunk, float scale_log2e, int sq_off = 0,
                                                                uint8_t* __restrict__ out4 = nullptr, uint8_t* __restrict__ out4s = nullptr, int out4_nseq = 0,
-                                                               uint8_t* __restrict__ out4l = nullptr, uint8_t* __restrict__ out4ls = nullptr) {
+                                                               uint8_t* __restrict__ out4l = nullptr, uint8_t* __restrict__ out4ls = nullptr,
+                                                               int reverse = 0, int wgrp = 8) {
   constexpr int ROW = DH * 2, SL = DH / 8, KS = DH / 32, NT = DH / 16, RPI = 64 / SL;
   constexpr int BLK_BYTES = ATTL_KB * ROW;
   constexpr int NINST = ATTL_KB / RPI;
@@ -270,9 +274,10 @@
   __shared__ __attribute__((aligned(16))) char smem[2 * 2 * BLK_BYTES];
   const int tid = threadIdx.x, lane = tid & 63;
   const int wave = __builtin_amdgcn_readfirstlane(tid >> 6);
-  int bid = blockIdx.x;
+  int bid = reverse ? (int)(gridDim.x - 1 - blockIdx.x) : (int)blockIdx.x;
   const int chunk = bid % nchunk; bid /= nchunk;
-  const int sq0 = bid / heads, h = bid - sq0 * heads;
+  const int sslot = bid / heads, h = bid - sslot * heads;
+  const int sq0 = walk_seq(sslot, (int)gridDim.x / (heads * nchunk), wgrp, 0);
   const size_t rs = (size_t)3 * d;
   auto kswz = [](int row) { return SL == 8 ? ((row >> 1) & 7) : ((0 - (row >> 2)) & 3); };
   auto vswz = [](int row) { return SL == 8 ? (((row >> 1) & 3) << 1) : (((row >> 1) & 1) << 1); };
@@ -486,26 +491,31 @@
 
 static bool att_streams(int N) { return N > ATT_NP || N < ATT_NP - 32; }
 
-void attention(hipStream_t s, const h16* qkv, h16* out, int nb, int N, int d, int heads, uint8_t* out4, uint8_t* out4s) {
+void attention(hipStream_t s, const h16* qkv, h16* out, int nb, int N, int d, int heads, uint8_t* out4, uint8_t* out4s, int reverse) {
   const int dh = d / heads;
+  const int wg = walk_group(N, false);
+  uint8_t* const nil = nullptr;
   const float scale_log2e = 1.4426950408889634f / sqrtf((float)dh);
   if (att_streams(N)) {
     const int nchunk = (N + 63) / 64;
     const bool f4 = N > ATT_NP && (N - 1) % 64 == 0;
     dim3 grid(nb * heads * nchunk), block(256);
-    if (dh == 64) hipLaunchKernelGGL(attention_long_kernel<64>, grid, block, 0, s, qkv, out, N, d, heads, nchunk, scale_log2e, 0, f4 ? out4 : nullptr, f4 ? out4s : nullptr, nb);
-    else hipLaunchKernelGGL(attention_long_kernel<32>, grid, block, 0, s, qkv, out, N, d, heads, nchunk, scale_log2e);
+    if (dh == 64) hipLaunchKernelGGL(attention_long_kernel<64>, grid, block, 0, s, qkv, out, N, d, heads, nchunk, scale_log2e, 0, f4 ? out4 : nil, f4 ? out4s : nil, nb, nil, nil, reverse, wg);
+    else hipLaunchKernelGGL(attention_long_kernel<32>, grid, block, 0, s, qkv, out, N, d, heads, nchunk, scale_log2e, 0, nil, nil, 0, nil, nil, reverse, wg);
     return;
   }
   dim3 grid(nb * heads), block(64 * ATT_NW);
   if (out4 && dh == 64 && N == 257)
-    hipLaunchKernelGGL((attention_kernel<64, 5>), grid, block, 0, s, qkv, out, N, d, heads, scale_log2e, 0, out4, out4s, nb);
-  else if (dh == 64) hipLaunchKernelGGL(attention_kernel<64>, grid, block, 0, s, qkv, out, N, d, heads, scale_log2e);
-  else hipLaunchKernelGGL(attention_kernel<32>, grid, block, 0, s, qkv, out, N, d, heads, scale_log2e);
-}
-
-int attention_pair(hipStream_t s, const h16* qkv, h16* out, int P, int N, int d, int heads, uint8_t* out4, uint8_t* out4s, uint8_t* out4l, uint8_t* out4ls) {
+    hipLaunchKernelGGL((attention_kernel<64, 5>), grid, block, 0, s, qkv, out, N, d, heads, scale_log2e, 0, out4, out4s, nb, nil, nil, reverse, wg);
+  else if (dh == 64) hipLaunchKernelGGL(attention_kernel<64>, grid, block, 0, s, qkv, out, N, d, heads, scale_log2e, 0, nil, nil, 0, nil, nil, reverse, wg);
+  else hipLaunchKernelGGL(attention_kernel<32>, grid, block, 0, s, qkv, out, N, d, heads, scale_log2e, 0, nil, nil, 0, nil, nil, reverse, wg);
+}
+
+int attention_pair(hipStream_t s, const h16* qkv, h16* out, int P, int N, int d, int heads, uint8_t* out4, uint8_t* out4s, uint8_t* out4l, uint8_t* out4ls,
+                   int reverse) {
   const int dh = d / heads;
+  const int wg = walk_group(N, true);
+  uint8_t* const nil = nullptr;
   if (dh != 64 && dh != 32) return -1;
   if ((out4l || out4ls) && (!out4 || !out4s || !out4l || !out4ls)) return -1;
   const float scale_log2e = 1.4426950408889634f / sqrtf((float)dh);
@@ -513,14 +523,14 @@
     if ((out4 || out4s) && (dh != 64 || (N - 1) % 64 || N < ATT_NP)) return -1;
     const int nchunk = ((N + 15) / 16 + 3) / 4;
     dim3 grid(P * heads * nchunk), block(256);
-    if (dh == 64) hipLaunchKernelGGL((attention_long_kernel<64, true>), grid, block, 0, s, qkv, out, N, d, heads, nchunk, scale_log2e, P, out4, out4s, P, out4l, out4ls);
-    else hipLaunchKernelGGL((attention_long_kernel<32, true>), grid, block, 0, s, qkv, out, N, d, heads, nchunk, scale_log2e, P);
+    if (dh == 64) hipLaunchKernelGGL((attention_long_kernel<64, true>), grid, block, 0, s, qkv, out, N, d, heads, nchunk, scale_log2e, P, out4, out4s, P, out4l, out4ls, reverse, wg);
+    else hipLaunchKernelGGL((attention_long_kernel<32, true>), grid, block, 0, s, qkv, out, N, d, heads, nchunk, scale_log2e, P, nil, nil, 0, nil, nil, reverse, wg);
     return 0;
   }
   dim3 grid(P * heads), block(64 * ATT_NW);
   if ((out4 || out4s) && (dh != 64 || N != 257)) return -1;
-  if (dh == 64) hipLaunchKernelGGL((attention_kernel<64, 4>), grid, block, 0, s, qkv, out, N, d, heads, scale_log2e, P, out4, out4s, P, out4l, out4ls);
-  else hipLaunchKernelGGL((attention_kernel<32, 4>), grid, block, 0, s, qkv, out, N, d, heads, scale_log2e, P);
+  if (dh == 64) hipLaunchKernelGGL((attention_kernel<64, 4>), grid, block, 0, s, qkv, out, N, d, heads, scale_log2e, P, out4, out4s, P, out4l, out4ls, reverse, wg);
+  else hipLaunchKernelGGL((attention_kernel<32, 4>), grid, block, 0, s, qkv, out, N, d, heads, scale_log2e, P, nil, nil, 0, nil, nil, reverse, wg);
   return 0;
 }
 
diff --git a/maskbit_amd/csrc/diag.hip b/maskbit_amd/csrc/diag.hip
--- a/maskbit_amd/csrc/diag.hip
+++ b/maskbit_amd/csrc/diag.hip
@@ -13,7 +13,11 @@
 
 namespace {
 
-int run_gemm(mb_stream stream, int epi, const mb::GemmArgs& a, int variant, const char* mini = nullptr) {
+int g_walk_reverse = 0;
+
+int run_gemm(mb_stream stream, int epi, const mb::GemmArgs& args, int variant, const char* mini = nullptr) {
+  mb::GemmArgs a = args;
+  a.reverse = g_walk_reverse;
   ProfScope p("gemm_diag", (hipStream_t)stream);
   if (mb::gemm_tn((hipStream_t)stream, (mb::GemmEpi)epi, a, variant))
     return mini ? fail(-3, "%s: shape refused", mini) : fail(-3, "GEMM shape M=%d N=%d K=%d is outside the kernels' shapes", a.M, a.N, a.K);
@@ -74,6 +78,17 @@
 extern "C" {
 
 int mb_set_cu_count(int n) { mb::set_cu_count(n); return 0; }
+int mb_diag_set_walk(int reverse) {
+  if (reverse != 0 && reverse != 1) return fail(-1, "mb_diag_set_walk: direction 0 or 1");
+  g_walk_reverse = reverse;
+  return 0;
+}
+int mb_walk_tile(int vb, int ntiles, int reverse) { return vb < 0 || vb >= ntiles ? -1 : mb::walk_tile(vb, ntiles, reverse ? 1 : 0); }
+int mb_walk_seq(int slot, int n, int grp, int reverse) { return slot < 0 || slot >= n || grp < 1 ? -1 : mb::walk_seq(slot, n, grp, reverse ? 1 : 0); }
+int mb_walk_row(int slot, int rows, int seq_rows, int pair, int reverse) {
+  return slot < 0 || slot >= rows ? -1 : mb::walk_row(slot, rows, mb::walk_rows(rows, seq_rows, pair != 0, reverse));
+}
+int mb_walk_group(int seq_rows, int pair) { return seq_rows < 2 ? -1 : mb::walk_group(seq_rows, pair != 0); }
 int mb_gemm_ht_supported(int epi, int M, int N, int K) {
   mb::GemmArgs a{nullptr, nullptr, nullptr, nullptr, nullptr, nullptr, M, N, K, 0};
   return mb::gemm_ht_supported((mb::GemmEpi)epi, a) ? 1 : 0;
@@ -119,6 +134,18 @@
   if ((!seq_rows && a.M % 257) || !mb::gemm_ht_supported((mb::GemmEpi)epi, a)) return fail(-3, "mb_gemm_mini: shape not supported by the sequence-aligned tiles");
   return run_gemm(stream, epi, a, 257, "mb_gemm_mini");
 }
+int mb_gemm_mini_ln(const void* A, const void* W, const float* bias, float* y, const float* ln_stats, const float* ln_g, const float* ln_b, int rows, int pair,
+                    int seq_rows, int N, int K, int nlo, const void* const* lo, mb_stream stream) {
+  if (!A || !W || !bias || !y || !ln_stats || !ln_g || !ln_b || rows <= 0 || K <= 0 || K % 64 || nlo < 0 || nlo > 2 || (nlo && !lo))
+    return fail(-1, "mb_gemm_mini_ln: bad arguments");
+  mb::GemmArgs a{(const h16*)A, (const h16*)W, bias, y, y, nullptr, pair ? 2 * rows : rows, N, K, 0, nullptr, ln_stats, ln_g, ln_b};
+  if (pair) a.pair_rows = rows;
+  a.seq_rows = seq_rows;
+  a.nlo = nlo;
+  for (int i = 0; i < nlo; ++i) a.lo[i] = {(const uint8_t*)lo[4 * i], (const uint8_t*)lo[4 * i + 1], (const uint8_t*)lo[4 * i + 2], (const uint8_t*)lo[4 * i + 3]};
+  if ((!seq_rows && a.M % 257) || !mb::gemm_ht_supported(mb::EPI_RES_F32, a)) return fail(-3, "mb_gemm_mini_ln: shape not supported by the sequence-aligned tiles");
+  return run_gemm(stream, mb::EPI_RES_F32, a, 257, "mb_gemm_mini_ln");
+}
 int mb_gemm_mini_split(int epi, const void* A_hi, const void* A_lo, const void* W, const float* bias, void* out_h16, void* out4, void* out4_scale,
                        int rows, int N, int kw, const void* const* lo , mb_stream stream) {
   if (!A_hi || !A_lo || !W || !bias || !out_h16 || !lo || epi < 0 || epi > 1 || rows <= 0 || rows % 257 || kw <= 0 || kw % 128)
@@ -166,7 +193,7 @@
 int mb_layernorm(const float* y, const float* gamma, const float* beta, float eps, float* x_f32, void* x_h16, void* x_lo, float* stats, int M,
                  int d, mb_stream stream) {
   if (!y || !gamma || !beta || M <= 0 || d <= 0 || d > 2048) return fail(-1, "mb_layernorm: bad arguments");
-  mb::layernorm_rows((hipStream_t)stream, y, gamma, beta, eps, x_f32, (h16*)x_h16, stats, M, d, (h16*)x_lo);
+  mb::layernorm_rows((hipStream_t)stream, y, gamma, beta, eps, x_f32, (h16*)x_h16, stats, M, d, (h16*)x_lo, mb::Fp4Rows{}, g_walk_reverse, 0);
   return launched();
 }
 int mb_layernorm_f4_seq(const float* y, const float* gamma, const float* beta, float eps, float* x_f32, void* x_h16, void* x4, void* x4_scale, void* xl4,
@@ -174,7 +201,7 @@
   if (!y || !gamma || !beta || (!x4 && !xl4) || M <= 0) return fail(-1, "mb_layernorm_f4: bad arguments (an e2m1 output is required)");
   mb::Fp4Rows f4;
   if (int rc = f4_rows("mb_layernorm_f4", f4, x4, x4_scale, xl4, xl4_scale, M, d, seq_rows)) return rc;
-  mb::layernorm_rows((hipStream_t)stream, y, gamma, beta, eps, x_f32, (h16*)x_h16, nullptr, M, d, nullptr, f4);
+  mb::layernorm_rows((hipStream_t)stream, y, gamma, beta, eps, x_f32, (h16*)x_h16, nullptr, M, d, nullptr, f4, g_walk_reverse, seq_rows);
   return launched();
 }
 int mb_layernorm_f4(const float* y, const float* gamma, const float* beta, float eps, float* x_f32, void* x_h16, void* x4, void* x4_scale, void* xl4,
@@ -187,7 +214,7 @@
   if (!y || !gamma || !beta || !x_h16 || P <= 0 || d <= 0 || d > 2048) return fail(-1, "mb_layernorm_pair: bad arguments");
   mb::Fp4Rows f4;
   if (int rc = f4_rows("mb_layernorm_pair", f4, x4, x4_scale, xl4, xl4_scale, P, d, seq_rows)) return rc;
-  if (mb::layernorm_pair((hipStream_t)stream, y, gamma, beta, eps, (h16*)x_h16, stats, P, d, f4))
+  if (mb::layernorm_pair((hipStream_t)stream, y, gamma, beta, eps, (h16*)x_h16, stats, P, d, f4, g_walk_reverse, seq_rows))
     return fail(-3, "mb_layernorm_pair: width %d is outside the pair kernels (768 or 1024)", d);
   return launched();
 }
@@ -195,7 +222,7 @@
   if (!x_f32 || !x_h16 || P <= 0 || d <= 0 || d > 2048) return fail(-1, "mb_pairify: bad arguments");
   mb::Fp4Rows f4;
   if (int rc = f4_rows("mb_pairify", f4, x4, x4_scale, xl4, xl4_scale, P, d, seq_rows)) return rc;
-  if (mb::pairify_rows((hipStream_t)stream, x_f32, (h16*)x_h16, P, d, f4))
+  if (mb::pairify_rows((hipStream_t)stream, x_f32, (h16*)x_h16, P, d, f4, g_walk_reverse, seq_rows))
     return fail(-3, "mb_pairify: width %d is outside the pair kernels (768 or 1024)", d);
   return launched();
 }
@@ -233,7 +260,7 @@
   if (!qkv || !out_h16 || (!out4) != (!out4_scale) || nb <= 0 || N <= 0 || d <= 0 || heads <= 0 || d % heads) return fail(-1, "mb_attention: bad arguments");
   if (d / heads != 32 && d / heads != 64) return fail(-3, "mb_attention: head width %d is outside the attention kernels (32 or 64)", d / heads);
   ProfScope p("attention", (hipStream_t)stream);
-  mb::attention((hipStream_t)stream, (const h16*)qkv, (h16*)out_h16, nb, N, d, heads, (uint8_t*)out4, (uint8_t*)out4_scale);
+  mb::attention((hipStream_t)stream, (const h16*)qkv, (h16*)out_h16, nb, N, d, heads, (uint8_t*)out4, (uint8_t*)out4_scale, g_walk_reverse);
   return launched();
 }
 int mb_attention_probs(const void* qkv, float* out_f32, int nb, int N, int d, int heads, mb_stream stream) {
@@ -245,14 +272,14 @@
 int mb_attention_pair(const void* qkv, void* out_h16, int pairs, int N, int d, int heads, mb_stream stream) {
   if (!qkv || !out_h16 || pairs <= 0 || N <= 0 || heads <= 0 || d % heads) return fail(-1, "mb_attention_pair: bad arguments");
   ProfScope p("attention", (hipStream_t)stream);
-  if (mb::attention_pair((hipStream_t)stream, (const h16*)qkv, (h16*)out_h16, pairs, N, d, heads, nullptr, nullptr))
+  if (mb::attention_pair((hipStream_t)stream, (const h16*)qkv, (h16*)out_h16, pairs, N, d, heads, nullptr, nullptr, nullptr, nullptr, g_walk_reverse))
     return fail(-3, "mb_attention_pair: head width %d (N = %d tokens) is outside the attention kernels", d / heads, N);
   return launched();
 }
 int mb_attention_pair_f4(const void* qkv, void* out_h16, void* out4, void* out4_scale, void* out4l, void* out4l_scale, int pairs, int N, int d, int heads, mb_stream stream) {
   if (!qkv || !out_h16 || !out4 || !out4_scale || (!out4l) != (!out4l_scale) || pairs <= 0 || N <= 0 || heads <= 0 || d % heads) return fail(-1, "mb_attention_pair_f4: bad arguments");
   ProfScope p("attention", (hipStream_t)stream);
-  if (mb::attention_pair((hipStream_t)stream, (const h16*)qkv, (h16*)out_h16, pairs, N, d, heads, (uint8_t*)out4, (uint8_t*)out4_scale, (uint8_t*)out4l, (uint8_t*)out4l_scale))
+  if (mb::attention_pair((hipStream_t)stream, (const h16*)qkv, (h16*)out_h16, pairs, N, d, heads, (uint8_t*)out4, (uint8_t*)out4_scale, (uint8_t*)out4l, (uint8_t*)out4l_scale, g_walk_reverse))
     return fail(-3, "mb_attention_pair_f4: head width %d / N = %d tokens: no e2m1 copy for this shape", d / heads, N);
   return launched();
 }
diff --git a/maskbit_amd/csrc/engine.hip b/maskbit_amd/csrc/engine.hip
--- a/maskbit_amd/csrc/engine.hip
+++ b/maskbit_amd/csrc/engine.hip
@@ -55,6 +55,7 @@
   } run;
   int* num_regen = nullptr;
   int alo_mask = 0, alo_mask_built = 0;
+  int walk = 1;
   int64_t *tok_a = nullptr, *tok_b = nullptr, *tok_cfg = nullptr, *lab_cfg = nullptr, *pred = nullptr, *codes = nullptr;
   uint8_t* drop_cfg = nullptr;
   float* logits = nullptr;
@@ -98,6 +99,8 @@
     return attn ? attention_probs(s, g->qkv, attn + (size_t)l * nb * N * N, nb, N, d, c.heads) : 0;
   };
   int attn_rc = 0, gemm_rc = 0;
+  int wdir = 0;
+  auto walk_next = [&] { wdir ^= g->walk; return wdir; };
   const bool xlo = c.precision >= 1;
   const bool wm = g->mini_ok && c.precision >= 2;
   const bool xlo_all = xlo && !wm;
@@ -117,6 +120,7 @@
     if (wm && epi == EPI_GELU_H16) { ga.out4 = g->h4.v; ga.out4_scale = g->h4.s; }
     if (((widx & 3) == 2 || xlo_all) && xlo_layer(widx >> 2)) { ga.K = 2 * d; ga.A2 = g->x_lo; ga.kw = d; }
     ga.sat = g->sat;
+    ga.reverse = walk_next();
     gemm_rc |= gemm_tn(s, epi, ga, wm ? 257 : 0);
   };
   auto rgemm = [&](const h16* A, const h16* W, const float* bias, int K, int widx, const uint8_t* a4, const uint8_t* a4s, const float* ln_g, const float* ln_b) {
@@ -124,6 +128,7 @@
     if (ln_g) { ga.ln_stats = g->ln_stats; ga.ln_g = ln_g; ga.ln_b = ln_b; }
     if (wm) ga.seq_rows = N;
     lo_set(ga, a4, a4s, widx);
+    ga.reverse = walk_next();
     gemm_rc |= gemm_tn(s, EPI_RES_F32, ga, wm ? 257 : 0);
   };
   {
@@ -136,23 +141,23 @@
   }
   for (int l = 0; l < c.depth; ++l) {
     const mb_gen::Layer& L = g->layers[l];
-    if (c.prenorm) { ProfScope p("layernorm", s, true); layernorm_rows(s, g->y_f32, L.ln1g, L.ln1b, 1e-12f, nullptr, g->x_h16, nullptr, M, d, xlo_qkv, f4x); }
+    if (c.prenorm) { ProfScope p("layernorm", s, true); layernorm_rows(s, g->y_f32, L.ln1g, L.ln1b, 1e-12f, nullptr, g->x_h16, nullptr, M, d, xlo_qkv, f4x, walk_next(), N); }
     { ProfScope p("gemm_qkv", s, true); xgemm(EPI_H16, L.wqkv, L.bqkv, g->qkv, 3 * d, 4 * l); }
-    { ProfScope p("attention", s, true); attention(s, g->qkv, g->att, nb, N, d, c.heads, wm ? g->att4.v : nullptr, wm ? g->att4.s : nullptr); }
+    { ProfScope p("attention", s, true); attention(s, g->qkv, g->att, nb, N, d, c.heads, wm ? g->att4.v : nullptr, wm ? g->att4.s : nullptr, walk_next()); }
     attn_rc |= attn_maps(l);
     { ProfScope p("gemm_attn_out", s, true);
       const bool re = !c.prenorm && l > 0;
       rgemm(g->att, L.wo, L.bo, d, 4 * l + 1, g->att4.v, g->att4.s, re ? g->layers[l - 1].ln2g : nullptr, re ? g->layers[l - 1].ln2b : nullptr); }
     { ProfScope p("layernorm", s, true);
-      layernorm_rows(s, g->y_f32, c.prenorm ? L.ln2g : L.ln1g, c.prenorm ? L.ln2b : L.ln1b, 1e-12f, nullptr, g->x_h16, c.prenorm ? nullptr : g->ln_stats, M, d, xlo_layer(l) ? xlo_ffn : nullptr, f4x); }
+      layernorm_rows(s, g->y_f32, c.prenorm ? L.ln2g : L.ln1g, c.prenorm ? L.ln2b : L.ln1b, 1e-12f, nullptr, g->x_h16, c.prenorm ? nullptr : g->ln_stats, M, d, xlo_layer(l) ? xlo_ffn : nullptr, f4x, walk_next(), N); }
     { ProfScope p("gemm_ffn_up", s, true); xgemm(EPI_GELU_H16, L.w1, L.b1, g->h, f, 4 * l + 2); }
     { ProfScope p("gemm_ffn_down", s, true);
       rgemm(g->h, L.w2, L.b2, f, 4 * l + 3, g->h4.v, g->h4.s, c.prenorm ? nullptr : L.ln1g, c.prenorm ? nullptr : L.ln1b); }
     if (!c.prenorm) { ProfScope p("layernorm", s, true);
       const bool last = l + 1 == c.depth;
-      layernorm_rows(s, g->y_f32, L.ln2g, L.ln2b, 1e-12f, nullptr, g->x_h16, g->ln_stats, M, d, last ? g->x_lo : xlo_qkv, last ? Fp4Rows{} : f4x); }
-  }
-  if (c.prenorm) { ProfScope p("layernorm", s, true); layernorm_rows(s, g->y_f32, g->lnag, g->lnab, 1e-12f, nullptr, g->x_h16, nullptr, M, d, g->x_lo); }
+      layernorm_rows(s, g->y_f32, L.ln2g, L.ln2b, 1e-12f, nullptr, g->x_h16, g->ln_stats, M, d, last ? g->x_lo : xlo_qkv, last ? Fp4Rows{} : f4x, walk_next(), N); }
+  }
+  if (c.prenorm) { ProfScope p("layernorm", s, true); layernorm_rows(s, g->y_f32, g->lnag, g->lnab, 1e-12f, nullptr, g->x_h16, nullptr, M, d, g->x_lo, Fp4Rows{}, walk_next(), N); }
   gemm_rc |= head_gemms(g, logits, M, s);
   if (int rc = launched()) return rc;
   if (attn_rc) return fail(-3, "attention maps: head dim %d / %d tokens not supported", d / c.heads, N);
@@ -166,6 +171,8 @@
   const mb_gen_cfg& c = g->c;
   const int d = c.hidden, f = c.mlp, N = g->N, nb = 2 * B, M = nb * N, P = B * N;
   int rc = 0;
+  int wdir = 0;
+  auto walk_next = [&] { wdir ^= g->walk; return wdir; };
   auto alo_on = [&](int gemm) { return wmode && c.precision >= 3 && ((g->alo_mask >> gemm) & 1); };
   auto f4_for = [&](bool feeds_ffn = false) {
     Fp4Rows f;
@@ -185,6 +192,7 @@
       ga.nlo = lo; ga.lo[0] = {a4, a4s, g->w4lo[widx], g->w4los[widx]};
       if (lo == 2) ga.lo[1] = {al4, al4s, g->w4[widx], g->w4s[widx]};
     }
+    ga.reverse = walk_next();
     return ga;
   };
   {
@@ -195,12 +203,12 @@
     if (embed_pair(s, e)) {
       e.drop = drop; e.nb = nb; e.f4 = Fp4Rows{};
       embed_ln(s, e);
-      rc |= pairify_rows(s, g->y_f32, g->x_h16, P, d, f4_for());
+      rc |= pairify_rows(s, g->y_f32, g->x_h16, P, d, f4_for(), walk_next(), N);
     }
   }
   if (c.prenorm && c.depth > 0) {
     ProfScope p("layernorm", s, true);
-    rc |= layernorm_pair(s, g->y_f32, g->layers[0].ln1g, g->layers[0].ln1b, 1e-12f, g->x_h16, nullptr, P, d, f4_for());
+    rc |= layernorm_pair(s, g->y_f32, g->layers[0].ln1g, g->layers[0].ln1b, 1e-12f, g->x_h16, nullptr, P, d, f4_for(), walk_next(), N);
   }
   for (int l = 0; l < c.depth; ++l) {
     const mb_gen::Layer& L = g->layers[l];
@@ -210,13 +218,13 @@
       rc |= gemm_tn(s, EPI_H16, ga, 257); }
     const bool lo_o = alo_on(1), lo_h = alo_on(3);
     { ProfScope p("attention", s, true); rc |= attention_pair(s, g->qkv, g->att, B, N, d, c.heads, wmode ? g->att4.v : nullptr, wmode ? g->att4.s : nullptr,
-                                                              lo_o ? g->attl4.v : nullptr, lo_o ? g->attl4.s : nullptr); }
+                                                              lo_o ? g->attl4.v : nullptr, lo_o ? g->attl4.s : nullptr, walk_next()); }
     { ProfScope p("gemm_attn_out", s, true);
       GemmArgs ga = pgemm(EPI_RES_F32, g->att, L.wo, L.bo, nullptr, g->y_f32, d, d, 4 * l + 1, wmode ? (alo_on(1) ? 2 : 1) : 0, g->att4.v, g->att4.s, g->attl4.v, g->attl4.s);
       if (l > 0 && !c.prenorm) { ga.ln_stats = g->ln_stats; ga.ln_g = g->layers[l - 1].ln2g; ga.ln_b = g->layers[l - 1].ln2b; }
       rc |= gemm_tn(s, EPI_RES_F32, ga, 257); }
     { ProfScope p("layernorm", s, true);
-      rc |= layernorm_pair(s, g->y_f32, c.prenorm ? L.ln2g : L.ln1g, c.prenorm ? L.ln2b : L.ln1b, 1e-12f, g->x_h16, c.prenorm ? nullptr : g->ln_stats, P, d, f4_for(true)); }
+      rc |= layernorm_pair(s, g->y_f32, c.prenorm ? L.ln2g : L.ln1g, c.prenorm ? L.ln2b : L.ln1b, 1e-12f, g->x_h16, c.prenorm ? nullptr : g->ln_stats, P, d, f4_for(true), walk_next(), N); }
     { ProfScope p("gemm_ffn_up", s, true);
       GemmArgs ga = pgemm(EPI_GELU_H16, g->x_h16, L.w1, L.b1, g->h, nullptr, f, d, 4 * l + 2, xlo_mode, g->x4.v, g->x4.s, g->xl4.v, g->xl4.s);
       if (wmode) { ga.out4 = g->h4.v; ga.out4_scale = g->h4.s; }
@@ -228,11 +236,11 @@
       rc |= gemm_tn(s, EPI_RES_F32, ga, 257); }
     { ProfScope p("layernorm", s, true);
       if (c.prenorm) {
-        if (l + 1 == c.depth) layernorm_rows(s, g->y_f32, g->lnag, g->lnab, 1e-12f, nullptr, g->x_h16, nullptr, M, d, g->x_lo);
-        else rc |= layernorm_pair(s, g->y_f32, g->layers[l + 1].ln1g, g->layers[l + 1].ln1b, 1e-12f, g->x_h16, nullptr, P, d, f4_for());
+        if (l + 1 == c.depth) layernorm_rows(s, g->y_f32, g->lnag, g->lnab, 1e-12f, nullptr, g->x_h16, nullptr, M, d, g->x_lo, Fp4Rows{}, walk_next(), N);
+        else rc |= layernorm_pair(s, g->y_f32, g->layers[l + 1].ln1g, g->layers[l + 1].ln1b, 1e-12f, g->x_h16, nullptr, P, d, f4_for(), walk_next(), N);
       }
-      else if (l + 1 == c.depth) layernorm_rows(s, g->y_f32, L.ln2g, L.ln2b, 1e-12f, nullptr, g->x_h16, g->ln_stats, M, d, g->x_lo);
-      else rc |= layernorm_pair(s, g->y_f32, L.ln2g, L.ln2b, 1e-12f, g->x_h16, g->ln_stats, P, d, f4_for()); }
+      else if (l + 1 == c.depth) layernorm_rows(s, g->y_f32, L.ln2g, L.ln2b, 1e-12f, nullptr, g->x_h16, g->ln_stats, M, d, g->x_lo, Fp4Rows{}, walk_next(), N);
+      else rc |= layernorm_pair(s, g->y_f32, L.ln2g, L.ln2b, 1e-12f, g->x_h16, g->ln_stats, P, d, f4_for(), walk_next(), N); }
   }
   rc |= head_gemms(g, logits, M, s);
   if (int lrc = launched()) return lrc;
@@ -483,6 +491,12 @@
   return 0;
 }
 
+int mb_gen_set_walk(mb_gen* g, int mode) {
+  if (!g || (mode != 0 && mode != 1)) return fail(-1, "mb_gen_set_walk: mode 0 (every launch front to back) or 1 (alternating)");
+  g->walk = mode;
+  return 0;
+}
+
 int mb_gen_saturation_count(mb_gen* g, unsigned* count, int reset, mb_stream stream) {
   if (!g || !count) return fail(-1, "mb_gen_saturation_count: null argument");
   HIP_TRY(hipMemcpyAsync(count, g->sat, sizeof(unsigned), hipMemcpyDeviceToHost, (hipStream_t)stream));
diff --git a/maskbit_amd/csrc/gemm.hip b/maskbit_amd/csrc/gemm.hip
--- a/maskbit_amd/csrc/gemm.hip
+++ b/maskbit_amd/csrc/gemm.hip
@@ -15,7 +15,7 @@
   const int wm = wave >> 1, wn = wave & 1;
   const int tiles_n = (a.N + BN - 1) / BN;
   const int tiles_m = (a.M + BM - 1) / BM;
-  const int L = xcd_remap(blockIdx.x, tiles_m * tiles_n);
+  const int L = walk_tile(blockIdx.x, tiles_m * tiles_n, a.reverse);
   const int m0 = (L / tiles_n) * BM, n0 = (L % tiles_n) * BN;
   const int K = a.K, KA = a.kw ? a.kw : a.K, nka = KA / BK;
   const int KW = a.kw ? a.kw : a.K, nkw = KW / BK;
diff --git a/maskbit_amd/csrc/gemm_ht.hip b/maskbit_amd/csrc/gemm_ht.hip
--- a/maskbit_amd/csrc/gemm_ht.hip
+++ b/maskbit_amd/csrc/gemm_ht.hip
@@ -63,7 +63,7 @@
   auto make_plan = [&](int vb, Plan& p) {
     int lane_o = lane;
     asm volatile("" : "+v"(lane_o));
-    const int L = xcd_remap(vb, ntiles);
+    const int L = walk_tile(vb, ntiles, a.reverse);
     const int sr = L / (8 * tiles_n);
     const int rows_sr = min(8, tiles_m - sr * 8);
     const int rem = L - sr * 8 * tiles_n;
diff --git a/maskbit_amd/csrc/mb_common.h b/maskbit_amd/csrc/mb_common.h
--- a/maskbit_amd/csrc/mb_common.h
+++ b/maskbit_amd/csrc/mb_common.h
@@ -113,7 +113,7 @@
   return __fmaf_rn(__fmul_rn(__fsub_rn(v, mean), rstd), g, b);
 }
 
-__device__ __forceinline__ int xcd_remap(int b, int nblk) {
+__host__ __device__ __forceinline__ int xcd_remap(int b, int nblk) {
   const int q = nblk >> 3, r = nblk & 7, x = b & 7, i = b >> 3;
   return (x < r ? x * (q + 1) : r * (q + 1) + (x - r) * q) + i;
 }
diff --git a/maskbit_amd/csrc/mb_kernels.h b/maskbit_amd/csrc/mb_kernels.h
--- a/maskbit_amd/csrc/mb_kernels.h
+++ b/maskbit_amd/csrc/mb_kernels.h
@@ -37,6 +37,7 @@
   LoSet lo[2] = {};
   int nlo = 0;
   unsigned* sat = nullptr;
+  int reverse = 0;
 };
 __host__ __device__ inline size_t w4_packed_offset(int n, int k, int K) {
   const int r = n & 15, c = (k & 127) >> 5;
@@ -48,6 +49,36 @@
 __host__ __device__ inline size_t fp4_scale_index(int blk, int nseq, int seq, int r, int groups = 4) {
   return (((size_t)blk * nseq + seq) * groups + (r >> 6)) * 64 + (r & 15) * 4 + ((r >> 4) & 3);
 }
+__host__ __device__ inline int walk_tile(int vb, int ntiles, int reverse) { return xcd_remap(reverse ? ntiles - 1 - vb : vb, ntiles); }
+__host__ __device__ inline int xcd_chunk_start(int x, int n) { return xcd_remap(x, n); }
+__host__ __device__ inline int walk_seq(int slot, int n, int grp, int reverse) {
+  if (reverse) slot = n - 1 - slot;
+  const int q = n >> 3, r = n & 7;
+  for (int lo = 0, before = 0;; lo += grp) {
+    const int a = q + 1 - lo < grp ? (q + 1 - lo > 0 ? q + 1 - lo : 0) : grp;
+    const int b = q - lo < grp ? (q - lo > 0 ? q - lo : 0) : grp;
+    const int step = r * a + (8 - r) * b;
+    if (slot < before + step) {
+      int s = slot - before, x;
+      if (s < r * a) { x = s / a; s -= x * a; }
+      else { s -= r * a; x = s / b; s -= x * b; x += r; }
+      return xcd_chunk_start(x, n) + lo + s;
+    }
+    before += step;
+  }
+}
+inline int walk_group(int seq_rows, bool pair) { const int tps = (seq_rows - 1) / (pair ? 128 : 256); return tps >= 8 ? 1 : tps >= 1 ? 8 / tps : 8; }
+struct WalkRows { int seq_rows, grp, reverse; };
+__host__ __device__ inline int walk_row(int slot, int rows, const WalkRows& w) {
+  if (w.reverse) slot = rows - 1 - slot;
+  const int ss = slot / w.seq_rows;
+  return walk_seq(ss, rows / w.seq_rows, w.grp, 0) * w.seq_rows + (slot - ss * w.seq_rows);
+}
+inline WalkRows walk_rows(int rows, int seq_rows, bool pair, int reverse) {
+  if (seq_rows <= 0 || rows % seq_rows) return WalkRows{rows, 8, reverse ? 1 : 0};
+  return WalkRows{seq_rows, walk_group(seq_rows, pair), reverse ? 1 : 0};
+}
+
 int gemm_tn(hipStream_t s, GemmEpi epi, const GemmArgs& a, int variant = 0);
 bool gemm_ht_supported(GemmEpi epi, const GemmArgs& a);
 void gemm_ht(hipStream_t s, GemmEpi epi, const GemmArgs& a, int mt);
@@ -60,11 +91,11 @@
 
 void layernorm_rows(hipStream_t s, const float* y, const float* gamma, const float* beta, float eps,
                     float* x_f32, h16* x_h16, float* stats, int M, int d, h16* x_lo = nullptr,
-                    const Fp4Rows& f4 = Fp4Rows{});
+                    const Fp4Rows& f4 = Fp4Rows{}, int reverse = 0, int seq_rows = 0);
 
 int layernorm_pair(hipStream_t s, const float* y, const float* gamma, const float* beta, float eps, h16* x_h16, float* stats, int P, int d,
-                   const Fp4Rows& f4 = Fp4Rows{});
-int pairify_rows(hipStream_t s, const float* x32, h16* x_h16, int P, int d, const Fp4Rows& f4 = Fp4Rows{});
+                   const Fp4Rows& f4 = Fp4Rows{}, int reverse = 0, int seq_rows = 0);
+int pairify_rows(hipStream_t s, const float* x32, h16* x_h16, int P, int d, const Fp4Rows& f4 = Fp4Rows{}, int reverse = 0, int seq_rows = 0);
 
 struct EmbedArgs {
   const int64_t* tokens;
@@ -86,9 +117,9 @@
 void transpose_f32(hipStream_t s, const float* src , float* dst , int rows, int cols);
 
 void attention(hipStream_t s, const h16* qkv, h16* out, int nb, int N, int d, int heads,
-               uint8_t* out4 = nullptr, uint8_t* out4s = nullptr);
+               uint8_t* out4 = nullptr, uint8_t* out4s = nullptr, int reverse = 0);
 int attention_pair(hipStream_t s, const h16* qkv, h16* out, int P, int N, int d, int heads, uint8_t* out4 = nullptr, uint8_t* out4s = nullptr,
-                   uint8_t* out4l = nullptr, uint8_t* out4ls = nullptr);
+                   uint8_t* out4l = nullptr, uint8_t* out4ls = nullptr, int reverse = 0);
 int attention_probs(hipStream_t s, const h16* qkv, float* out, int nb, int N, int d, int heads);
 
 struct StepArgs {
diff --git a/maskbit_amd/csrc/norm_embed.hip b/maskbit_amd/csrc/norm_embed.hip
--- a/maskbit_amd/csrc/norm_embed.hip
+++ b/maskbit_amd/csrc/norm_embed.hip
@@ -84,10 +84,11 @@
 template <int NV>
 __global__ __launch_bounds__(256) void ln_rows_kernel(const float* __restrict__ y, const float* __restrict__ gamma,
                                                       const float* __restrict__ beta, float eps, float* x_f32,
-                                                      h16* x_h16, float* stats, int M, int d, h16* x_lo, Fp4Rows f4) {
-  const int lane = threadIdx.x & 63;
-  const int row = blockIdx.x * 4 + (threadIdx.x >> 6);
-  if (row >= M) return;
+                                                      h16* x_h16, float* stats, int M, int d, h16* x_lo, Fp4Rows f4, WalkRows wk) {
+  const int lane = threadIdx.x & 63;
+  const int slot = blockIdx.x * 4 + __builtin_amdgcn_readfirstlane(threadIdx.x >> 6);
+  if (slot >= M) return;
+  const int row = walk_row(slot, M, wk);
   const float* yr = y + (size_t)row * d;
   constexpr bool VEC = NV > 0;
   float4 v[VEC ? NV : 1]; float sc[VEC ? 1 : MAXS];
@@ -139,10 +140,11 @@
 
 template <int NV>
 __global__ __launch_bounds__(256) void ln_pair_kernel(const float* __restrict__ y, const float* __restrict__ gamma, const float* __restrict__ beta, float eps,
-                                                      h16* __restrict__ x_h16, float* __restrict__ stats, int P, int d, Fp4Rows f4) {
-  const int lane = threadIdx.x & 63;
-  const int row = blockIdx.x * 4 + (threadIdx.x >> 6);
-  if (row >= P) return;
+                                                      h16* __restrict__ x_h16, float* __restrict__ stats, int P, int d, Fp4Rows f4, WalkRows wk) {
+  const int lane = threadIdx.x & 63;
+  const int slot = blockIdx.x * 4 + __builtin_amdgcn_readfirstlane(threadIdx.x >> 6);
+  if (slot >= P) return;
+  const int row = walk_row(slot, P, wk);
   float4 vc[NV], vu[NV];
 #pragma unroll
   for (int q = 0; q < NV; ++q) { vc[q] = *(const float4*)(y + (size_t)row * d + q * 256 + lane * 4); vu[q] = *(const float4*)(y + (size_t)(row + P) * d + q * 256 + lane * 4); }
@@ -152,10 +154,11 @@
 }
 
 template <int NV>
-__global__ __launch_bounds__(256) void pairify_kernel(const float* __restrict__ x32, h16* __restrict__ x_h16, int P, int d, Fp4Rows f4) {
-  const int lane = threadIdx.x & 63;
-  const int row = blockIdx.x * 4 + (threadIdx.x >> 6);
-  if (row >= P) return;
+__global__ __launch_bounds__(256) void pairify_kernel(const float* __restrict__ x32, h16* __restrict__ x_h16, int P, int d, Fp4Rows f4, WalkRows wk) {
+  const int lane = threadIdx.x & 63;
+  const int slot = blockIdx.x * 4 + __builtin_amdgcn_readfirstlane(threadIdx.x >> 6);
+  if (slot >= P) return;
+  const int row = walk_row(slot, P, wk);
   float4 vc[NV], vu[NV];
 #pragma unroll
   for (int q = 0; q < NV; ++q) { vc[q] = *(const float4*)(x32 + (size_t)row * d + q * 256 + lane * 4); vu[q] = *(const float4*)(x32 + (size_t)(row + P) * d + q * 256 + lane * 4); }
@@ -163,27 +166,30 @@
 }
 
 int layernorm_pair(hipStream_t s, const float* y, const float* gamma, const float* beta, float eps, h16* x_h16, float* stats, int P, int d,
-                   const Fp4Rows& f4) {
+                   const Fp4Rows& f4, int reverse, int seq_rows) {
   dim3 grid((P + 3) / 4), block(256);
-  if (d == 1024) hipLaunchKernelGGL(ln_pair_kernel<4>, grid, block, 0, s, y, gamma, beta, eps, x_h16, stats, P, d, f4);
-  else if (d == 768) hipLaunchKernelGGL(ln_pair_kernel<3>, grid, block, 0, s, y, gamma, beta, eps, x_h16, stats, P, d, f4);
+  const WalkRows wk = walk_rows(P, seq_rows, true, reverse);
+  if (d == 1024) hipLaunchKernelGGL(ln_pair_kernel<4>, grid, block, 0, s, y, gamma, beta, eps, x_h16, stats, P, d, f4, wk);
+  else if (d == 768) hipLaunchKernelGGL(ln_pair_kernel<3>, grid, block, 0, s, y, gamma, beta, eps, x_h16, stats, P, d, f4, wk);
   else return -1;
   return 0;
 }
-int pairify_rows(hipStream_t s, const float* x32, h16* x_h16, int P, int d, const Fp4Rows& f4) {
+int pairify_rows(hipStream_t s, const float* x32, h16* x_h16, int P, int d, const Fp4Rows& f4, int reverse, int seq_rows) {
   dim3 grid((P + 3) / 4), block(256);
-  if (d == 1024) hipLaunchKernelGGL(pairify_kernel<4>, grid, block, 0, s, x32, x_h16, P, d, f4);
-  else if (d == 768) hipLaunchKernelGGL(pairify_kernel<3>, grid, block, 0, s, x32, x_h16, P, d, f4);
+  const WalkRows wk = walk_rows(P, seq_rows, true, reverse);
+  if (d == 1024) hipLaunchKernelGGL(pairify_kernel<4>, grid, block, 0, s, x32, x_h16, P, d, f4, wk);
+  else if (d == 768) hipLaunchKernelGGL(pairify_kernel<3>, grid, block, 0, s, x32, x_h16, P, d, f4, wk);
   else return -1;
   return 0;
 }
 
 void layernorm_rows(hipStream_t s, const float* y, const float* gamma, const float* beta, float eps,
-                    float* x_f32, h16* x_h16, float* stats, int M, int d, h16* x_lo, const Fp4Rows& f4) {
+                    float* x_f32, h16* x_h16, float* stats, int M, int d, h16* x_lo, const Fp4Rows& f4, int reverse, int seq_rows) {
   dim3 grid((M + 3) / 4), block(256);
-  if (d == 1024) hipLaunchKernelGGL(ln_rows_kernel<4>, grid, block, 0, s, y, gamma, beta, eps, x_f32, x_h16, stats, M, d, x_lo, f4);
-  else if (d == 768) hipLaunchKernelGGL(ln_rows_kernel<3>, grid, block, 0, s, y, gamma, beta, eps, x_f32, x_h16, stats, M, d, x_lo, f4);
-  else hipLaunchKernelGGL(ln_rows_kernel<0>, grid, block, 0, s, y, gamma, beta, eps, x_f32, x_h16, stats, M, d, x_lo, Fp4Rows{});
+  const WalkRows wk = walk_rows(M, seq_rows, false, reverse);
+  if (d == 1024) hipLaunchKernelGGL(ln_rows_kernel<4>, grid, block, 0, s, y, gamma, beta, eps, x_f32, x_h16, stats, M, d, x_lo, f4, wk);
+  else if (d == 768) hipLaunchKernelGGL(ln_rows_kernel<3>, grid, block, 0, s, y, gamma, beta, eps, x_f32, x_h16, stats, M, d, x_lo, f4, wk);
+  else hipLaunchKernelGGL(ln_rows_kernel<0>, grid, block, 0, s, y, gamma, beta, eps, x_f32, x_h16, stats, M, d, x_lo, Fp4Rows{}, wk);
 }
 
 constexpr int MAXBITS = 24;
```
